# olofson/audiality2

Hardware: AMD Instinct MI355X
Metric: voice-samples/sec + max realtime voices @48kHz (higher is better)
Workload: dtype int32; 1 GPU; 65536 voices 2xwtosc->panmix, 256 per group voice inline->fbdelay->fbdelay (benchmark/fmtest4.a2s delay settings; 256 groups, 512 fbdelays), 48 kHz, fragment=64, stereo (BASELINE configs[3]); voices_per_gpu=65536, chain=osc2-pan, groups=256

## Files before the change

audiality2_amd/build.py:

```python
import hashlib
import os
import shutil
import subprocess

HERE = os.path.dirname(os.path.abspath(__file__))
ROOT = os.path.dirname(HERE)
HIPCC = shutil.which("hipcc") or "/opt/rocm/bin/hipcc"


MARK = b"A2AMD_SRCHASH:"


def source_hash(sources, cmd=()):
    h = hashlib.sha256()
    for s in sources:
        h.update(os.path.basename(s).encode() + b"\0")
        with open(s, "rb") as f:
            h.update(f.read())
        h.update(b"\0")
    h.update(" ".join(cmd).encode())
    return h.hexdigest()[:32]


def stamped_hash(lib, mark=MARK):
    if not os.path.exists(lib):
        return None
    with open(lib, "rb") as f:
        blob = f.read()
    i = blob.find(mark)
    if i < 0:
        return None
    return blob[i + len(mark):i + len(mark) + 32].decode("ascii", "replace")


ENGMARK = b"A2AMD_ENGHASH:"


def engine_hash(engine):
    files = []
    for d in ("include", "src", os.path.join("src", "units"), os.path.join("src", "drivers")):
        p = os.path.join(engine, d)
        if os.path.isdir(p):
            files += [os.path.join(p, f) for f in sorted(os.listdir(p)) if f.endswith((".h", ".h.cmake", ".h.in"))]
    return source_hash(files, (stamped_hash(os.path.join(HERE, "liba2amd_units.so")) or "",))


def _stale(target, want):
    return stamped_hash(target) != want


def _define(h):
    return '-DA2AMD_SRCHASH="%s"' % h


def build_lib(force=False):
    csrc = os.path.join(HERE, "csrc")
    srcs = [os.path.join(csrc, f) for f in ("a2amd_host.cpp", "a2amd_sched.cpp", "a2amd_render.cpp", "a2amd_dist.cpp",
                                            "a2amd_vm.cpp", "a2amd_kernels.hip", "a2amd_fast.hip", "a2amd_vm.hip", "a2amd_wavecap.hip", "a2amd_wavepost.hip", "a2amd_win.hip", "a2amd_vmwin.hip", "a2amd_noise.hip", "a2amd_noisepan.hip", "a2amd_noisefiltpan.hip", "a2amd_cutsweep.hip", "a2amd_oscbare.hip")]
    deps = srcs + [os.path.join(csrc, "a2amd_host.h"), os.path.join(csrc, "a2amd_switches.h"), os.path.join(csrc, "a2amd_device.h"), os.path.join(csrc, "a2amd_dsp.h"),
                   os.path.join(csrc, "a2amd_fm.h"), os.path.join(csrc, "a2amd_vmcore.h"), os.path.join(csrc, "a2amd_taps.h"), os.path.join(csrc, "a2amd_winctl.h"), os.path.join(csrc, "a2amd_vmdev.h"), os.path.join(csrc, "a2amd_noisemap.h"), os.path.join(csrc, "a2amd_noisevoice.h"), os.path.join(csrc, "a2amd_settled.h"), os.path.join(csrc, "a2amd_cutsweep.h"), os.path.join(csrc, "a2amd_filt.h"), os.path.join(ROOT, "include", "a2amd.h"),
                   os.path.join(ROOT, "include", "a2amd_noise.h"), os.path.join(ROOT, "include", "a2amd_noisepan.h"), os.path.join(ROOT, "include", "a2amd_noisefilt.h"), os.path.join(ROOT, "include", "a2amd_sweep.h"), os.path.join(ROOT, "include", "a2amd_wavepost.h"),
                   os.path.join(ROOT, "include", "a2amd_bus.h"), os.path.join(ROOT, "include", "a2amd_oscbare.h"), os.path.join(ROOT, "include", "a2amd_fbdpan.h"), os.path.join(ROOT, "include", "a2amd_buswin.h"), os.path.join(ROOT, "include", "a2amd_vmbatch.h"), os.path.join(ROOT, "include", "a2amd_osc2.h"), os.path.join(ROOT, "include", "a2amd_vm.h")]
    out = os.path.join(HERE, "liba2amd.so")
    flags = ["--offload-arch=gfx950", "-O3", "-std=c++17", "-fPIC", "-shared", "-Wno-unused-value"]
    want = source_hash(deps, flags)
    if force or _stale(out, want):
        subprocess.run([HIPCC] + flags + [_define(want), "-o", out] + srcs, check=True)
    return out


def build_units(force=False):
    src = os.path.join(HERE, "csrc", "a2amd_units.c")
    deps = [src, os.path.join(ROOT, "include", "a2amd.h"), os.path.join(ROOT, "include", "a2amd_noise.h"), os.path.join(ROOT, "include", "a2amd_noisepan.h"),
            os.path.join(ROOT, "include", "a2amd_noisefilt.h"), os.path.join(ROOT, "include", "a2amd_sweep.h"), os.path.join(ROOT, "include", "a2amd_bus.h"),
            os.path.join(ROOT, "include", "a2amd_wavepost.h"), os.path.join(ROOT, "include", "a2amd_oscbare.h"), os.path.join(ROOT, "include", "a2amd_fbdpan.h"), os.path.join(ROOT, "include", "a2amd_buswin.h"), os.path.join(ROOT, "include", "a2amd_vmbatch.h"), os.path.join(ROOT, "include", "a2amd_osc2.h"), os.path.join(ROOT, "include", "a2amd_plugin.h"),
            os.path.join(ROOT, "include", "a2amd_walk.h"), os.path.join(ROOT, "include", "a2amd_vm.h")]
    out = os.path.join(HERE, "liba2amd_units.so")
    flags = ["-O2", "-Wall", "-fPIC", "-shared"]
    want = source_hash(deps, flags)
    if force or _stale(out, want):
        subprocess.run(["gcc"] + flags + [_define(want), "-o", out, src,
                        "-L" + HERE, "-la2amd", "-ldl", "-lpthread", "-lm", "-Wl,-rpath,$ORIGIN"], check=True)
    return out


def build_walk(force=False, engine=None):
    engine = engine or os.environ.get("A2_ENGINE_SRC", "/root/reference")
    out = os.path.join(HERE, "liba2amd_walk.so")
    src = os.path.join(HERE, "csrc", "a2amd_walk.c")
    own = [src, os.path.join(ROOT, "include", "a2amd_walk.h"), os.path.join(ROOT, "include", "a2amd_vm.h"),
           os.path.join(ROOT, "include", "a2amd_plugin.h")]
    flags = ["-O2", "-Wall", "-fPIC", "-shared"]
    want = source_hash(own, flags)
    kept = os.path.join(ROOT, "oracle", "_ref", "liba2amd_walk.so")
    if not (os.path.exists(os.path.join(engine, "src", "internals.h")) and shutil.which("cmake")):
        if (not os.path.exists(out) or _stale(out, want)) and not _stale(kept, want):
            shutil.copyfile(kept, out)
        if os.path.exists(out) and _stale(out, want):
            raise RuntimeError(f"{out} was not built from this tree's a2amd_walk.c (stamp {stamped_hash(out)}, "
                               f"sources {want}) and the engine's source tree ({engine}) is not here to rebuild it")
        return out if os.path.exists(out) else None
    inc = os.path.join(HERE, "_engine_include")
    weng = engine_hash(engine)
    if force or _stale(out, want) or stamped_hash(out, ENGMARK) != weng:
        subprocess.run(["cmake", f"-DENGINE={engine}", f"-DOUT={inc}", "-P", os.path.join(HERE, "csrc", "engine_header.cmake")],
                       check=True, stdout=subprocess.DEVNULL)
        subprocess.run(["gcc"] + flags + [_define(want), '-DA2AMD_ENGHASH="%s"' % weng, "-I" + inc] +
                       ["-I" + os.path.join(engine, d) for d in ("include", "src", "src/units", "src/drivers")] +
                       ["-o", out, src, "-L" + HERE, "-la2amd_units", "-la2amd", "-ldl", "-lpthread", "-Wl,-rpath,$ORIGIN"],
                       check=True)
    if stamped_hash(kept) != want or stamped_hash(kept, ENGMARK) != weng:
        os.makedirs(os.path.dirname(kept), exist_ok=True)
        shutil.copyfile(out, kept)
    return out


def build_oracle(force=False):
    odir = os.path.join(ROOT, "oracle")
    targets = ["restate"]
    if os.path.exists("/root/reference/src/core.c") and shutil.which("cmake"):
        targets += ["ref", "tools", "optionb"]
    subprocess.run(["make", "-s", "-C", odir] + (["-B"] if force else []) + targets, check=True)
    return os.path.join(odir, "liba2oracle.so")


def build_all(force=False):
    lib = build_lib(force)
    build_units(force)
    build_walk(force)
    return lib, build_oracle(force)
```

audiality2_amd/csrc/a2amd_device.h:

```cpp
#pragma once
#include <stdint.h>

#define A2D_MAXCHAIN   16
#define A2D_CHAIN_INLINE 8
#define A2D_MAXBATCH 256
#define FBW_MAXWIN (2 * A2D_MAXBATCH)
#define A2D_USTATE    24
#define A2D_MAXCH      8
#define A2D_FRAG      64
#define A2D_MIPS      10
#define A2D_FBD_BUFSIZE 131072
#define A2D_MAXPHINC  512
#define A2D_COEF_WORDS 3
#define A2D_WTOSC_MAXLENGTH (0x01000000 - 1 - 131)

enum { A2D_WTOSC = 0, A2D_PANMIX, A2D_FILTER12, A2D_FBDELAY, A2D_INLINE, A2D_XINSERT,
	A2D_FM1, A2D_FM2, A2D_FM3, A2D_FM4, A2D_FM3P, A2D_FM4P, A2D_FM2R, A2D_FM4R,
	A2D_DC, A2D_WAVESHAPER, A2D_DCBLOCK, A2D_LIMITER, A2D_XSINK, A2D_XSOURCE };
#define A2D_IS_FM(k) ((k) >= A2D_FM1 && (k) <= A2D_FM4R)

enum { A2D_OSC_OFF = 0, A2D_OSC_NOISE, A2D_OSC_WAVE, A2D_OSC_MIPWAVE };

#define A2D_DESC(kind, add, nin, nout, wired) \
	(((uint32_t)(kind) << 24) | ((uint32_t)(add) << 4) | ((uint32_t)(nin) << 8) | \
	 ((uint32_t)(nout) << 12) | ((uint32_t)(wired) << 16))
#define A2D_KIND(d)  ((d) >> 24)
#define A2D_ADD(d)   (((d) >> 4) & 1u)
#define A2D_NIN(d)   (((d) >> 8) & 15u)
#define A2D_NOUT(d)  (((d) >> 12) & 15u)
#define A2D_WIRED(d) (((d) >> 16) & 1u)

enum {
	OW_MODE = 0, OW_WAVE, OW_DPHASE, OW_PHASE_LO, OW_PHASE_HI, OW_NOISE,
	OW_PRAMPING, OW_P = 7, OW_A = 11, OW_SEED = 15 };
enum {
	PW_VOL = 0, PW_PAN = 4 };
enum {
	FW_Q = 0, FW_LP = 4, FW_BP, FW_HP, FW_F1, FW_D1A, FW_D1B, FW_D2A, FW_D2B,
	FW_F1NEXT, FW_RAMP };
enum {
	DW_FBDELAY = 0, DW_LDELAY, DW_RDELAY, DW_DRYGAIN, DW_FBGAIN, DW_LGAIN,
	DW_RGAIN, DW_BUFPOS, DW_BUFIDX };

enum {
	CW_VALUE = 0, CW_MODE = 4 };
enum {
	SW_AMOUNT = 0 };
enum {
	BW_F1 = 0, BW_D1A, BW_D1B, BW_D2A, BW_D2B };
enum {
	LW_RELEASE = 0, LW_THRESHOLD, LW_PEAK };
enum {
	MW_SLOT = 0 };
enum {
	FO_A = 0, FO_FB = 4, FO_P = 8, FO_LASTPITCH = 12, FO_PHASE, FO_DPHASE, FO_LAST, FO_WORDS };
#define A2D_FMSTATE 64

#define A2D_WF_RAWTAPS 0x40000000u

struct A2DWave {
	int32_t  type;
	uint32_t flags;
	uint32_t period;
	uint32_t size[A2D_MIPS];
	uint32_t off[A2D_MIPS];
	uint32_t pad;
};

struct A2DVoice {
	int32_t nunits;
	int32_t unit[A2D_CHAIN_INLINE];
	int32_t out_off, out_nch;
	int32_t own_off, own_nch;
	int32_t pad[3];
};

static_assert(sizeof(A2DVoice) == 64, "the voice record is one 64-byte line");
struct A2DVoiceExt { int32_t unit[A2D_MAXCHAIN - A2D_CHAIN_INLINE]; };

struct A2DRec {
	uint32_t head;
	int32_t  value;
	uint32_t dur;
	uint32_t start;
};
enum { R_SEG = 1, R_WRITE, R_INIT, R_KILL, R_F1SET, R_F1RAMP, R_NOISESEED, R_NOP };
#define A2D_HEAD(frag, op, unit, reg) \
	((uint32_t)(frag) | ((uint32_t)(op) << 16) | ((uint32_t)(unit) << 24) | ((uint32_t)(reg) << 28))
#define A2D_RFRAG(h) ((h) & 0xffffu)
#define A2D_ROP(h)   (((h) >> 16) & 0xffu)
#define A2D_RUNIT(h) (((h) >> 24) & 15u)
#define A2D_RREG(h)  (((h) >> 28) & 15u)

struct A2DRun { int32_t first, count; };

#define A2D_VM_NOWRITE 0xffu
#define A2D_VM_TRAPWRITE 0xfeu
#define A2D_VM_MAXCUT  2
#define A2D_VM_MAXENV  2
#define A2D_VM_MAXPOS  8
#define A2D_VM_ENVPOS  14
#define A2D_ENV_LUTSHIFT 6
#define A2D_ENV_LUTSIZE  (1 << A2D_ENV_LUTSHIFT)
#define A2D_ENV_LUTS     8
struct A2DVmEnv {
	int32_t ramper[4];
	int32_t lut;
	int32_t scale, offset, out;
	int32_t active;
	uint8_t regbase;
	uint8_t k;
	uint8_t target;
	uint8_t pad;
};
struct A2DVmVoice {
	uint32_t waketime;
	uint32_t code, ncode;
	uint16_t pc;
	uint8_t  state, ncut;
	int32_t  voice;
	int32_t  fault;
	uint8_t  cmap[64];
	uint8_t  kind[A2D_MAXCHAIN];
	uint8_t  cutpos[A2D_VM_MAXCUT];
	uint8_t  pad[2];
	int32_t  cut[A2D_VM_MAXCUT][4];
	A2DVmEnv env[A2D_VM_MAXENV];
	int32_t  nenv;
	uint32_t exit_when;
	int32_t  has_exit;
	int32_t  r[64];
};

struct A2DVmParams {
	A2DVmVoice     *vmv;
	const int      *list;
	int32_t         n;
	const uint32_t *code;
	const uint32_t *ptab;
	const int32_t  *f1tab;
	const uint16_t *envlut;
	A2DRun         *runs;
	A2DRun         *vmrun;
	A2DRec         *recs;
	uint32_t        rec_base, rec_cap;
	uint32_t       *total;
	uint32_t        now;
	uint32_t        msdur;
	int32_t         samplerate, basepitch;
	int32_t         nfrags;
	uint8_t         fragframes[A2D_MAXBATCH];
	uint8_t         fragbase[A2D_MAXBATCH];
};

enum { XW_SLOT = 0, XW_MODE = 1 };
#define A2D_XIO_HALF ((size_t)A2D_MAXBATCH * 8 * A2D_FRAG)
#define A2D_XIO_SLOT (2 * A2D_XIO_HALF)

#define A2D_FAST_FCH 8
#define A2D_OSC2_FCH 4
#define A2D_OSC2_SCH 16
#define A2D_MAXVPW   32

struct A2DParams {
	const A2DVoice *voices;
	const A2DVoiceExt *vext;
	const uint32_t *udesc;
	int32_t        *ustate;
	int32_t        *vactive;
	const A2DRun   *runs;
	const A2DRec   *recs;
	const A2DWave  *waves;
	const int16_t  *wavepool;
	const int32_t  *wavecoef;
	int32_t        *busmem;
	int32_t        *fbdmem;
	const uint32_t *ptab;
	int32_t        *fmstate;
	const uint32_t *fmsine;
	int32_t *xio;
	const uint32_t *nseed;
	const int32_t  *nslot;
	int32_t         nnoise;
	const int32_t  *cutf;
	const int32_t  *cslot;
	int32_t         ncut;
	int32_t         nfrags;
	int32_t         samplerate;
	int32_t         debug;
	uint8_t         fragframes[A2D_MAXBATCH];
	uint16_t        fragstart[A2D_MAXBATCH];
};

#ifdef __HIPCC__
#define A2D_HD static inline __host__ __device__
#else
#define A2D_HD static inline
#endif
A2D_HD bool a2d_osc2_slice(int nfrags, int ysplit, int slice, int *c_lo, int *c_hi, int *nslices)
{
	const int nchunks = (nfrags + A2D_OSC2_FCH - 1) / A2D_OSC2_FCH;
	const int per = (nchunks + ysplit - 1) / ysplit;
	*c_lo = slice * per;
	*c_hi = *c_lo + per < nchunks ? *c_lo + per : nchunks;
	*nslices = (nchunks + per - 1) / per;
	return *c_lo < nchunks;
}
A2D_HD bool a2d_osc2_whole(unsigned start_first, unsigned start_last, unsigned frames_last, int n)
{
	return start_last + frames_last - start_first == (unsigned)n * A2D_FRAG;
}

#ifdef __HIPCC__
static inline __host__ __device__ bool a2d_noise_seed(const A2DParams &p, int f, int ui, unsigned *seed)
{
	if(!p.nseed)
		return false;
	const int k = p.nslot[ui];
	if(k <= 0 || k > p.nnoise)
		return false;
	*seed = p.nseed[(size_t)f * (size_t)p.nnoise + (size_t)(k - 1)];
	return true;
}
#endif

#ifdef __HIPCC__
static inline __host__ __device__ bool a2d_cut_coeff(const A2DParams &p, int f, int ui, int *f1)
{
	if(p.ncut <= 0)
		return false;
#if defined(__HIP_DEVICE_COMPILE__)
	typedef const __attribute__((address_space(4))) A2DParams *CP;
	typedef const __attribute__((address_space(4))) int32_t *CI;
	uintptr_t qa = (uintptr_t)&p;
	asm volatile("" : "+s"(qa));
	const CP q = (CP)qa;
	const int ncut = q->ncut;
	const int k = *((CI)(uintptr_t)q->cslot + ui);
	if(k <= 0 || k > ncut)
		return false;
	const int v = *((CI)(uintptr_t)q->cutf + ((size_t)f * (size_t)ncut + (size_t)(k - 1)));
#else
	const int k = p.cslot[ui];
	if(k <= 0 || k > p.ncut)
		return false;
	const int v = p.cutf[(size_t)f * (size_t)p.ncut + (size_t)(k - 1)];
#endif
	if(v < 0)
		return false;
	*f1 = v;
	return true;
}
#endif

struct A2DCutSweep { int32_t ramper[4]; int32_t unit, slot, pad[2]; };
int a2d_launch_cut_sweep(const A2DCutSweep *list, int n, int f0, int count, unsigned frames, int32_t *cutf, int stride,
		size_t words, int32_t *cslot, int nunits, void *stream);
int a2d_launch_cut_resolve(int32_t *cutf, size_t words, const int32_t *f1tab, void *stream);

struct A2DNoiseOsc { uint32_t ph_lo, ph_hi, dphase; int32_t unit, slot, pad[3]; };
int a2d_launch_noise_seeds(const A2DNoiseOsc *osc, int n, uint32_t start, int f0, int count, unsigned frames,
		uint32_t *seed, int stride, size_t seed_words, int32_t *nslot, int nunits, void *stream);

int a2d_launch_leaf_noisepan(const A2DParams *dparams, const A2DParams &hp, const int *dlist, int nlist, int vpw, void *stream);
int a2d_launch_leaf_noisefiltpan(const A2DParams *dparams, const A2DParams &hp, const int *dlist, int nlist, int vpg, void *stream);
int a2d_launch_leaf_oscbare(const A2DParams *dparams, const A2DParams &hp, const int *dlist, int nlist, int vpw, void *stream);

int a2d_launch_vm(const A2DVmParams &vp, int emit, void *stream);
int a2d_launch_vm_pool(const A2DVmParams &vp, unsigned *out, void *stream);
#define A2D_WIN_STAGED 2
struct A2DVmwOut {
	A2DVmVoice *vmv;
	int        *ustate;
	int        *vactive;
	A2DRun     *runs;
	uint32_t   *total;
	uint32_t   *idle;
};
int a2d_launch_vm_commit(const A2DVmParams &vp, const A2DParams &hp, int nosc, int filt, const A2DVmwOut &from, void *stream);
int a2d_launch_vm_win(const A2DVmParams &vp, const A2DParams &hp, int nosc, int filt, int fa, int fb, uint32_t now_fa,
		uint32_t batch_end, int *wslot, int *wext, int *wscr, unsigned *widx, unsigned *wtop, unsigned wcap, void *stream,
		const A2DVmwOut *out = nullptr);
#define A2D_VMW_ROW (64 - 1 - 1)

int a2d_launch_voices(const A2DParams *dparams, const int *dlist, int nlist, int vpw, void *stream);
enum { A2D_STAGED_NONE = 0, A2D_STAGED_PHASES, A2D_STAGED_FULL };
struct A2DCommit { const int *list; int nlist, nosc; const int *ustage; const unsigned char *staged; };
struct A2DCommitSet { A2DCommit c[2]; int n; };
int a2d_launch_leaf_oscpan(const A2DParams *dparams, const A2DParams &hp, const int *dlist, int nlist,
		int vpw, int ysplit, int *ustage, unsigned char *staged, void *stream, void *event_after_main, A2DCommit *defer);
int a2d_launch_bus_driver(const A2DParams *dparams, const int *dlist, int nlist, int nfrags, int consume,
		const A2DCommitSet *commits, void *stream, int *master_host = nullptr, int ramping = 0);
int a2d_launch_commit(const A2DParams &hp, const A2DCommit &cm, void *stream);
int a2d_launch_bus_fbdchain(const A2DParams *dparams, const int *dlist, int nlist, int consume, void *stream);
int a2d_launch_bus_fbdpan(const A2DParams *dparams, const int *dlist, int nlist, int consume, void *stream, int windows = 0);
int a2d_launch_park(int32_t *stage, int32_t *bus, unsigned words, void *stream);
int a2d_launch_add_bus(int32_t *dst, int32_t *src, unsigned words, void *stream);
int a2d_launch_add_inject(const int32_t *inj, int32_t *bus, int nch, int n, int nfrags, void *stream);
int a2d_launch_build_coef(const int16_t *pool, int *coef, unsigned lo, unsigned hi, void *stream);
int a2d_launch_capture(const int32_t *bus, int32_t *dst, const uint32_t *fragpos, int nfrags, int nch, void *stream);
int a2d_launch_wave_from_pcm(const int32_t *pcm, int16_t *pool, const uint32_t *off, const uint32_t *size, int levels, int looped,
		int pre, int post, void *stream);
int a2d_launch_wave_level0(const int32_t *pcm, int16_t *d, unsigned size, void *stream);
int a2d_launch_wave_finish(int16_t *pool, const uint32_t *off, const uint32_t *size, int levels, int looped, int pre, int post,
		void *stream);
unsigned a2d_wavepost_scratch_words(unsigned size, unsigned flags, unsigned chunk);
int a2d_launch_wave_level0_post(const int32_t *pcm, int16_t *d, unsigned size, unsigned flags, unsigned chunk, uint32_t *scratch,
		void *stream);
int a2d_osc2filtpan_max_vpg(void);
int a2d_launch_leaf_osc2filtpan(const A2DParams *dparams, const A2DParams &hp, const int *dlist, int nlist,
		int vpg, void *stream);
int a2d_launch_leaf_oscfiltpan(const A2DParams *dparams, const A2DParams &hp, const int *dlist, int nlist,
		int vpw, void *stream);
int a2d_launch_scatter_runs(const int *didx, const A2DRun *dval, int n, A2DRun *druns, void *stream);
int a2d_launch_leaf_osc2pan(const A2DParams *dparams, const A2DParams &hp, const int *dlist, int nlist,
		int vpw, int ysplit, int *ustage, unsigned char *staged, void *stream, A2DCommit *defer, int voice_major, int *ysplit_used);
struct A2Switches;
int a2d_launch_leaf_recs(const A2Switches &sw, const A2DParams *dparams, const A2DParams &hp, int nosc, int filt, const int *dlist,
		int nlist, int vpw, void *stream, int skip_empty = 0);
#define A2D_WIN_WORDS 24
#define A2D_WIN_SLOTWORDS(nosc, filt) ((filt) ? ((nosc) == 1 ? 20 : 24) : ((nosc) == 1 ? 12 : 20))
int a2d_launch_win_ctl(const A2DParams *dparams, const A2DParams &hp, int nosc, int filt, const int *dlist, int nlist,
		int skip_empty, int fa, int fb, int *wslot, int *wext, unsigned *widx, unsigned *wtop, unsigned wcap, int *wrc,
		void *stream);
int a2d_launch_win_render(const A2Switches &sw, const A2DParams &hp, int nosc, int filt, const int *dlist, int nlist, int fa, int fb,
		const int *wslot, const int *wext, const unsigned *widx, void *stream);
int a2d_launch_leaf_recs_all(const A2Switches &sw, const A2DParams *dparams, const A2DParams &hp, const int *const *lists, const int *counts,
		int vpw, void *stream, int skip_mask = 0);
int a2d_launch_leaf_fmpan(const A2DParams *dparams, const A2DParams &hp, int kind, const int *dlist, int nlist,
		int vpw, void *stream);
int a2d_launch_leaf_fmpan_all(const A2DParams *dparams, const A2DParams &hp, const int *dlist,
		const int *count8, int vpw, void *stream);
```

audiality2_amd/csrc/a2amd_fast.hip:

```cpp
#include <hip/hip_runtime.h>
#include <type_traits>
#include <algorithm>
#include <stdlib.h>
#include "a2amd_device.h"
#include "a2amd_switches.h"
#include "a2amd_dsp.h"
#include "a2amd_fm.h"
#include "a2amd_filt.h"

#include "a2amd_taps.h"

__global__ void k_build_coef(const int16_t *__restrict__ pool, int *__restrict__ coef, unsigned lo, unsigned hi)
{
	const unsigned j = lo + blockIdx.x * blockDim.x + threadIdx.x;
	if(j >= hi)
		return;
	const int dm = pool[j - 1], d0 = pool[j], d1 = pool[j + 1], d2 = pool[j + 2];
	const int c = (d1 - dm) >> 1;
	const int a = (3 * (d0 - d1) + d2 - dm) >> 1;
	const int b = dm - d0 + c - a;
	int *e = coef + A2D_COEF_WORDS * (size_t)j;
	e[0] = a;
	e[1] = b;
	e[2] = (int)(((unsigned)c << 16) | ((unsigned)d0 & 0xffffu));
// ... 75 lines not shown
};

struct OscPend { Quad16 qa, qb; unsigned ph, ph2; int ak, x; bool taps; };

DEV int osc_fragment_end(const OscPend &pd)
{
	if(pd.taps)
		return mul64s(inter_quads(pd.qa, pd.qb, pd.ph, pd.ph2), pd.ak, 17);
	return pd.x;
}

DEV OscPend osc_fragment_begin(const FastPtrs &g, OscS &o, int nframes, int lane)
{
	OscPend pd;
	pd.qa.lo = pd.qa.hi = pd.qb.lo = pd.qb.hi = 0;
	pd.ph = pd.ph2 = 0;
	pd.ak = 0;
	pd.taps = false;
	int x = 0;
	const bool in = (unsigned)lane < (unsigned)nframes;
	if(o.mode == A2D_OSC_MIPWAVE) {
		const A2DWave *w = g.waves + o.wave;
		const unsigned size0 = w->size[0], period = w->period, flags = w->flags;
		if(!size0) {
			o.wave = -1;
			o.mode = A2D_OSC_OFF;
		} else {
			ramp_prepare_s(o.p, nframes);
			if(!(o.dphase && (!o.p.timer && !o.p_ramping))) {
				unsigned lastv = (unsigned)o.p.value;
				ramp_run(o.p, nframes);
				o.p_ramping = o.p.delta;
				o.dphase = (unsigned)rfl((int)p2i(g.ptab, (int)((lastv + (unsigned)o.p.value) >> 9)));
			}
			ramp_prepare_s(o.a, nframes);
			unsigned dph;
			const unsigned mm = a2s_mip(o.dphase, period, &dph);
			uint64_t ph = o.phase >> mm;
			const unsigned sizem = w->size[mm];
			bool play = true;
			if(flags & 0x100u) {
				ph = wrap_phase(ph, sizem);
			} else if((ph >> 24) > (uint64_t)(sizem + 1))
				play = false;
			if(play) {
				if(dph <= (A2D_MAXPHINC << 16)) {
					const int16_t *d = g.wavepool + w->off[mm];
					if(in) {
						uint64_t phk = ph + (uint64_t)(unsigned)lane * dph;
						pd.ak = wadd(o.a.value, wmul(o.a.delta, lane));
						pd.ph = (unsigned)(phk >> 16);
						pd.ph2 = pd.ph + ((dph >> 16) >> 1);
						pd.qa = *(const Quad16 *)(d + (int)(pd.ph >> 8) - 1);
						pd.qb = *(const Quad16 *)(d + (int)(pd.ph2 >> 8) - 1);
						pd.taps = true;
					}
				}
				ph += (uint64_t)dph * (unsigned)nframes;
				o.phase = ph << mm;
				ramp_run(o.a, nframes);
			}
		}
	} else if(o.mode == A2D_OSC_NOISE) {
		ramp_prepare_s(o.p, nframes);
		if(!(o.dphase && (!o.p.timer && !o.p_ramping))) {
			unsigned lastv = (unsigned)o.p.value;
			ramp_run(o.p, nframes);
			o.p_ramping = o.p.delta;
			o.dphase = (unsigned)rfl((int)p2i(g.ptab, (int)((lastv + (unsigned)o.p.value) >> 9)));
		}
		ramp_prepare_s(o.a, nframes);
		const uint64_t phk = o.phase + (uint64_t)(unsigned)(in ? lane : 0) * o.dphase;
		const uint64_t nph = phk + o.dphase;
		const bool draw = in && ((o.dphase >= (1u << 23)) || ((nph ^ phk) >> 23));
		const unsigned long long m = __ballot(draw);
		const int me = (int)(threadIdx.x & 63);
		const unsigned long long below = (me >= 63) ? ~0ull : ((2ull << me) - 1ull);
		const int mine = __popcll(m & below), total = __popcll(m);
		int held = o.noise, myval = o.noise;
		unsigned st = o.seed;
		for(int j = 1; j <= total; ++j) {
			held = noise_next(st) - 32767;
			if(j == mine)
				myval = held;
		}
		o.seed = st;
		o.noise = held;
		if(in) {
			int ak = wadd(o.a.value, wmul(o.a.delta, lane));
			x = wmul(myval, ak >> 10) >> 6;
		}
		o.phase += (uint64_t)(unsigned)nframes * o.dphase;
		ramp_run(o.a, nframes);
	} else {
		ramp_prepare_s(o.p, nframes);
		ramp_prepare_s(o.a, nframes);
		ramp_run(o.p, nframes);
		ramp_run(o.a, nframes);
	}
	pd.x = x;
	return pd;
}

DEV int osc_fragment_s(const FastPtrs &g, OscS &o, int nframes, int lane)
{
	const OscPend pd = osc_fragment_begin(g, o, nframes, lane);
	return osc_fragment_end(pd);
}

DEV void pan_fragment_s(Ramp &vol, Ramp &pan, int x, int nframes, int lane, int &acc0, int &acc1)
{
	const bool clamp = a2s_pan_over(pan.target) || a2s_pan_over(pan.value);
	ramp_prepare_s(vol, nframes);
	ramp_prepare_s(pan, nframes);
	if((unsigned)lane < (unsigned)nframes) {
		int vk = wadd(vol.value, wmul(vol.delta, lane));
		int pk = wadd(pan.value, wmul(pan.delta, lane));
		int vp = mul64s(pk, vk, 24);
		int v0 = wsub(vk, vp), v1 = wadd(vk, vp);
		if(clamp) {
			int lim = wshl(vk, 1);
			if(v0 > lim) v0 = lim;
			if(v1 > lim) v1 = lim;
		}
		acc0 = wadd(acc0, mul64s(x, v0, 24));
		acc1 = wadd(acc1, mul64s(x, v1, 24));
	}
	ramp_run(vol, nframes);
	ramp_run(pan, nframes);
}

DEV void oscpan_fragment(const FastPtrs &g, OscS &o, Ramp &vol, Ramp &pan,
		int nframes, int lane, int &acc0, int &acc1)
{
	int x = osc_fragment_s(g, o, nframes, lane);
	pan_fragment_s(vol, pan, x, nframes, lane, acc0, acc1);
}

DEV int frames_of(const int (&ffr)[A2D_MAXBATCH / 64], int f)
{
	int r = 0;
#pragma unroll
	for(int k = 0; k < A2D_MAXBATCH / 64; ++k)
		if((f >> 6) == k)
			r = rdl(ffr[k], f & 63);
	return r;
}

enum { SV_MODE = 0, SV_WAVE, SV_DPHASE, SV_PHLO, SV_PHHI, SV_PRAMP, SV_P = 6, SV_A = 10,
	SV_VOL = 14, SV_PAN = 18, SV_NWORDS = 22 };

enum { DV_SETTLED = 0, DV_MM, DV_DPH, DV_SIZEM, DV_DOFF, DV_V0, DV_V1, DV_NWORDS };

DEV bool settled_wave(const A2DWave *w, unsigned dphase, int *d, bool settled = true)
{
	unsigned dph;
	const unsigned mm = a2s_mip(dphase, w->period, &dph);
	d[0] = (int)mm;
	d[1] = (int)dph;
	d[2] = (int)w->size[mm];
	d[3] = (int)w->off[mm];
	return settled && a2s_wave_ok(w->size[0], w->flags, dph);
}

DEV void osc_from_mem(OscS &o, const volatile int *w)
{
	o.mode = rfl(w[OW_MODE]);
	o.wave = rfl(w[OW_WAVE]);
	o.dphase = (unsigned)rfl(w[OW_DPHASE]);
	o.phase = (uint64_t)(unsigned)rfl(w[OW_PHASE_LO]) | ((uint64_t)(unsigned)rfl(w[OW_PHASE_HI]) << 32);
	o.p_ramping = rfl(w[OW_PRAMPING]);
	o.p.value = rfl(w[OW_P]); o.p.target = rfl(w[OW_P + 1]);
	o.p.delta = rfl(w[OW_P + 2]); o.p.timer = rfl(w[OW_P + 3]);
	o.a.value = rfl(w[OW_A]); o.a.target = rfl(w[OW_A + 1]);
	o.a.delta = rfl(w[OW_A + 2]); o.a.timer = rfl(w[OW_A + 3]);
	o.noise = 0;
	o.seed = 0;
}

DEV void osc_to_mem(int *w, const OscS &o)
{
	w[OW_MODE] = o.mode;
	w[OW_WAVE] = o.wave;
	w[OW_DPHASE] = (int)o.dphase;
	w[OW_PHASE_LO] = (int)(unsigned)o.phase;
	w[OW_PHASE_HI] = (int)(unsigned)(o.phase >> 32);
	w[OW_PRAMPING] = o.p_ramping;
	w[OW_P] = o.p.value; w[OW_P + 1] = o.p.target; w[OW_P + 2] = o.p.delta; w[OW_P + 3] = o.p.timer;
	w[OW_A] = o.a.value; w[OW_A + 1] = o.a.target; w[OW_A + 2] = o.a.delta; w[OW_A + 3] = o.a.timer;
}

DEV void stage_mark(unsigned char *m, bool mine, bool settled, bool last_slice, bool walker)
{
	if(mine && !settled) {
		if(walker)
			*m = A2D_STAGED_FULL;
	} else if(last_slice)
		*m = mine ? A2D_STAGED_PHASES : A2D_STAGED_NONE;
}

#define OSC1_WPE 4
__global__ __launch_bounds__(64 * FAST_WPB) __attribute__((amdgpu_waves_per_eu(OSC1_WPE, OSC1_WPE)))
void k_leaf_oscpan(const A2DParams *__restrict__ pp, const int *__restrict__ list, int nlist, int vpw,
		int ysplit, const A2DVoice *__restrict__ voices, const int *ustate,
		int *ustage, const int16_t *__restrict__ wavepool,
		const A2DWave *__restrict__ waves, const uint32_t *__restrict__ ptab, int *__restrict__ busmem,
		const int *__restrict__ wavecoef, unsigned char *__restrict__ staged)
{
	const A2DParams &p = *pp;
	const int wv = rfl((int)(threadIdx.x >> 6));
	const int lane = threadIdx.x & 63;
	const int first = (blockIdx.x * FAST_WPB + wv) * vpw;
	if(first >= nlist)
		return;
	const int nv = min(vpw, nlist - first);
	const int nfrags = p.nfrags;
	const int dbg = p.debug;
	FastPtrs g = { wavepool, waves, ptab, dbg };
	const CoefRsrc crs = coef_rsrc(wavecoef);

	const int nchunks = (nfrags + FAST_FCH - 1) / FAST_FCH;
	const int per = (nchunks + ysplit - 1) / ysplit;
	const int slice = blockIdx.y;
	const int c_lo = slice * per, c_hi = min(nchunks, c_lo + per);
	const bool last_slice = c_hi >= nchunks;
	if(c_lo >= nchunks)
		return;
	const int nslices = (nchunks + per - 1) / per;

	int ffr[A2D_MAXBATCH / 64], fst[A2D_MAXBATCH / 64];
#pragma unroll
	for(int k = 0; k < A2D_MAXBATCH / 64; ++k) {
		ffr[k] = (k * 64 + lane < nfrags) ? p.fragframes[k * 64 + lane] : 0;
		fst[k] = (k * 64 + lane < nfrags) ? p.fragstart[k * 64 + lane] : 0;
	}

	int dv[DV_NWORDS], amp_l = 0, phlo_l = 0, phhi_l = 0;
	int u0 = 0, u1 = 0, my_off = -1, my_nch = 2;
	bool mine = false;
#pragma unroll
	for(int k = 0; k < DV_NWORDS; ++k)
		dv[k] = 0;
	if(lane < nv)
		mine = p.runs[list[first + lane]].count == 0;
	if(mine) {
		const A2DVoice &vc = voices[list[first + lane]];
		u0 = vc.unit[0];
		u1 = vc.unit[1];
		my_off = vc.out_off;
		my_nch = vc.out_nch;
		const int *w0 = ustate + (size_t)u0 * A2D_USTATE;
		const int *w1 = ustate + (size_t)u1 * A2D_USTATE;
		int sv[SV_NWORDS];
		sv[SV_MODE] = w0[OW_MODE]; sv[SV_WAVE] = w0[OW_WAVE]; sv[SV_DPHASE] = w0[OW_DPHASE];
		sv[SV_PHLO] = w0[OW_PHASE_LO]; sv[SV_PHHI] = w0[OW_PHASE_HI]; sv[SV_PRAMP] = w0[OW_PRAMPING];
#pragma unroll
		for(int k = 0; k < 4; ++k) {
			sv[SV_P + k] = w0[OW_P + k];
			sv[SV_A + k] = w0[OW_A + k];
			sv[SV_VOL + k] = w1[PW_VOL + k];
			sv[SV_PAN + k] = w1[PW_PAN + k];
		}
		bool settled = a2s_osc_settled(sv[SV_MODE], (unsigned)sv[SV_DPHASE], sv[SV_PRAMP], sv + SV_P, sv + SV_A) &&
				a2s_arrived(sv + SV_VOL, sv + SV_PAN);
		if(settled) {
			settled = settled_wave(waves + sv[SV_WAVE], (unsigned)sv[SV_DPHASE], dv + DV_MM);
			a2s_pan_gains(sv[SV_VOL], sv[SV_PAN], a2s_pan_over(sv[SV_PAN]), &dv[DV_V0], &dv[DV_V1]);
		}
		dv[DV_SETTLED] = settled ? ((sv[SV_MODE] == A2D_OSC_MIPWAVE && (waves[sv[SV_WAVE]].flags & A2D_WF_RAWTAPS)) ? 3 : 1) : 0;
		amp_l = sv[SV_A];
		phlo_l = sv[SV_PHLO];
		phhi_l = sv[SV_PHHI];
	}
	const unsigned long long unsettled_mask = __ballot(mine && !dv[DV_SETTLED]);
	const unsigned long long settled_mask = __ballot(mine && dv[DV_SETTLED]);
	const unsigned long long raw_mask = __ballot(mine && dv[DV_SETTLED] == 3);

	for(int c = c_lo; c < c_hi; ++c) {
		const int f0 = c * FAST_FCH;
		const int nf = min((int)FAST_FCH, nfrags - f0);
		int acc0[FAST_FCH], acc1[FAST_FCH];
#pragma unroll
		for(int j = 0; j < FAST_FCH; ++j)
			acc0[j] = acc1[j] = 0;
		int nfr[FAST_FCH];
#pragma unroll
		for(int j = 0; j < FAST_FCH; ++j)
			nfr[j] = (j < nf) ? frames_of(ffr, f0 + j) : 0;
		const unsigned before = (unsigned)frames_of(fst, f0);
		unsigned pre[FAST_FCH];
		pre[0] = 0;
#pragma unroll
		for(int j = 1; j < FAST_FCH; ++j)
			pre[j] = pre[j - 1] + (unsigned)nfr[j - 1];
		const uint64_t lbase = ((((uint64_t)(unsigned)phlo_l) | ((uint64_t)(unsigned)phhi_l << 32)) >>
				(unsigned)dv[DV_MM]) + (uint64_t)before * (unsigned)dv[DV_DPH];
		const int base_lo = (int)(unsigned)lbase, base_hi = (int)(unsigned)(lbase >> 32);
		int cur_off = rdl(my_off, 0), cur_nch = rdl(my_nch, 0);
		for(int v = 0; v < nv; ++v) {
			if(!((settled_mask >> v) & 1ull))
				continue;
			const int voff = rdl(my_off, v);
			if(voff != cur_off) {
				flush_acc(busmem, cur_off, cur_nch, f0, nf, lane, dbg, acc0, acc1);
				cur_off = voff;
				cur_nch = rdl(my_nch, v);
			}
			const unsigned dph = (unsigned)rdl(dv[DV_DPH], v);
			const unsigned sizem = (unsigned)rdl(dv[DV_SIZEM], v), doff = (unsigned)rdl(dv[DV_DOFF], v);
			const int v0 = rdl(dv[DV_V0], v), v1 = rdl(dv[DV_V1], v), amp = rdl(amp_l, v);
			const unsigned dph16 = dph >> 16;
			uint64_t ph = (uint64_t)(unsigned)rdl(base_lo, v) | ((uint64_t)(unsigned)rdl(base_hi, v) << 32);
			uint64_t phs[FAST_FCH];
			if(!(sizem & (sizem - 1)) && !(ph >> 48)) {
// ... 48 lines not shown
					kb[j] = coef_at(crs, cb, pb[j]);
				}
#pragma unroll
				for(int j = 0; j < 4; ++j) {
					int sm = inter_coefs(ka[j], pa[j], kb[j], pb[j]);
					int x = mul64s(sm, amp, 17);
					x = (lane < nfr[h + j]) ? x : 0;
					acc0[h + j] = wadd(acc0[h + j], mul64s(x, v0, 24));
					acc1[h + j] = wadd(acc1[h + j], mul64s(x, v1, 24));
				}
			}
			if(last_slice && c == c_hi - 1) {
				const bool me = lane == v;
				const uint64_t endph = ph << (unsigned)rdl(dv[DV_MM], v);
				WRL(phlo_l, (int)(unsigned)endph);
				WRL(phhi_l, (int)(unsigned)(endph >> 32));
			}
		}
		flush_acc(busmem, cur_off, cur_nch, f0, nf, lane, dbg, acc0, acc1);
	}

	const unsigned long long todo_mask = unsettled_mask & __ballot(lane % nslices == slice);
	if(todo_mask) {
		for(int f0 = 0; f0 < nfrags; f0 += FAST_FCH) {
			const int nf = min((int)FAST_FCH, nfrags - f0);
			int acc0[FAST_FCH], acc1[FAST_FCH];
#pragma unroll
			for(int j = 0; j < FAST_FCH; ++j)
				acc0[j] = acc1[j] = 0;
			int cur_off = rdl(my_off, 0), cur_nch = rdl(my_nch, 0);
			for(int v = 0; v < nv; ++v) {
				if(!((todo_mask >> v) & 1ull))
					continue;
				const int voff = rdl(my_off, v);
				if(voff != cur_off) {
					flush_acc(busmem, cur_off, cur_nch, f0, nf, lane, dbg, acc0, acc1);
					cur_off = voff;
					cur_nch = rdl(my_nch, v);
				}
				OscS o;
				Ramp vol, pan;
				const int *src = f0 ? ustage : ustate;
				osc_from_mem(o, src + (size_t)rdl(u0, v) * A2D_USTATE);
				{
					const volatile int *wpv = src + (size_t)rdl(u1, v) * A2D_USTATE;
					vol.value = rfl(wpv[0]); vol.target = rfl(wpv[1]); vol.delta = rfl(wpv[2]); vol.timer = rfl(wpv[3]);
					pan.value = rfl(wpv[4]); pan.target = rfl(wpv[5]); pan.delta = rfl(wpv[6]); pan.timer = rfl(wpv[7]);
				}
				for(int j = 0; j < nf; ++j) {
					int o0 = 0, o1 = 0;
					oscpan_fragment(g, o, vol, pan, frames_of(ffr, f0 + j), lane, o0, o1);
#pragma unroll
					for(int jj = 0; jj < FAST_FCH; ++jj)
						if(jj == j) {
							acc0[jj] = wadd(acc0[jj], o0);
							acc1[jj] = wadd(acc1[jj], o1);
						}
				}
				if(lane == 0) {
					osc_to_mem(ustage + (size_t)rdl(u0, v) * A2D_USTATE, o);
					int *wpv = ustage + (size_t)rdl(u1, v) * A2D_USTATE;
					wpv[0] = vol.value; wpv[1] = vol.target; wpv[2] = vol.delta; wpv[3] = vol.timer;
					wpv[4] = pan.value; wpv[5] = pan.target; wpv[6] = pan.delta; wpv[7] = pan.timer;
				}
			}
			flush_acc(busmem, cur_off, cur_nch, f0, nf, lane, dbg, acc0, acc1);
			__builtin_amdgcn_fence(__ATOMIC_RELEASE, "wavefront");
			__builtin_amdgcn_s_waitcnt(0);
		}
	}

	if(mine && dv[DV_SETTLED] && last_slice) {
		int *w0 = ustage + (size_t)u0 * A2D_USTATE;
		w0[OW_PHASE_LO] = phlo_l;
		w0[OW_PHASE_HI] = phhi_l;
	}
	if(ustage != ustate && lane < nv)
		stage_mark(staged + first + lane, mine, dv[DV_SETTLED] != 0, last_slice, lane % nslices == slice);
}

DEV void commit_block(const A2DCommit &cm, int block, const A2DVoice *__restrict__ voices, int *__restrict__ ustate)
{
	const int i = block * 256 + threadIdx.x;
	if(i >= cm.nlist * cm.nosc)
		return;
	const int e = i / cm.nosc, o = i - e * cm.nosc;
	const int what = cm.staged[e];
	if(what == A2D_STAGED_NONE)
		return;
	const A2DVoice &vc = voices[cm.list[e]];
	const size_t a = (size_t)vc.unit[o] * A2D_USTATE;
	ustate[a + OW_PHASE_LO] = cm.ustage[a + OW_PHASE_LO];
	ustate[a + OW_PHASE_HI] = cm.ustage[a + OW_PHASE_HI];
	if(what != A2D_STAGED_FULL)
		return;
	for(int k = 0; k < 15; ++k)
		if(k != OW_NOISE && k != OW_PHASE_LO && k != OW_PHASE_HI)
			ustate[a + k] = cm.ustage[a + k];
	if(o == 0) {
		const size_t ap = (size_t)vc.unit[cm.nosc] * A2D_USTATE;
		for(int k = 0; k < 8; ++k)
			ustate[ap + k] = cm.ustage[ap + k];
	}
}

DEV int commit_blocks(const A2DCommit &cm) { return (cm.nlist * cm.nosc + 255) / 256; }

__global__ __launch_bounds__(256)
void k_commit_oscpan(A2DCommit cm, const A2DVoice *__restrict__ voices, int *__restrict__ ustate)
{
	commit_block(cm, blockIdx.x, voices, ustate);
}

#define OSC2_FCH A2D_OSC2_FCH
#define OSC2_SCH A2D_OSC2_SCH
static_assert(OSC2_SCH % OSC2_FCH == 0, "a super-chunk is whole chunks");
enum { OV_MODE = 0, OV_WAVE, OV_DPHASE, OV_PHLO, OV_PHHI, OV_PRAMP, OV_P = 6, OV_A = 10, OV_NWORDS = 14 };
enum { OD_MM = 0, OD_DPH, OD_SIZEM, OD_DOFF, OD_NWORDS };

DEV void osc_from_lanes(OscS &o, const int (&so)[OV_NWORDS], int v)
{
	o.mode = rdl(so[OV_MODE], v);
	o.wave = rdl(so[OV_WAVE], v);
	o.dphase = (unsigned)rdl(so[OV_DPHASE], v);
	o.phase = (uint64_t)(unsigned)rdl(so[OV_PHLO], v) | ((uint64_t)(unsigned)rdl(so[OV_PHHI], v) << 32);
	o.p_ramping = rdl(so[OV_PRAMP], v);
	o.p.value = rdl(so[OV_P], v); o.p.target = rdl(so[OV_P + 1], v);
	o.p.delta = rdl(so[OV_P + 2], v); o.p.timer = rdl(so[OV_P + 3], v);
	o.a.value = rdl(so[OV_A], v); o.a.target = rdl(so[OV_A + 1], v);
	o.a.delta = rdl(so[OV_A + 2], v); o.a.timer = rdl(so[OV_A + 3], v);
	o.noise = 0;
	o.seed = 0;
}

DEV void osc_to_lanes(int (&so)[OV_NWORDS], const OscS &o, bool me)
{
	WRL(so[OV_MODE], o.mode);
	WRL(so[OV_WAVE], o.wave);
	WRL(so[OV_DPHASE], (int)o.dphase);
	WRL(so[OV_PHLO], (int)(unsigned)o.phase);
	WRL(so[OV_PHHI], (int)(unsigned)(o.phase >> 32));
	WRL(so[OV_PRAMP], o.p_ramping);
	WRL(so[OV_P], o.p.value); WRL(so[OV_P + 1], o.p.target);
	WRL(so[OV_P + 2], o.p.delta); WRL(so[OV_P + 3], o.p.timer);
	WRL(so[OV_A], o.a.value); WRL(so[OV_A + 1], o.a.target);
	WRL(so[OV_A + 2], o.a.delta); WRL(so[OV_A + 3], o.a.timer);
}

struct Osc2Voice {
	unsigned dph[2], sizem[2];
	int cb[2], amp[2];
	uint64_t ph[2], end[2];
};

template<bool WHOLE>
DEV void osc2_chunk(const CoefRsrc &crs, Osc2Voice &s, const unsigned (&ldph)[2], const int (&nfr)[OSC2_FCH],
		const unsigned (&pre)[OSC2_FCH], int nf, bool park, int (&xs)[OSC2_FCH])
{
	Coef4 ka[2][OSC2_FCH], kb[2][OSC2_FCH];
	unsigned pa[2][OSC2_FCH], pb[2][OSC2_FCH];
#pragma unroll
	for(int o = 0; o < 2; ++o) {
		const unsigned dph = s.dph[o], sizem = s.sizem[o];
		uint64_t ph = s.ph[o];
		uint64_t phs[OSC2_FCH];
		if(!(sizem & (sizem - 1)) && !(ph >> 48)) {
			const uint64_t mask = ((uint64_t)sizem << 24) - 1;
#pragma unroll
			for(int j = 0; j < OSC2_FCH; ++j)
				phs[j] = (ph + (uint64_t)dph * (WHOLE ? (unsigned)(j * A2D_FRAG) : pre[j])) & mask;
			ph = phs[OSC2_FCH - 1] + (uint64_t)dph * (WHOLE ? (unsigned)A2D_FRAG : (unsigned)nfr[OSC2_FCH - 1]);
		} else {
#pragma unroll
			for(int j = 0; j < OSC2_FCH; ++j) {
				ph = wrap_phase(ph, sizem);
				phs[j] = ph;
				ph += (uint64_t)dph * (WHOLE ? (unsigned)A2D_FRAG : (unsigned)nfr[j]);
			}
		}
#pragma unroll
		for(int j = 0; j < OSC2_FCH; ++j) {
			pa[o][j] = tap_phase(phs[j], ldph[o]);
			asm("" : "+v"(pa[o][j]));
			pb[o][j] = pa[o][j] + (dph >> 17);
			ka[o][j] = coef_at(crs, s.cb[o], pa[o][j]);
			kb[o][j] = coef_at(crs, s.cb[o], pb[o][j]);
		}
		if(park) {
			uint64_t e = ph;
#pragma unroll
			for(int j = OSC2_FCH - 2; j >= 0; --j)
				if(nf == j + 1)
					e = phs[j] + (uint64_t)dph * (WHOLE ? (unsigned)A2D_FRAG : (unsigned)nfr[j]);
			s.end[o] = e;
		}
		s.ph[o] = ph;
	}
#pragma unroll
	for(int o = 0; o < 2; ++o)
#pragma unroll
		for(int j = 0; j < OSC2_FCH; ++j) {
			const int y = mul64s(inter_coefs(ka[o][j], pa[o][j], kb[o][j], pb[o][j]), s.amp[o], 17);
			xs[j] = o ? wadd(xs[j], y) : y;
		}
}

DEV void osc2_voice_from_lanes(Osc2Voice &s, unsigned (&ldph)[2], unsigned (&mm)[2], const int (&od)[2][OD_NWORDS],
		const int (&amp_l)[2], const int (&phlo_l)[2], const int (&phhi_l)[2], int v, unsigned before, int lane)
{
#pragma unroll
	for(int o = 0; o < 2; ++o) {
		mm[o] = (unsigned)rdl(od[o][OD_MM], v);
		s.dph[o] = (unsigned)rdl(od[o][OD_DPH], v);
		s.sizem[o] = (unsigned)rdl(od[o][OD_SIZEM], v);
		s.cb[o] = coef_base((unsigned)rdl(od[o][OD_DOFF], v));
		s.amp[o] = rdl(amp_l[o], v);
		const uint64_t phase = (uint64_t)(unsigned)rdl(phlo_l[o], v) | ((uint64_t)(unsigned)rdl(phhi_l[o], v) << 32);
		s.ph[o] = (phase >> mm[o]) + (uint64_t)before * s.dph[o];
		ldph[o] = lane_dph(lane, s.dph[o]);
	}
}

#define OSC2_WPE 4
__global__ __launch_bounds__(64 * FAST_WPB) __attribute__((amdgpu_waves_per_eu(OSC2_WPE, OSC2_WPE)))
void k_leaf_osc2pan(const A2DParams *__restrict__ pp, const int *__restrict__ list, int nlist, int vpw,
		int ysplit, const A2DVoice *__restrict__ voices, const int *ustate, int *ustage,
		const int16_t *__restrict__ wavepool, const A2DWave *__restrict__ waves,
		const uint32_t *__restrict__ ptab, int *__restrict__ busmem, const int *__restrict__ wavecoef,
		unsigned char *__restrict__ staged, int vmajor)
{
	const A2DParams &p = *pp;
	const int wv = rfl((int)(threadIdx.x >> 6));
	const int lane = threadIdx.x & 63;
	const int first = (blockIdx.x * FAST_WPB + wv) * vpw;
	if(first >= nlist)
		return;
	const int nv = min(vpw, nlist - first);
	const int nfrags = p.nfrags;
	const int dbg = p.debug;
	FastPtrs g = { wavepool, waves, ptab, dbg };
	const CoefRsrc crs = coef_rsrc(wavecoef);

	const int slice = blockIdx.y;
	int c_lo, c_hi, nslices;
	if(!a2d_osc2_slice(nfrags, ysplit, slice, &c_lo, &c_hi, &nslices))
		return;
	const bool last_slice = c_hi * OSC2_FCH >= nfrags;

	int ffr[A2D_MAXBATCH / 64], fst[A2D_MAXBATCH / 64];
#pragma unroll
	for(int k = 0; k < A2D_MAXBATCH / 64; ++k) {
		ffr[k] = (k * 64 + lane < nfrags) ? p.fragframes[k * 64 + lane] : 0;
		fst[k] = (k * 64 + lane < nfrags) ? p.fragstart[k * 64 + lane] : 0;
	}

	int od[2][OD_NWORDS], amp_l[2] = { 0, 0 }, phlo_l[2] = { 0, 0 }, phhi_l[2] = { 0, 0 };
	int v0l = 0, v1l = 0, settled_l = 0;
	int uu[3] = { 0, 0, 0 }, my_off = -1, my_nch = 2;
	bool mine = false;
#pragma unroll
	for(int o = 0; o < 2; ++o)
#pragma unroll
		for(int k = 0; k < OD_NWORDS; ++k)
			od[o][k] = 0;
	if(lane < nv)
		mine = p.runs[list[first + lane]].count == 0;
	if(mine) {
		const A2DVoice &vc = voices[list[first + lane]];
		my_off = vc.out_off;
		my_nch = vc.out_nch;
		bool settled = true;
		int wave_l[2], dphase_l[2];
#pragma unroll
		for(int o = 0; o < 2; ++o) {
			uu[o] = vc.unit[o];
			const int *w = ustate + (size_t)uu[o] * A2D_USTATE;
			wave_l[o] = w[OW_WAVE];
			dphase_l[o] = w[OW_DPHASE];
			amp_l[o] = w[OW_A];
			phlo_l[o] = w[OW_PHASE_LO];
			phhi_l[o] = w[OW_PHASE_HI];
			settled = settled && a2s_osc_settled(w[OW_MODE], (unsigned)dphase_l[o], w[OW_PRAMPING], w + OW_P, w + OW_A);
		}
		uu[2] = vc.unit[2];
		const int *wp = ustate + (size_t)uu[2] * A2D_USTATE;
		int sp[8];
#pragma unroll
		for(int k = 0; k < 8; ++k)
			sp[k] = wp[k];
		settled = settled && a2s_arrived(sp + PW_VOL, sp + PW_PAN);
		if(settled) {
#pragma unroll
			for(int o = 0; o < 2; ++o)
				settled = settled_wave(waves + wave_l[o], (unsigned)dphase_l[o], od[o], settled);
			a2s_pan_gains(sp[PW_VOL], sp[PW_PAN], a2s_pan_over(sp[PW_PAN]), &v0l, &v1l);
		}
		settled_l = settled ? 1 : 0;
	}
	const unsigned long long unsettled_mask = __ballot(mine && !settled_l);

	__shared__ int tiles[FAST_WPB][OSC2_SCH][2][A2D_FRAG];
	int (*const tile)[2][A2D_FRAG] = tiles[wv];
	if(vmajor)
#pragma unroll
		for(int r = 0; r < OSC2_SCH; ++r)
			tile[r][0][lane] = tile[r][1][lane] = 0;
	for(int s_lo = c_lo; s_lo < c_hi; s_lo += OSC2_SCH / OSC2_FCH) {
		const int s_hi = min(c_hi, s_lo + OSC2_SCH / OSC2_FCH);
		const int fa = s_lo * OSC2_FCH, nfs = min(nfrags, s_hi * OSC2_FCH) - fa;
		const bool last = last_slice && s_hi == c_hi;
		const unsigned before = (unsigned)frames_of(fst, fa);
		if(vmajor && a2d_osc2_whole(before, (unsigned)frames_of(fst, fa + nfs - 1), (unsigned)frames_of(ffr, fa + nfs - 1), nfs)) {
			const int nsc = s_hi - s_lo;
			const int nopre_i[OSC2_FCH] = { 0, 0, 0, 0 };
			const unsigned nopre_u[OSC2_FCH] = { 0, 0, 0, 0 };
			int cur_off = rdl(my_off, 0), cur_nch = rdl(my_nch, 0);
			for(int v = 0; v < nv; ++v) {
				if(!rdl(settled_l, v))
					continue;
				const int voff = rdl(my_off, v);
				if(voff != cur_off) {
					flush_tile(busmem, cur_off, cur_nch, fa, nfs, nsc * OSC2_FCH, lane, dbg, tile);
					cur_off = voff;
					cur_nch = rdl(my_nch, v);
				}
				const int v0 = rdl(v0l, v), v1 = rdl(v1l, v);
				Osc2Voice s;
				unsigned ldph[2], mm[2];
				osc2_voice_from_lanes(s, ldph, mm, od, amp_l, phlo_l, phhi_l, v, before, lane);
				for(int k = 0; k < nsc; ++k) {
					const bool park = last && k == nsc - 1;
					int xs[OSC2_FCH];
					osc2_chunk<true>(crs, s, ldph, nopre_i, nopre_u, nfs - k * OSC2_FCH, park, xs);
#pragma unroll
					for(int j = 0; j < OSC2_FCH; ++j) {
						tile_add(&tile[k * OSC2_FCH + j][0][lane], mul64s(xs[j], v0, 24));
						tile_add(&tile[k * OSC2_FCH + j][1][lane], mul64s(xs[j], v1, 24));
					}
					if(park) {
						const bool me = lane == v;
#pragma unroll
						for(int o = 0; o < 2; ++o) {
							const uint64_t endph = s.end[o] << mm[o];
							WRL(phlo_l[o], (int)(unsigned)endph);
							WRL(phhi_l[o], (int)(unsigned)(endph >> 32));
						}
					}
				}
			}
			flush_tile(busmem, cur_off, cur_nch, fa, nfs, nsc * OSC2_FCH, lane, dbg, tile);
			continue;
		}
		for(int c = s_lo; c < s_hi; ++c) {
			const int f0 = c * OSC2_FCH;
			const int nf = min((int)OSC2_FCH, nfrags - f0);
			int acc0[OSC2_FCH], acc1[OSC2_FCH], nfr[OSC2_FCH];
#pragma unroll
			for(int j = 0; j < OSC2_FCH; ++j) {
				acc0[j] = acc1[j] = 0;
				nfr[j] = (j < nf) ? frames_of(ffr, f0 + j) : 0;
			}
			const unsigned before = (unsigned)frames_of(fst, f0);
			unsigned pre[OSC2_FCH];
			pre[0] = 0;
#pragma unroll
			for(int j = 1; j < OSC2_FCH; ++j)
				pre[j] = pre[j - 1] + (unsigned)nfr[j - 1];
			const bool park = last && c == s_hi - 1;
			int cur_off = rdl(my_off, 0), cur_nch = rdl(my_nch, 0);
			for(int v = 0; v < nv; ++v) {
				if(!rdl(settled_l, v))
					continue;
				const int voff = rdl(my_off, v);
				if(voff != cur_off) {
					flush_acc(busmem, cur_off, cur_nch, f0, nf, lane, dbg, acc0, acc1);
					cur_off = voff;
					cur_nch = rdl(my_nch, v);
				}
				const int v0 = rdl(v0l, v), v1 = rdl(v1l, v);
				Osc2Voice s;
				unsigned ldph[2], mm[2];
				int xs[OSC2_FCH];
				osc2_voice_from_lanes(s, ldph, mm, od, amp_l, phlo_l, phhi_l, v, before, lane);
				osc2_chunk<false>(crs, s, ldph, nfr, pre, nf, park, xs);
#pragma unroll
				for(int j = 0; j < OSC2_FCH; ++j) {
					const int x = (lane < nfr[j]) ? xs[j] : 0;
					acc0[j] = wadd(acc0[j], mul64s(x, v0, 24));
					acc1[j] = wadd(acc1[j], mul64s(x, v1, 24));
				}
				if(park) {
					const bool me = lane == v;
#pragma unroll
					for(int o = 0; o < 2; ++o) {
						const uint64_t endph = s.end[o] << mm[o];
						WRL(phlo_l[o], (int)(unsigned)endph);
						WRL(phhi_l[o], (int)(unsigned)(endph >> 32));
					}
				}
			}
			flush_acc(busmem, cur_off, cur_nch, f0, nf, lane, dbg, acc0, acc1);
		}
	}

	const unsigned long long todo_mask = unsettled_mask & __ballot(lane % nslices == slice);
	if(todo_mask) {
		for(int f0 = 0; f0 < nfrags; f0 += OSC2_FCH) {
			const int nf = min((int)OSC2_FCH, nfrags - f0);
			int acc0[OSC2_FCH], acc1[OSC2_FCH];
#pragma unroll
			for(int j = 0; j < OSC2_FCH; ++j)
				acc0[j] = acc1[j] = 0;
			int cur_off = rdl(my_off, 0), cur_nch = rdl(my_nch, 0);
			for(int v = 0; v < nv; ++v) {
				if(!((todo_mask >> v) & 1ull))
					continue;
				const int voff = rdl(my_off, v);
				if(voff != cur_off) {
					flush_acc(busmem, cur_off, cur_nch, f0, nf, lane, dbg, acc0, acc1);
					cur_off = voff;
					cur_nch = rdl(my_nch, v);
				}
				OscS oa, ob;
				Ramp vol, pan;
				const int *src = f0 ? ustage : ustate;
				osc_from_mem(oa, src + (size_t)rdl(uu[0], v) * A2D_USTATE);
				osc_from_mem(ob, src + (size_t)rdl(uu[1], v) * A2D_USTATE);
				{
					const volatile int *wpv = src + (size_t)rdl(uu[2], v) * A2D_USTATE;
					vol.value = rfl(wpv[0]); vol.target = rfl(wpv[1]); vol.delta = rfl(wpv[2]); vol.timer = rfl(wpv[3]);
					pan.value = rfl(wpv[4]); pan.target = rfl(wpv[5]); pan.delta = rfl(wpv[6]); pan.timer = rfl(wpv[7]);
				}
				for(int j = 0; j < nf; ++j) {
					const int n = frames_of(ffr, f0 + j);
					int o0 = 0, o1 = 0;
					const OscPend pa_ = osc_fragment_begin(g, oa, n, lane), pb_ = osc_fragment_begin(g, ob, n, lane);
					const int x = wadd(osc_fragment_end(pa_), osc_fragment_end(pb_));
					pan_fragment_s(vol, pan, x, n, lane, o0, o1);
#pragma unroll
					for(int jj = 0; jj < OSC2_FCH; ++jj)
						if(jj == j) {
							acc0[jj] = wadd(acc0[jj], o0);
							acc1[jj] = wadd(acc1[jj], o1);
						}
				}
				if(lane == 0) {
					osc_to_mem(ustage + (size_t)rdl(uu[0], v) * A2D_USTATE, oa);
					osc_to_mem(ustage + (size_t)rdl(uu[1], v) * A2D_USTATE, ob);
					int *wpv = ustage + (size_t)rdl(uu[2], v) * A2D_USTATE;
					wpv[0] = vol.value; wpv[1] = vol.target; wpv[2] = vol.delta; wpv[3] = vol.timer;
					wpv[4] = pan.value; wpv[5] = pan.target; wpv[6] = pan.delta; wpv[7] = pan.timer;
				}
			}
			flush_acc(busmem, cur_off, cur_nch, f0, nf, lane, dbg, acc0, acc1);
			__builtin_amdgcn_fence(__ATOMIC_RELEASE, "wavefront");
			__builtin_amdgcn_s_waitcnt(0);
		}
	}

	if(mine && settled_l && last_slice) {
#pragma unroll
		for(int o = 0; o < 2; ++o) {
			int *w = ustage + (size_t)uu[o] * A2D_USTATE;
			w[OW_PHASE_LO] = phlo_l[o];
			w[OW_PHASE_HI] = phhi_l[o];
		}
	}
	if(ustage != ustate && lane < nv)
		stage_mark(staged + first + lane, mine, settled_l != 0, last_slice, lane % nslices == slice);
}

#define RECS_FCH 4
#define RECS_WPB 8

DEV void osc_init_s(const FastPtrs &g, OscS &o, int pitch)
{
	o.wave = -1;
	o.mode = A2D_OSC_OFF;
	o.phase = 0;
	o.p_ramping = 0;
	o.noise = 0;
	o.seed = 0;
	ramp_init(o.a, 0);
	ramp_init(o.p, pitch);
	o.dphase = (unsigned)rfl((int)p2i(g.ptab, o.p.value >> 8));
}

DEV void osc_write_s(const FastPtrs &g, OscS &o, int reg, int v, int start, int dur)
{
	switch(reg) {
	  case 0: {
		int wt = 0;
		o.wave = v;
		if(v >= 0) {
			const A2DWave *w = g.waves + v;
			wt = w->type;
			if(wt == 3 && w->size[0] > (unsigned)A2D_WTOSC_MAXLENGTH)
				wt = 0;
		}
		if(wt == 3)
			o.mode = A2D_OSC_MIPWAVE;
		else if(wt == 1)
			o.mode = A2D_OSC_NOISE;
// ... 1692 lines not shown
#pragma unroll
	for(int k = 0; k < FBC_MAXD; ++k)
		if(k < nd) {
			const int *w = p.ustate + (size_t)vc.unit[k + 1] * A2D_USTATE;
			d[k].fb = rfl(w[DW_FBDELAY]); d[k].l = rfl(w[DW_LDELAY]); d[k].r = rfl(w[DW_RDELAY]);
			d[k].dry = rfl(w[DW_DRYGAIN]); d[k].fbg = rfl(w[DW_FBGAIN]); d[k].lg = rfl(w[DW_LGAIN]); d[k].rg = rfl(w[DW_RGAIN]);
			d[k].pos = rfl(w[DW_BUFPOS]);
			d[k].b0 = p.fbdmem + (size_t)rfl(w[DW_BUFIDX]) * 2 * A2D_FBD_BUFSIZE;
			d[k].b1 = d[k].b0 + A2D_FBD_BUFSIZE;
			d[k].add = rfl((int)A2D_ADD(p.udesc[vc.unit[k + 1]]));
			dmin = min(dmin, min(d[k].fb, min(d[k].l, d[k].r)));
			dmax = max(dmax, max(d[k].fb, max(d[k].l, d[k].r)));
		}
	__syncthreads();
	const bool rest = at_rest != 0;
	int rv0 = 0, rv1 = 0;
	if(rest) {
		const int vk = fr[0][0], vp = mul64s(fr[0][2], vk, 24);
		rv0 = wsub(vk, vp); rv1 = wadd(vk, vp);
		if(fr[0][4]) {
			const int lim = wshl(vk, 1);
			if(rv0 > lim) rv0 = lim;
			if(rv1 > lim) rv1 = lim;
		}
	}
	const int rf = max(1, min(dmin, A2D_FBD_BUFSIZE - dmax) / A2D_FRAG);
	int *own = p.busmem + vc.own_off;
	int *out = p.busmem + vc.out_off;
	const int out_nch = vc.out_nch;
	for(int f0 = 0; f0 < nfrags; f0 += rf) {
		const int fend = min(nfrags, f0 + rf);
		for(int idx = f0 * A2D_FRAG + (int)threadIdx.x; idx < fend * A2D_FRAG; idx += FBC_THREADS) {
			const int f = idx >> 6, lane = idx & 63;
			if(lane >= p.fragframes[f])
				continue;
			const int t = (int)p.fragstart[f] + lane;
			int *src = own + (size_t)f * 2 * A2D_FRAG;
			int x0 = src[lane], x1 = src[A2D_FRAG + lane];
			if(consume) {
				src[lane] = 0;
				src[A2D_FRAG + lane] = 0;
			}
#pragma unroll
			for(int k = 0; k < FBC_MAXD; ++k)
				if(k < nd) {
					const FbdU &u = d[k];
					const int pos = wadd(u.pos, t);
					int o0 = mul64s(u.b1[(pos - u.fb) & M], u.fbg, 16);
					int o1 = mul64s(u.b0[(pos - u.fb) & M], u.fbg, 16);
					const int t0 = u.b0[(pos - u.l) & M], t1 = u.b1[(pos - u.r) & M];
					u.b0[pos & M] = wadd(x0, o0);
					u.b1[pos & M] = wadd(x1, o1);
					o0 = wadd(o0, mul64s(t0, u.lg, 16));
					o1 = wadd(o1, mul64s(t1, u.rg, 16));
					o0 = wadd(o0, mul64s(x0, u.dry, 16));
					o1 = wadd(o1, mul64s(x1, u.dry, 16));
					if(u.add) {
						x0 = wadd(x0, o0);
						x1 = wadd(x1, o1);
					} else {
						x0 = o0;
						x1 = o1;
					}
				}
			int v0 = rv0, v1 = rv1;
			if(!rest) {
				int r = f, wk = lane;
				if constexpr(WIN) {
					r = min((int)wfirst[f], FBW_MAXWIN - 1);
					const int rl = min((int)wfirst[f + 1], FBW_MAXWIN) - 1;
					while(r < rl && lane >= (fr[r][4] >> 16))
						++r;
					wk = lane - ((fr[r][4] >> 8) & 0xff);
				}
				const int vk = wadd(fr[r][0], wmul(fr[r][1], wk));
				const int pk = wadd(fr[r][2], wmul(fr[r][3], wk));
				const int vp = mul64s(pk, vk, 24);
				v0 = wsub(vk, vp); v1 = wadd(vk, vp);
				if(WIN ? fr[r][4] & 1 : fr[r][4]) {
					const int lim = wshl(vk, 1);
					if(v0 > lim) v0 = lim;
					if(v1 > lim) v1 = lim;
				}
			}
			const int o0 = mul64s(x0, v0, 24), o1 = mul64s(x1, v1, 24);
			int *dst = out + (size_t)f * out_nch * A2D_FRAG;
			if(o0)
				atomicAdd(&dst[lane], o0);
			if(o1)
				atomicAdd(&dst[A2D_FRAG + lane], o1);
		}
		if(fend < nfrags)
			__syncthreads();
	}
	if(threadIdx.x == 0) {
		int total = 0;
		for(int f = 0; f < nfrags; ++f)
			total += p.fragframes[f];
#pragma unroll
		for(int k = 0; k < FBC_MAXD; ++k)
			if(k < nd)
				p.ustate[(size_t)vc.unit[k + 1] * A2D_USTATE + DW_BUFPOS] = wadd(d[k].pos, total);
	}
}

__global__ __launch_bounds__(FBC_THREADS)
void k_bus_fbdpan(const A2DParams *__restrict__ pp, const int *__restrict__ list, int nlist, int consume)
{
	bus_fbdpan<false>(pp, list, consume);
}

__global__ __launch_bounds__(FBC_THREADS)
void k_bus_fbdpan_win(const A2DParams *__restrict__ pp, const int *__restrict__ list, int nlist, int consume)
{
	bus_fbdpan<true>(pp, list, consume);
}

int a2d_launch_bus_fbdpan(const A2DParams *dparams, const int *dlist, int nlist, int consume, void *stream, int windows)
{
	if(nlist <= 0)
		return 0;
	hipLaunchKernelGGL(windows ? k_bus_fbdpan_win : k_bus_fbdpan, dim3(nlist), dim3(FBC_THREADS), 0, (hipStream_t)stream,
			dparams, dlist, nlist, consume);
	return (int)hipGetLastError();
}

int a2d_launch_leaf_oscpan(const A2DParams *dparams, const A2DParams &hp, const int *dlist, int nlist,
		int vpw, int ysplit, int *ustage, unsigned char *staged, void *stream, void *event_after_main, A2DCommit *defer)
{
	if(nlist <= 0)
		return 0;
	vpw = vpw < 1 ? 1 : (vpw > 64 ? 64 : vpw);
	if(ysplit < 1 || !ustage || !staged)
		ysplit = 1;
	int nwaves = (nlist + vpw - 1) / vpw;
	int nblocks = (nwaves + FAST_WPB - 1) / FAST_WPB;
	hipLaunchKernelGGL(k_leaf_oscpan, dim3(nblocks, ysplit), dim3(64 * FAST_WPB), 0, (hipStream_t)stream,
			dparams, dlist, nlist, vpw, ysplit, hp.voices, (const int *)hp.ustate,
			ysplit > 1 ? ustage : hp.ustate, hp.wavepool, hp.waves, hp.ptab, hp.busmem, hp.wavecoef, staged);
	if(event_after_main)
		hipEventRecord((hipEvent_t)event_after_main, (hipStream_t)stream);
	if(ysplit > 1) {
		A2DCommit cm = { dlist, nlist, 1, ustage, staged };
		if(defer)
			*defer = cm;
		else
			a2d_launch_commit(hp, cm, stream);
	} else if(defer)
		defer->nlist = 0;
	return (int)hipGetLastError();
}

int a2d_launch_leaf_osc2pan(const A2DParams *dparams, const A2DParams &hp, const int *dlist, int nlist,
		int vpw, int ysplit, int *ustage, unsigned char *staged, void *stream, A2DCommit *defer, int voice_major, int *ysplit_used)
{
	if(nlist <= 0)
		return 0;
	vpw = vpw < 1 ? 1 : (vpw > 64 ? 64 : vpw);
	if(ysplit < 1 || !ustage || !staged)
		ysplit = 1;
	if(ysplit_used)
		*ysplit_used = ysplit;
	int nwaves = (nlist + vpw - 1) / vpw;
	int nblocks = (nwaves + FAST_WPB - 1) / FAST_WPB;
	hipLaunchKernelGGL(k_leaf_osc2pan, dim3(nblocks, ysplit), dim3(64 * FAST_WPB), 0, (hipStream_t)stream,
			dparams, dlist, nlist, vpw, ysplit, hp.voices, (const int *)hp.ustate,
			ysplit > 1 ? ustage : hp.ustate, hp.wavepool, hp.waves, hp.ptab, hp.busmem, hp.wavecoef, staged, voice_major);
	if(ysplit > 1) {
		A2DCommit cm = { dlist, nlist, 2, ustage, staged };
		if(defer)
			*defer = cm;
		else
			a2d_launch_commit(hp, cm, stream);
	} else if(defer)
		defer->nlist = 0;
	return (int)hipGetLastError();
}

__global__ void k_scatter_runs(const int *__restrict__ idx, const A2DRun *__restrict__ val, int n,
		A2DRun *__restrict__ runs)
{
	int i = blockIdx.x * blockDim.x + threadIdx.x;
	if(i < n)
		runs[idx[i]] = val[i];
}

int a2d_launch_scatter_runs(const int *didx, const A2DRun *dval, int n, A2DRun *druns, void *stream)
{
	if(n <= 0)
		return 0;
	hipLaunchKernelGGL(k_scatter_runs, dim3((n + 255) / 256), dim3(256), 0, (hipStream_t)stream,
			didx, dval, n, druns);
	return (int)hipGetLastError();
}

int a2d_launch_leaf_oscfiltpan(const A2DParams *dparams, const A2DParams &hp, const int *dlist, int nlist,
		int vpg, void *stream)
{
	if(nlist <= 0)
		return 0;
	vpg = vpg < 1 ? 1 : (vpg > FILT_MAXV ? FILT_MAXV : vpg);
	int nblocks = (nlist + vpg - 1) / vpg;
	size_t lds = (size_t)3 * vpg * FILT_PITCH * sizeof(int);
	hipLaunchKernelGGL(k_leaf_oscfiltpan, dim3(nblocks), dim3(64 * FILT_WAVES), lds, (hipStream_t)stream,
			dparams, dlist, nlist, vpg, hp.voices, hp.ustate, hp.wavepool, hp.waves, hp.ptab, hp.busmem, hp.wavecoef);
	return (int)hipGetLastError();
}

int a2d_osc2filtpan_max_vpg(void)
{
	const int nfull = FILT_WAVES - 1 - (FILT_WAVES / 4 - 1);
	const int v = nfull * (FILT2_LAUNCHV < FILT2_FASTV ? FILT2_LAUNCHV : FILT2_FASTV);
	return v > FILT_MAXV ? FILT_MAXV : v;
}

int a2d_launch_leaf_osc2filtpan(const A2DParams *dparams, const A2DParams &hp, const int *dlist, int nlist,
		int vpg, void *stream)
{
	if(nlist <= 0)
		return 0;
	vpg = vpg < 1 ? 1 : (vpg > FILT_MAXV ? FILT_MAXV : vpg);
	int nblocks = (nlist + vpg - 1) / vpg;
	size_t lds = (size_t)3 * vpg * FILT_PITCH * sizeof(int);
	hipLaunchKernelGGL(k_leaf_osc2filtpan, dim3(nblocks), dim3(64 * FILT_WAVES), lds, (hipStream_t)stream,
			dparams, dlist, nlist, vpg, hp.voices, hp.ustate, hp.wavepool, hp.waves, hp.ptab, hp.busmem, hp.wavecoef);
	return (int)hipGetLastError();
}

enum { PV_VOL = 0, PV_PAN = 4, PV_NWORDS = 8 };

DEV void pan_window_s(Ramp &vol, Ramp &pan, int x, int off, int len, int lane, int &acc0, int &acc1)
{
	const bool clamp = a2s_pan_over(pan.target) || a2s_pan_over(pan.value);
	ramp_prepare_s(vol, len);
	ramp_prepare_s(pan, len);
	const int k = lane - off;
	if(k >= 0 && k < len) {
		int vk = wadd(vol.value, wmul(vol.delta, k));
		int pk = wadd(pan.value, wmul(pan.delta, k));
		int vp = mul64s(pk, vk, 24);
		int v0 = wsub(vk, vp), v1 = wadd(vk, vp);
		if(clamp) {
			int lim = wshl(vk, 1);
			if(v0 > lim) v0 = lim;
			if(v1 > lim) v1 = lim;
		}
		acc0 = wadd(acc0, mul64s(x, v0, 24));
		acc1 = wadd(acc1, mul64s(x, v1, 24));
	}
	ramp_run(vol, len);
	ramp_run(pan, len);
}

template<int NOPS, int OSBITS, int PAR>
DEV void fmpan_body(const A2DParams &p, const int *__restrict__ list, int first, int nv, int lane,
		int *tile, const uint32_t *sine, const A2DVoice *__restrict__ voices, int *ustate,
		int *fmstate, const uint32_t *__restrict__ ptab, int *__restrict__ busmem)
{
	const int nfrags = p.nfrags;
	const int dbg = p.debug;
	const A2DRec *__restrict__ recs = p.recs;
	int ffr[A2D_MAXBATCH / 64];
#pragma unroll
	for(int k = 0; k < A2D_MAXBATCH / 64; ++k)
		ffr[k] = (k * 64 + lane < nfrags) ? p.fragframes[k * 64 + lane] : 0;

	int pv[PV_NWORDS];
#pragma unroll
	for(int k = 0; k < PV_NWORDS; ++k)
		pv[k] = 0;
	FmOp op[NOPS];
#pragma unroll
	for(int i = 0; i < NOPS; ++i) {
		op[i].a = op[i].fb = op[i].p = Ramp{ 0, 0, 0, 0 };
		op[i].last_pitch = op[i].last = 0;
		op[i].phase = op[i].dphase = 0;
	}
	unsigned step[NOPS], fix[NOPS];
#pragma unroll
	for(int i = 0; i < NOPS; ++i)
		step[i] = fix[i] = 0;
	int slot = -1, u0 = 0, u1 = 0, my_off = -1, my_nch = 2, v0 = 0, v1 = 0, settled = 0;
	int run_first = 0, run_count = 0, fmslot = -1;
	int actB = 0;
	const bool writer = lane < nv;
	if(lane < nv)
		slot = list[first + lane];
	else if(lane < 16 && !(p.debug & 4))
		slot = list[first + lane % nv];
	const bool mine = slot >= 0;
	const unsigned long long mine_mask = __ballot(mine);
	if(mine) {
		const A2DVoice &vc = voices[slot];
		u0 = vc.unit[0];
		u1 = vc.unit[1];
		my_off = vc.out_off;
		my_nch = vc.out_nch;
		const A2DRun run = p.runs[slot];
		run_first = run.first;
		run_count = run.count;
		actB = p.vactive[slot];
	}
	bool touched = mine && actB;
	if(touched) {
		fmslot = ustate[(size_t)u0 * A2D_USTATE + MW_SLOT];
		const int *fw = fmstate + (size_t)fmslot * A2D_FMSTATE;
#pragma unroll
		for(int i = 0; i < NOPS; ++i)
			fmop_load(op[i], fw + i * FO_WORDS);
		const int *w1 = ustate + (size_t)u1 * A2D_USTATE;
#pragma unroll
		for(int k = 0; k < 4; ++k) {
			pv[PV_VOL + k] = w1[PW_VOL + k];
			pv[PV_PAN + k] = w1[PW_PAN + k];
		}
		settled = !run_count && a2s_arrived(pv + PV_VOL, pv + PV_PAN);
		if(settled)
			a2s_pan_gains(pv[PV_VOL], pv[PV_PAN], a2s_pan_over(pv[PV_PAN]), &v0, &v1);
	}
	int curB = 0, curC = 0, actC = actB;
// ... 389 lines not shown
```

audiality2_amd/csrc/a2amd_host.cpp:

```cpp
#include "a2amd_host.h"
#include "a2amd_noisemap.h"
#include "a2amd_cutsweep.h"
#include "a2amd_settled.h"

namespace a2h { thread_local char g_err[256] = ""; }

extern "C" {

const char *a2amd_version(void) { return "a2amd 0.1 (gfx950)"; }
#ifndef A2AMD_SRCHASH
#define A2AMD_SRCHASH "unstamped"
#endif
const char *a2amd_source_stamp(void) { return "A2AMD_SRCHASH:" A2AMD_SRCHASH; }

const char *a2amd_last_error(const a2amd_ctx *c) { return c ? c->err : g_err; }

int a2amd_device_count(void)
{
	int n = 0;
	return hipGetDeviceCount(&n) == hipSuccess ? n : 0;
}


int a2amd_open(const a2amd_config *cfg, a2amd_ctx **out)
{
	if(!cfg || !out || cfg->channels < 1 || cfg->channels > A2D_MAXCH || cfg->samplerate <= 0) {
		snprintf(g_err, sizeof(g_err), "a2amd_open: bad configuration");
		return A2AMD_EINVAL;
	}
	int ndev = 0;
	hipError_t e = hipGetDeviceCount(&ndev);
	if(e != hipSuccess || ndev <= 0 || cfg->device >= ndev) {
		snprintf(g_err, sizeof(g_err), "a2amd_open: no usable HIP device (%s, %d devices, want #%d); "
				"this library has no CPU fallback", hipGetErrorString(e), ndev, cfg->device);
		return A2AMD_ENODEVICE;
	}
	a2amd_ctx *c = new a2amd_ctx();
	c->cfg = *cfg;
	c->err[0] = 0;
	if(!c->cfg.max_batch)
		c->cfg.max_batch = 1;
	if(c->cfg.max_batch > A2D_MAXBATCH)
		c->cfg.max_batch = A2D_MAXBATCH;
	memset(&c->stats, 0, sizeof(c->stats));
	build_pitch_table(c->ptab);
	a2amd_read_switches(&c->sw);
	c->bus_stride_frames = (size_t)c->cfg.max_batch * A2D_FRAG;
	c->bus_used = c->bus_stride_frames * (size_t)c->cfg.channels;
#define OPENCHK(call) do { hipError_t e_ = (call); if(e_ != hipSuccess) { \
	snprintf(g_err, sizeof(g_err), "a2amd_open: %s: %s", #call, hipGetErrorString(e_)); \
	delete c; return A2AMD_EHIP; } } while(0)
	OPENCHK(hipSetDevice(cfg->device));
	if(cfg->stream)
		c->stream = (hipStream_t)cfg->stream;
	else {
		OPENCHK(hipStreamCreateWithFlags(&c->stream, hipStreamNonBlocking));
		c->own_stream = true;
	}
	OPENCHK(hipEventCreate(&c->ev0));
	OPENCHK(hipEventCreate(&c->ev1));
	OPENCHK(hipEventCreate(&c->ev2));
	c->ev_pool.push_back(c->ev0);
	c->ev_pool.push_back(c->ev1);
	c->ev_pool.push_back(c->ev2);
	OPENCHK(hipMalloc((void **)&c->d_ptab, sizeof(c->ptab)));
	OPENCHK(hipMalloc((void **)&c->d_wavepool.d, (size_t)(8u << 20) * sizeof(int16_t)));
	c->d_wavepool.cap = 8u << 20;
	OPENCHK(hipMalloc((void **)&c->d_wavecoef.d, (size_t)(8u << 20) * A2D_COEF_WORDS * sizeof(int32_t)));
	c->d_wavecoef.cap = 8u << 20;
#undef OPENCHK
	*out = c;
	return A2AMD_OK;
}

void a2amd_close(a2amd_ctx *c)
{
	if(!c)
		return;
	use_device(c);
	hipStreamSynchronize(c->stream);
	if(c->vm.pred_stream)
		hipStreamSynchronize(c->vm.pred_stream);
	drop_graphs(c);
	if(c->comm && g_rccl.CommDestroy)
		g_rccl.CommDestroy(c->comm);
	if(c->grp_ev)
		hipEventDestroy(c->grp_ev);
	hipFree(c->d_voices.d); hipFree(c->d_vext.d); hipFree(c->d_udesc.d); hipFree(c->d_ustate.d); hipFree(c->d_ustage.d);
	hipFree(c->d_vactive.d); hipFree(c->d_runs.d); hipFree(c->d_recs.d);
	hipFree(c->d_nseed.d); hipFree(c->d_nslot.d);
	hipFree(c->d_cutf.d); hipFree(c->d_cslot.d);
	hipFree(c->d_win.d); hipFree(c->d_wext.d); hipFree(c->d_wscr.d); hipFree(c->d_wrc.d); hipFree(c->d_widx.d); hipFree(c->d_wtop);
	if(c->h_wtop)
		hipHostFree(c->h_wtop);
	if(c->wtop_ev)
		hipEventDestroy(c->wtop_ev);
	if(c->win_stream)
		hipStreamDestroy(c->win_stream);
	for(int k = 0; k < 7; ++k)
		if(c->win_fork[k])
			hipStreamDestroy(c->win_fork[k]);
	for(int k = 0; k < 8; ++k)
		if(c->win_fev[k])
			hipEventDestroy(c->win_fev[k]);
	for(int k = 0; k < 5; ++k)
		if(c->win_ev[k])
			hipEventDestroy(c->win_ev[k]);
	hipFree(c->d_waves.d); hipFree(c->d_wavepool.d); hipFree(c->d_wavecoef.d); hipFree(c->d_busmem.d);
	vm_close(c);
	hipFree(c->capture.d); hipFree(c->capture.d_fragpos); hipFree(c->d_wavepost.d);
	hipFree(c->d_fbdmem.d); hipFree(c->d_fmstate.d); hipFree(c->d_xio.d); hipFree(c->d_fmsine); hipFree(c->d_list.d); hipFree(c->d_staged.d); hipFree(c->d_scatter.d); hipFree(c->d_ptab); hipFree(c->d_blob.d);
	for(int k = 0; k < 2; ++k) { if(c->h_blob[k]) hipHostFree(c->h_blob[k]); if(c->blob_ev[k]) hipEventDestroy(c->blob_ev[k]); }
	if(c->h_master)
		hipHostFree(c->h_master);
	for(int k = 0; k < 2; ++k) { if(c->rb[k].h) hipHostFree(c->rb[k].h); if(c->rb[k].ev) hipEventDestroy(c->rb[k].ev); }
	for(hipEvent_t e : c->ev_pool)
		hipEventDestroy(e);
	if(c->own_stream)
		hipStreamDestroy(c->stream);
	delete c;
}

int a2amd_set_pitch_table(a2amd_ctx *c, const uint32_t *t)
{
	memcpy(c->ptab, t, sizeof(c->ptab));
	c->ptab_dirty = true;
	return A2AMD_OK;
}

int a2amd_get_pitch_table(const a2amd_ctx *c, uint32_t *t)
{
	memcpy(t, c->ptab, sizeof(c->ptab));
	return A2AMD_OK;
}

}
namespace a2h {
void wave_tap_policy(a2amd_ctx *c)
{
	const int force = c->sw.raw;
	const size_t budget = (size_t)c->sw.coef_cache_mb << 20;
	const bool big = c->wavepool_used * (4 * A2D_COEF_WORDS) > budget;
	for(size_t i = 0; i < c->waves.size(); ++i) {
		HWave &w = c->waves[i];
		if(!w.live || w.dw.type != A2AMD_WMIPWAVE)
			continue;
		const bool raw = force >= 0 ? force != 0 : (big && w.dw.size[0] >= 4096);
		const uint32_t f = (w.dw.flags & ~A2D_WF_RAWTAPS) | (raw ? A2D_WF_RAWTAPS : 0u);
		if(f != w.dw.flags) {
			w.dw.flags = f;
			c->mwaves[i].flags = f;
			c->waves_dirty = true;
		}
	}
}
}
// ... 65 lines not shown
		cap->d = c->capture.d;
		cap->n = c->capture.n;
		cap->device = c->cfg.device;
		c->capture.d = nullptr;
		c->capture.cap = 0;
		*out = cap;
	}
	c->capture.on = false;
	c->capture.n = 0;
	return A2AMD_OK;
}

unsigned a2amd_capture_frames(const a2amd_capture *cap) { return cap ? (unsigned)cap->n : 0; }

void a2amd_capture_free(a2amd_capture *cap)
{
	if(!cap)
		return;
	int dev = 0;
	hipGetDevice(&dev);
	hipSetDevice(cap->device);
	hipFree(cap->d);
	hipSetDevice(dev);
	delete cap;
}

int a2amd_wave_stats(a2amd_ctx *c, uint64_t *h2d, uint32_t *uploaded, uint32_t *resident)
{
	if(h2d) *h2d = c->wave_h2d_bytes;
	if(uploaded) *uploaded = c->waves_uploaded;
	if(resident) *resident = c->waves_resident;
	return A2AMD_OK;
}

static int wave_place(a2amd_ctx *c, uint64_t key, const a2amd_wavedesc *w, const a2amd_capture *cap, unsigned chunk = 0);

int a2amd_wave_upload(a2amd_ctx *c, uint64_t key, const a2amd_wavedesc *w)
{
	if(!w)
		return c->fail(A2AMD_EINVAL, "wave_upload: null descriptor");
	return wave_place(c, key, w, nullptr);
}

static int captured_refusals(a2amd_ctx *c, const a2amd_wavedesc *w, const a2amd_capture *cap)
{
	if(!w || !cap)
		return c->fail(A2AMD_EINVAL, "wave_upload_captured: null");
	if(cap->device != c->cfg.device)
		return c->fail(A2AMD_EUNSUPPORTED, "wave_upload_captured: the capture lives on GPU %d, the context on %d", cap->device, c->cfg.device);
	if(w->type != A2AMD_WWAVE && w->type != A2AMD_WMIPWAVE)
		return c->fail(A2AMD_EUNSUPPORTED, "wave_upload_captured: wave type %d", w->type);
	if((size_t)w->size[0] != cap->n)
		return c->fail(A2AMD_EUNSUPPORTED, "wave_upload_captured: the wave has %u samples, the capture %zu", w->size[0], cap->n);
	for(int l = 1; l < (w->type == A2AMD_WMIPWAVE ? A2D_MIPS : 1); ++l)
		if(w->size[l] != ((w->size[0] + (1u << l) - 1) >> l))
			return c->fail(A2AMD_EINVAL, "wave_upload_captured: level %d has %u samples", l, w->size[l]);
	return A2AMD_OK;
}

int a2amd_wave_upload_captured(a2amd_ctx *c, uint64_t key, const a2amd_wavedesc *w, const a2amd_capture *cap)
{
	if(w && cap && (w->flags & 0x000d0000u))
		return c->fail(A2AMD_EUNSUPPORTED, "wave_upload_captured: flags %#x ask for post-processing", w->flags);
	if(int r = captured_refusals(c, w, cap))
		return r;
	return wave_place(c, key, w, cap);
}

int a2amd_wave_upload_captured_post(a2amd_ctx *c, uint64_t key, const a2amd_wavedesc *w, const a2amd_capture *cap, unsigned chunk)
{
	if(int r = captured_refusals(c, w, cap))
		return r;
	if(w->flags & 0x00080000u)
		return c->fail(A2AMD_EUNSUPPORTED, "wave_upload_captured_post: A2_REVMIX (the reference's result is not defined)");
	if((w->flags & 0x00040000u) && w->size[0] < 2)
		return c->fail(A2AMD_EUNSUPPORTED, "wave_upload_captured_post: A2_XFADE on %u samples", w->size[0]);
	if((w->flags & 0x00010000u) && !chunk)
		return c->fail(A2AMD_EUNSUPPORTED, "wave_upload_captured_post: A2_NORMALIZE needs the size of the writes");
	use_device(c);
	if(int r = grow(c, c->d_wavepost, a2d_wavepost_scratch_words(w->size[0], w->flags, chunk), 1, false))
		return r;
	return wave_place(c, key, w, cap, chunk);
}

static int wave_place(a2amd_ctx *c, uint64_t key, const a2amd_wavedesc *w, const a2amd_capture *cap, unsigned chunk)
{
	use_device(c);
	int id = -1;
	for(size_t i = 0; i < c->waves.size(); ++i)
		if(c->waves[i].live && c->waves[i].key == key)
			id = (int)i;
	if(id < 0) {
		if(!c->free_wave_slots.empty()) {
			id = c->free_wave_slots.back();
			c->free_wave_slots.pop_back();
		} else {
			id = (int)c->waves.size();
			c->waves.push_back(HWave());
			c->mwaves.push_back(A2DWave());
		}
	} else {
		if(c->waves[id].pool_len)
			c->deferred_wavepool_free.push_back(std::make_pair(c->waves[id].pool_off, c->waves[id].pool_len));
		--c->stats.live_waves;
	}
	HWave &hw = c->waves[id];
	hw.live = true;
	hw.key = key;
	memset(&hw.dw, 0, sizeof(hw.dw));
	hw.dw.type = w->type;
	hw.dw.flags = w->flags;
	hw.dw.period = w->period;
	int levels = w->type == A2AMD_WMIPWAVE ? A2D_MIPS : w->type == A2AMD_WWAVE ? 1 : 0;
	size_t total = 0;
	for(int l = 0; l < levels; ++l)
		total += A2AMD_WAVEPRE + (size_t)w->size[l] + A2AMD_WAVEPOST;
	total = (total + 7) & ~(size_t)7;
	size_t pos = (size_t)-1;
	for(size_t k = 0; k < c->wavepool_free.size() && total; ++k)
		if(c->wavepool_free[k].second >= total) {
			pos = c->wavepool_free[k].first;
			c->wavepool_free[k].first += total;
			c->wavepool_free[k].second -= total;
			if(!c->wavepool_free[k].second)
				c->wavepool_free.erase(c->wavepool_free.begin() + (long)k);
			HIPCHK(c, hipStreamSynchronize(c->stream));
			break;
		}
	if(pos == (size_t)-1) {
		if(c->wavepool_used + total > c->d_wavepool.cap) {
			if((c->wavepool_used + total) * (4 * A2D_COEF_WORDS) > (((size_t)1 << 32) - 4096))
				return c->fail(A2AMD_ENOMEM, "wave pool beyond %zu samples", (((size_t)1 << 32) - 4096) / (4 * A2D_COEF_WORDS));
			if(int r = grow(c, c->d_wavepool, c->wavepool_used + total, 1, true)) return r;
			if(int r = grow(c, c->d_wavecoef, c->d_wavepool.cap, A2D_COEF_WORDS, false)) return r;
			if(c->wavepool_used > 3 && a2d_launch_build_coef(c->d_wavepool.d, c->d_wavecoef.d, 1,
					(unsigned)c->wavepool_used - 2, c->stream))
				return c->fail(A2AMD_EHIP, "coefficient build failed");
			c->waves_dirty = true;
			drop_graphs(c);
			c->blob_quiet = false;
		}
		pos = c->wavepool_used;
		c->wavepool_used += total;
	}
	hw.pool_off = pos;
	hw.pool_len = total;
	uint32_t loff[A2D_MIPS] = { 0 }, lsize[A2D_MIPS] = { 0 };
	const size_t pos0 = pos;
	for(int l = 0; l < levels; ++l) {
		size_t n = A2AMD_WAVEPRE + (size_t)w->size[l] + A2AMD_WAVEPOST;
		if(!cap) {
			HIPCHK(c, hipMemcpy(c->d_wavepool.d + pos, w->data[l], n * sizeof(int16_t), hipMemcpyHostToDevice));
			c->wave_h2d_bytes += n * sizeof(int16_t);
		}
		loff[l] = (uint32_t)(pos - pos0);
		lsize[l] = w->size[l];
		hw.dw.size[l] = w->size[l];
		hw.dw.off[l] = (uint32_t)(pos + A2AMD_WAVEPRE);
		pos += n;
	}
	if(cap) {
		int16_t *pool0 = c->d_wavepool.d + pos0;
		const int looped = (w->flags & 0x100u) != 0;
		if(levels && ((w->flags & 0x00050000u)
				? a2d_launch_wave_level0_post(cap->d, pool0 + A2AMD_WAVEPRE, lsize[0], w->flags, chunk, c->d_wavepost.d, c->stream) ||
					a2d_launch_wave_finish(pool0, loff, lsize, levels, looped, A2AMD_WAVEPRE, A2AMD_WAVEPOST, c->stream)
				: a2d_launch_wave_from_pcm(cap->d, pool0, loff, lsize, levels, looped, A2AMD_WAVEPRE, A2AMD_WAVEPOST, c->stream)))
			return c->fail(A2AMD_EHIP, "wave build from capture failed");
		++c->waves_resident;
	} else
		++c->waves_uploaded;
	if(total > 3 && a2d_launch_build_coef(c->d_wavepool.d, c->d_wavecoef.d, (unsigned)hw.pool_off + 1,
			(unsigned)(hw.pool_off + total) - 2, c->stream))
		return c->fail(A2AMD_EHIP, "coefficient build failed");
	c->mwaves[id] = hw.dw;
	c->waves_dirty = true;
	++c->stats.live_waves;
	wave_tap_policy(c);
	return id;
}

int a2amd_wave_drop(a2amd_ctx *c, uint64_t key)
{
	for(size_t i = 0; i < c->waves.size(); ++i)
		if(c->waves[i].live && c->waves[i].key == key) {
			c->waves[i].live = false;
			c->waves[i].dw.size[0] = 0;
			if(c->waves[i].pool_len)
				c->deferred_wavepool_free.push_back(std::make_pair(c->waves[i].pool_off, c->waves[i].pool_len));
			c->waves[i].pool_len = 0;
			c->waves[i].key = 0;
			c->deferred_wave_slots.push_back((int)i);
			if(!c->nfrags && !c->frag_open) {
				for(auto &r : c->deferred_wavepool_free)
					wavepool_release(c, r.first, r.second);
				c->deferred_wavepool_free.clear();
			}
			c->mwaves[i] = c->waves[i].dw;
			c->waves_dirty = true;
			--c->stats.live_waves;
			return A2AMD_OK;
		}
	return c->fail(A2AMD_EINVAL, "wave_drop: unknown key");
}

int a2amd_fragment(a2amd_ctx *c, unsigned frames)
{
	if(!frames || frames > A2D_FRAG)
		return c->fail(A2AMD_EINVAL, "fragment of %u frames", frames);
	if(!c->stack.empty())
		return c->fail(A2AMD_ESTATE, "fragment inside an inline window");
	if(c->uploaded)
		return c->fail(A2AMD_ESTATE, "batch already uploaded; finish the render first");
	close_fragment(c);
	if(c->nfrags >= (int)c->cfg.max_batch)
		return c->fail(A2AMD_ESTATE, "more than max_batch=%u fragments without a render", c->cfg.max_batch);
	if(!c->nfrags)
		c->vm.batch_time = c->walk_time;
	c->cur_frag = c->nfrags++;
	c->walk_serial = c->serial_base + c->cur_frag;
	c->fragframes[c->cur_frag] = frames;
	c->fragbase[c->cur_frag] = 0;
	c->frag_open = true;
	c->walked_started = 0;
	c->building = -1;
	if(c->defmap_dirty || c->defmap.size() < c->voices.size() + 4096) {
		if(c->defmap.size() < c->voices.size() + 4096)
			c->defmap.assign(c->voices.size() * 2 + 65536, 0);
		else
			std::fill(c->defmap.begin(), c->defmap.begin() + std::min(c->defmap.size(), c->voices.size()), 0);
		c->defmap_dirty = false;
	}
	c->defmap_used = false;
	return A2AMD_OK;
}

int a2amd_fragment_offset(a2amd_ctx *c, unsigned offset)
{
	if(!c->frag_open || c->uploaded)
		return c->fail(A2AMD_ESTATE, "fragment_offset outside a fragment");
	if(offset + c->fragframes[c->cur_frag] > A2D_FRAG)
		return c->fail(A2AMD_EINVAL, "fragment_offset %u with %u frames", offset, c->fragframes[c->cur_frag]);
	c->fragbase[c->cur_frag] = (uint8_t)offset;
	return A2AMD_OK;
}

namespace {
int sweep_stretch_check(a2amd_ctx *c, const char *who, unsigned frames, unsigned count)
{
	if(!frames || frames > A2D_FRAG)
		return c->fail(A2AMD_EINVAL, "fragment of %u frames", frames);
	if(!c->stack.empty())
		return c->fail(A2AMD_ESTATE, "fragment inside an inline window");
	if(c->uploaded)
		return c->fail(A2AMD_ESTATE, "batch already uploaded; finish the render first");
	if((uint64_t)c->nfrags + count > c->cfg.max_batch)
		return c->fail(A2AMD_ESTATE, "more than max_batch=%u fragments without a render", c->cfg.max_batch);
	for(int ui : c->sweeping) {
		const HUnit &u = c->units[ui];
		const HVoice &v = c->voices[u.voice];
		if(v.vm >= 0)
			continue;
		if(!c->frag_open && !v.recs.empty() && (int)A2D_RFRAG(v.recs.back().head) >= c->nfrags)
			return c->fail(A2AMD_ESTATE, "%s: a write to the voice of filter %d, whose cutoff is sweeping, since the last "
					"fragment was closed: walk a fragment by calls first", who, ui);
	}
	return 0;
}

void sweep_stretch(a2amd_ctx *c, unsigned frames, unsigned count)
{
	a2amd_ctx::CutStretch st = { c->nfrags, (int)count, frames, c->cut_list.size(), 0 };
	for(size_t i = c->sweeping.size(); i-- > 0;) {
		const int ui = c->sweeping[i];
		HUnit &u = c->units[ui];
		HVoice &v = c->voices[u.voice];
		if(v.vm >= 0)
			continue;
		if(u.cslot_batch != c->serial_base) {
			u.cslot_batch = c->serial_base;
			u.cslot = c->cut_slots++;
		}
		int32_t r[4] = { u.cutoff.value, u.cutoff.target, u.cutoff.delta, u.cutoff.timer };
		const A2DCutSweep e = { { r[0], r[1], r[2], r[3] }, ui, u.cslot, { 0, 0 } };
		c->cut_list.push_back(e);
		const bool was = u.cutoff.timer != 0;
		for(unsigned j = 0; j < count && a2cs_moving(r); ++j) {
			int32_t pitch;
			c->n_cut_windows += a2cs_step(r, (int)frames, &pitch);
		}
		u.cutoff.value = r[0];
		u.cutoff.target = r[1];
		u.cutoff.delta = r[2];
		u.cutoff.timer = r[3];
		c->n_cutoff_ramps += (int)(u.cutoff.timer != 0) - (int)was;
		if(!cutoff_moving(u))
			v.plain = 0;
		sweep_track(c, ui);
	}
	st.n = c->cut_list.size() - st.first;
	if(st.n)
		c->cut_st.push_back(st);
}
}

int a2amd_cutoff_sweep(int32_t ramper[4], unsigned frames, unsigned count, const uint32_t *ptab128, int samplerate,
// ... 1119 lines not shown
```

audiality2_amd/csrc/a2amd_render.cpp:

```cpp
#include "a2amd_host.h"

extern "C" {
static double now_us()
{
	timespec ts;
	clock_gettime(CLOCK_MONOTONIC, &ts);
	return ts.tv_sec * 1e6 + ts.tv_nsec * 1e-3;
}
static double g_t[4], g_n;
static double g_why[13];
static double g_cnt[6];
struct TimingDump { ~TimingDump() {
	A2Switches sw; a2amd_read_switches(&sw); if(sw.hosttiming && g_n) fprintf(stderr,
	"a2amd host timing per render: upload %.1f us, issue %.1f us, readback %.1f us (%g renders; %g quiet uploads, "
	"%g graph launches, %g records, %g voices with records, %g walk scans, %g R_NOPs)\n",
	g_t[0] / g_n, g_t[1] / g_n, g_t[2] / g_n, g_n, g_cnt[0], g_cnt[5], g_cnt[1], g_cnt[4], g_cnt[2], g_cnt[3]);
	if(sw.hosttiming && g_n) { fprintf(stderr, "a2amd uploads by first reason against the quiet path "
	"(blob, recs, prev recs, voices, udesc, waves, lists, ptab, dirty voices, fbd, nfrags, bus, none):");
	for(int k = 0; k < 13; ++k) fprintf(stderr, " %g", g_why[k]); fprintf(stderr, "\n"); } } } g_timing_dump;

}
namespace a2h { double *dbg_counters() { return g_cnt; } double *dbg_why() { return g_why; } }
extern "C" {

}
int a2h::fetch_taps(a2amd_ctx *c, bool final)
{
	bool any = false;
	for(size_t k = 0; k < c->xio.size(); ++k) {
		XioSlot &x = c->xio[k];
		if(x.unit >= 0 && x.tapped) {
			if(final)
				x.tapped = (c->units[x.unit].xio_mode & A2AMD_XIO_TAP) != 0;
			HIPCHK(c, hipMemcpyAsync(x.tap.data(), c->d_xio.d + k * A2D_XIO_SLOT,
					(size_t)c->nfrags * A2AMD_MAXCHANNELS * A2D_FRAG * sizeof(int32_t),
					hipMemcpyDeviceToHost, c->stream));
			any = true;
		}
	}
	if(any)
		HIPCHK(c, hipStreamSynchronize(c->stream));
	return 0;
}

extern "C" {
int a2amd_render(a2amd_ctx *c, unsigned phases, int32_t *const *out, unsigned cap)
{
	use_device(c);
	const bool timing = c->sw.hosttiming;
	double t0 = timing ? now_us() : 0;
	if(!c->stack.empty())
		return c->fail(A2AMD_ESTATE, "render inside an inline window");
	if((phases & A2AMD_RENDER_KEEP) && !c->noise_st.empty())
		return c->fail(A2AMD_EUNSUPPORTED, "A2AMD_RENDER_KEEP on a batch with device-seeded noise windows "
				"(a2amd_fragment_repeat_noise): a re-run would need a new generator word");
	if((phases & A2AMD_RENDER_KEEP) && !c->cut_st.empty())
		return c->fail(A2AMD_EUNSUPPORTED, "A2AMD_RENDER_KEEP on a batch with a cutoff sweep table "
				"(a2amd_fragment_repeat with a sweeping filter): a re-run would need the ramp to go on");
	close_fragment(c);
	unsigned total = 0;
	for(int f = 0; f < c->nfrags; ++f)
		total += c->fragframes[f];
	if(!c->nfrags) {
		if(!(phases & A2AMD_RENDER_KEEP))
			;
		return 0;
	}
	c->snap_valid = false;
	if(c->vm.unwalked >= 0)
		return c->fail(A2AMD_ESTATE, "voice %d is run by the device VM, but the host's walk left it out of a fragment "
				"(no default window reported, no call)", c->vm.unwalked);
	if(phases & A2AMD_RENDER_UPLOAD)
		if(int r = upload(c))
			return r;
	double t1 = timing ? now_us() : 0;
	if(timing)
		g_t[0] += t1 - t0;
	if((phases & (A2AMD_RENDER_SUBTREES | A2AMD_RENDER_ROOT)) && !c->uploaded)
		return c->fail(A2AMD_ESTATE, "render phases out of order: upload first");

	if((phases & A2AMD_RENDER_SUBTREES) && c->profiling) {
		if(c->ev_used + 3 > c->ev_pool.size())
			for(int i = 0; i < 3; ++i) {
				hipEvent_t e;
				HIPCHK(c, hipEventCreate(&e));
				c->ev_pool.push_back(e);
			}
		c->ev0 = c->ev_pool[c->ev_used];
		c->ev1 = c->ev_pool[c->ev_used + 1];
		c->ev2 = c->ev_pool[c->ev_used + 2];
		c->ev_used += 3;
	}
	c->master_dst = nullptr;
	c->master_direct = false;
	int gv = 0;
	{
		const unsigned both = A2AMD_RENDER_SUBTREES | A2AMD_RENDER_ROOT;
		bool taps = false;
		for(const XioSlot &x : c->xio)
			if(x.unit >= 0 && x.tapped)
				taps = true;
		if(!c->sw.no_direct && (phases & A2AMD_RENDER_READBACK) && (phases & both) == both && !(phases & A2AMD_RENDER_KEEP) &&
				!(phases & A2AMD_RENDER_TAPS) && !c->comm && !c->dist_local && c->uploaded &&
				(c->with_recs.empty() || c->last_buswin.fbd_dropped + c->last_buswin.fbdpan_voices) &&
				c->consume_ok && c->sub_resume < 0 && !c->paused_at && !taps) {
			const size_t n = (size_t)c->nfrags * c->cfg.channels * A2D_FRAG;
			if(phases & A2AMD_RENDER_ASYNC) {
				if(c->rb_count < 2) {
					const int ri = (c->rb_head + c->rb_count) & 1;
					a2amd_ctx::Readback &rb = c->rb[ri];
					if(n > rb.cap) {
						if(rb.h)
							HIPCHK(c, hipHostFree(rb.h));
						rb.h = nullptr;
						rb.cap = 0;
						HIPCHK(c, hipHostMalloc((void **)&rb.h, n * sizeof(int32_t), hipHostMallocDefault));
						rb.cap = n;
					}
					c->master_dst = rb.h;
					gv = 1 + ri;
				}
			} else if(out) {
				if(n > c->h_master_cap) {
					if(c->h_master)
						HIPCHK(c, hipHostFree(c->h_master));
					c->h_master = nullptr;
					c->h_master_cap = 0;
					HIPCHK(c, hipHostMalloc((void **)&c->h_master, n * sizeof(int32_t), hipHostMallocDefault));
					c->h_master_cap = n;
				}
				c->master_dst = c->h_master;
				gv = 1;
			}
		}
	}
	auto run_phases = [&](unsigned kphases) -> int {
		if(!kphases)
			return 0;
		if(c->uploaded && !c->profiling && c->stream && c->with_recs.empty() && !c->sw.no_graph &&
				c->vm.list.empty() &&
				!(phases & A2AMD_RENDER_TAPS) && c->sub_resume < 0 && !c->paused_at &&
				((phases & A2AMD_RENDER_KEEP) ? (phases & ~A2AMD_RENDER_KEEP) ==
				 (phases & (A2AMD_RENDER_SUBTREES | A2AMD_RENDER_ROOT)) :
				 c->quiet_streak >= 1 && c->nfrags >= 8)) {
			const int slot = kphases == A2AMD_RENDER_SUBTREES ? 2 : kphases == A2AMD_RENDER_ROOT ? 3 : 1;
			const int gi = slot + 4 * (slot == 2 ? 0 : gv);
			if((c->gexec[gi] && c->gdst[gi] == c->master_dst) || !build_graph(c, gi, 1, kphases)) {
				if(slot != 3)
					if(int r = ensure_clean(c))
						return r;
				HIPCHK(c, hipGraphLaunch(c->gexec[gi], c->stream));
				c->master_direct = c->gdirect[gi];
				c->last_bus.consume = c->gconsume[gi];
// ... 191 lines not shown
			drop_graphs(c);
			graphs = false;
		}
	}
	while(steps) {
		if(graphs && steps >= (unsigned)GRAPH_STEPS) {
			if(int r = ensure_clean(c))
				return r;
			HIPCHK(c, hipGraphLaunch(c->gexec[0], c->stream));
			c->others_clean = c->root_clean = c->consume_ok;
			steps -= GRAPH_STEPS;
			c->stats.fragments += (uint64_t)c->nfrags * GRAPH_STEPS;
			c->stats.voice_fragments += (uint64_t)c->nfrags * c->list_all.size() * GRAPH_STEPS;
		} else if(graphs) {
			if(int r = ensure_clean(c))
				return r;
			HIPCHK(c, hipGraphLaunch(c->gexec[1], c->stream));
			c->others_clean = c->root_clean = c->consume_ok;
			--steps;
			c->stats.fragments += c->nfrags;
			c->stats.voice_fragments += (uint64_t)c->nfrags * c->list_all.size();
		} else {
			if(c->profiling) {
				if(c->ev_used + 3 > c->ev_pool.size())
					for(int i = 0; i < 3; ++i) {
						hipEvent_t e;
						HIPCHK(c, hipEventCreate(&e));
						c->ev_pool.push_back(e);
					}
				c->ev0 = c->ev_pool[c->ev_used];
				c->ev1 = c->ev_pool[c->ev_used + 1];
				c->ev2 = c->ev_pool[c->ev_used + 2];
				c->ev_used += 3;
			}
			if(int r = c->profiling ?
					issue_kernels(c, A2AMD_RENDER_SUBTREES | A2AMD_RENDER_ROOT, c->ev0, c->ev1, c->ev2) :
					issue_kernels(c, A2AMD_RENDER_SUBTREES | A2AMD_RENDER_ROOT, nullptr, nullptr, nullptr))
				return r;
			--steps;
		}
	}
	return A2AMD_OK;
}

static int drain_events(a2amd_ctx *c)
{
	if(!c->ev_used)
		return 0;
	HIPCHK(c, hipStreamSynchronize(c->stream));
	for(size_t i = 0; i + 2 < c->ev_used + 0 && i + 2 < c->ev_pool.size(); i += 3) {
		float a = 0, b = 0;
		if(hipEventElapsedTime(&a, c->ev_pool[i], c->ev_pool[i + 1]) == hipSuccess &&
				hipEventElapsedTime(&b, c->ev_pool[i], c->ev_pool[i + 2]) == hipSuccess) {
			c->stats.timed_leaf_ms += a;
			c->stats.timed_all_ms += b;
			++c->stats.timed_batches;
		}
	}
	c->ev_used = 0;
	return 0;
}

int a2amd_get_stats(a2amd_ctx *c, a2amd_stats *st)
{
	if(c->profiling)
		if(int r = drain_events(c))
			return r;
	*st = c->stats;
	return A2AMD_OK;
}

int a2amd_last_batch(const a2amd_ctx *c, a2amd_batch_info *bi)
{
	if(!c || !bi)
		return A2AMD_EINVAL;
	*bi = c->last_batch;
	return A2AMD_OK;
}

int a2amd_last_batch_noise(const a2amd_ctx *c, a2amd_noise_batch_info *out)
{
	if(!c || !out)
		return A2AMD_EINVAL;
	*out = c->last_noise;
	return A2AMD_OK;
}

int a2amd_last_batch_noise_filter(const a2amd_ctx *c, a2amd_noise_filter_batch_info *out)
{
	if(!c || !out)
		return A2AMD_EINVAL;
	*out = c->last_noise_filter;
	out->min_voices = (uint32_t)c->sw.nzf_min;
	return A2AMD_OK;
}

int a2amd_last_batch_sweeps(const a2amd_ctx *c, a2amd_sweep_batch_info *out)
{
	if(!c || !out)
		return A2AMD_EINVAL;
	*out = c->last_sweeps;
	return A2AMD_OK;
}

int a2amd_last_batch_buses(const a2amd_ctx *c, a2amd_bus_info *out)
{
	if(!c || !out)
		return A2AMD_EINVAL;
	*out = c->last_bus;
	out->master_direct = c->master_direct;
	return A2AMD_OK;
}

int a2amd_last_batch_bare(const a2amd_ctx *c, a2amd_bare_batch_info *out)
{
	if(!c || !out)
		return A2AMD_EINVAL;
	*out = c->last_bare;
	return A2AMD_OK;
}

int a2amd_last_batch_osc2(const a2amd_ctx *c, a2amd_osc2_batch_info *out)
{
	if(!c || !out)
		return A2AMD_EINVAL;
	*out = c->last_osc2;
	if(!out->launched || c->blob_nfrags < 1 || c->blob_nfrags > A2D_MAXBATCH)
		return A2AMD_OK;
	unsigned start[A2D_MAXBATCH];
	for(int f = 0, acc = 0; f < c->blob_nfrags; ++f) {
		start[f] = (unsigned)acc;
		acc += (int)c->blob_frames[f];
	}
	unsigned n = 0;
	for(int slice = 0; slice < (int)out->ysplit; ++slice) {
		int c_lo, c_hi, nslices;
		if(!a2d_osc2_slice(c->blob_nfrags, (int)out->ysplit, slice, &c_lo, &c_hi, &nslices))
			break;
		for(int s_lo = c_lo; s_lo < c_hi; s_lo += A2D_OSC2_SCH / A2D_OSC2_FCH, ++n) {
			const int s_hi = std::min(c_hi, s_lo + A2D_OSC2_SCH / A2D_OSC2_FCH);
			const int fa = s_lo * A2D_OSC2_FCH, fb = std::min(c->blob_nfrags, s_hi * A2D_OSC2_FCH);
			if(out->voice_major && a2d_osc2_whole(start[fa], start[fb - 1], c->blob_frames[fb - 1], fb - fa))
				++out->superchunks_voice_major;
			else {
				++out->superchunks_chunk_major;
				if(n < 64)
					out->chunk_major_mask |= 1ull << n;
			}
		}
	}
	return A2AMD_OK;
}

int a2amd_last_batch_fbdpan(const a2amd_ctx *c, a2amd_fbdpan_batch_info *out)
{
	if(!c || !out)
		return A2AMD_EINVAL;
	*out = c->last_fbdpan;
	return A2AMD_OK;
}

int a2amd_last_batch_bus_windows(const a2amd_ctx *c, a2amd_bus_windows_info *out)
{
	if(!c || !out)
		return A2AMD_EINVAL;
	*out = c->last_buswin;
	out->window_cap = FBW_MAXWIN;
	return A2AMD_OK;
}

int a2amd_set_profiling(a2amd_ctx *c, int on)
{
	if(int r = drain_events(c))
		return r;
	if(on) {
		c->stats.timed_leaf_ms = c->stats.timed_all_ms = 0;
		c->stats.timed_batches = 0;
	}
	c->profiling = on != 0;
	return A2AMD_OK;
}

}
```

audiality2_amd/csrc/a2amd_sched.cpp:

```cpp
#include "a2amd_host.h"
#include "a2amd_cutsweep.h"
#include <functional>

namespace a2h {




void touch(a2amd_ctx *c, int vi)
{
	HVoice &v = c->voices[vi];
	const long long serial = c->serial_base + rec_tag(c);
	if(v.touched != serial) {
		v.touched = serial;
		v.frag_mark = v.recs.size();
	}
}



void spell_out_pending(a2amd_ctx *c, int vi)
{
	HVoice &dv = c->voices[vi];
	const bool marked = c->frag_open && c->defmap_used && (size_t)vi < c->defmap.size() && c->defmap[vi];
// ... 1370 lines not shown
				HIPCHK(c, hipStreamWaitEvent(c->stream, c->vm.spec_go, 0));
				c->vm.spec_go_pending = false;
			}
		}
		at = atw = 0;
		for(int j = 0; j < nj; ++j) {
			const Job &b = jobs[j];
			if(b.spec) {
				if(fa == 0 && a2d_launch_win_render(c->sw, c->hparams, b.nosc, b.filt, b.list, b.n, 0, nfrags, c->vm.d_swin[sset].d + b.satw,
						c->vm.d_swext[sset].d, c->vm.d_swidx[sset].d + b.sat, c->stream))
					return c->fail(A2AMD_EHIP, "window render launch failed: %s", hipGetErrorString(hipGetLastError()));
				if(fa == 0)
					++c->stats.launches;
				continue;
			}
			if(a2d_launch_win_render(c->sw, c->hparams, b.nosc, b.filt, b.list, b.n, fa, fb, wslot + atw,
					wext, widx + at, c->stream))
				return c->fail(A2AMD_EHIP, "window render launch failed: %s", hipGetErrorString(hipGetLastError()));
			at += (size_t)b.n * (size_t)(fb - fa);
			atw += (size_t)b.n * (size_t)(fb - fa) * A2D_WIN_SLOTWORDS(b.nosc, b.filt);
			++c->stats.launches;
		}
		if(two)
			HIPCHK(c, hipEventRecord(c->win_ev[2 + set], c->stream));
		if(wtiming && !two && !c->capturing) {
			float t_ctl = 0, t_ren = 0;
			HIPCHK(c, hipEventRecord(tev[2], c->stream));
			HIPCHK(c, hipEventSynchronize(tev[2]));
			hipEventElapsedTime(&t_ctl, tev[0], tev[1]);
			hipEventElapsedTime(&t_ren, tev[1], tev[2]);
			fprintf(stderr, "a2amd windows: fragments [%d, %d), %zu voices in %d list(s), %zu records: control pass %.1f us, render pass %.1f us\n",
					fa, fb, nvoices, nj, nrec, t_ctl * 1e3, t_ren * 1e3);
		}
	}
	if(!c->capturing && plain_jobs) {
		if(!c->h_wtop) {
			HIPCHK(c, hipHostMalloc((void **)&c->h_wtop, 4 * sizeof(unsigned), hipHostMallocDefault));
			memset(c->h_wtop, 0, 4 * sizeof(unsigned));
			HIPCHK(c, hipEventCreateWithFlags(&c->wtop_ev, hipEventDisableTiming));
		}
		HIPCHK(c, hipMemcpyAsync(c->h_wtop, c->d_wtop, 4 * sizeof(unsigned), hipMemcpyDeviceToHost, c->stream));
		HIPCHK(c, hipEventRecord(c->wtop_ev, c->stream));
		c->wtop_pending = true;
	}
	if(c->vm.fused && !c->vm.spec_use)
		if(int r = vm_fused_done(c))
			return r;
	if(c->sw.win_check && !c->capturing && plain_jobs) {
		unsigned top[4] = { 0, 0, 0, 0 };
		HIPCHK(c, hipMemcpyAsync(top, c->d_wtop, sizeof(top), hipMemcpyDeviceToHost, c->stream));
		HIPCHK(c, hipStreamSynchronize(c->stream));
		if(top[1] || (two && top[3])) {
			if(c->vm.fused)
				c->vm.fused_off = true;
			return c->fail(A2AMD_ESTATE, "window pool overflow (%u / %u of %zu entries)", top[0], top[2], c->d_wext.cap);
		}
	}
	return 0;
}

static void flush_commits(a2amd_ctx *c, A2DCommitSet *pend)
{
	for(int k = 0; k < pend->n; ++k)
		a2d_launch_commit(c->hparams, pend->c[k], c->stream);
	pend->n = 0;
}

static int launch_recs(a2amd_ctx *c, int nosc, int filt, const int *list, int n, int skip_empty)
{
	if(!n)
		return 0;
	const int vpw = c->sw.rvpw_set ? c->sw.rvpw : (n + 8191) / 8192;
	if(a2d_launch_leaf_recs(c->sw, c->d_params, c->hparams, nosc, filt, list, n, vpw, c->stream, skip_empty))
		return c->fail(A2AMD_EHIP, "leaf records launch failed: %s", hipGetErrorString(hipGetLastError()));
	++c->stats.launches;
	return 0;
}

static bool oscpan_alone(const a2amd_ctx *c)
{
	for(int k = 0; k < LEAF_N; ++k)
		if((c->leaf[k].count != 0) != (k == LEAF_OSCPAN))
			return false;
	return c->dyn[DYN_REST].first + c->dyn[DYN_REST].count == 0;
}

struct LeafPass {
	A2DCommitSet *pend;
	hipEvent_t e1;
	bool use_win;
	bool solo;
	bool done;
};

static int launch_leaves(a2amd_ctx *c, LeafPass &lp)
{
	if(lp.done)
		return 0;
	lp.done = true;
	A2DCommitSet &pend = *lp.pend;
	const int *const list = c->d_list.d;
	auto none_quiet = [&](int k, int nleaf) {
		return (c->sw.vmskip & (k == 2 ? 2 : 1)) && c->vm.spec_use && !c->vm.list.empty() && c->vm.n_cls[k] == nleaf && c->vm.spec_idle[k] == 0;
	};
	const ListRange oscpan = c->leaf[LEAF_OSCPAN];
	if(oscpan.count && none_quiet(0, oscpan.count)) {
		if(lp.solo && lp.e1)
			HIPCHK(c, hipEventRecord(lp.e1, c->stream));
		++c->vm.quiet_skipped;
	} else if(oscpan.count) {
		int vpw, ysplit;
		pick_fast_shape(c->sw, oscpan.count, c->nfrags, &vpw, &ysplit);
		if(a2d_launch_leaf_oscpan(c->d_params, c->hparams, list + oscpan.first, oscpan.count,
				vpw, ysplit, c->d_ustage.d, c->d_staged.d + oscpan.first, c->stream, lp.solo ? (void *)lp.e1 : nullptr,
				&pend.c[pend.n]))
			return c->fail(A2AMD_EHIP, "fast leaf launch failed: %s", hipGetErrorString(hipGetLastError()));
		if(pend.c[pend.n].nlist)
			++pend.n;
		++c->stats.launches;
		c->vm.last.quiet_launched[0] = 1;
	}
	const ListRange noisepan = c->leaf[LEAF_NOISEPAN];
	if(noisepan.count && !c->noise_st.empty() && c->n_noise_quiet) {
		const int vpw = c->sw.nzvpw_set ? c->sw.nzvpw : (noisepan.count + 1023) / 1024;
		if(a2d_launch_leaf_noisepan(c->d_params, c->hparams, list + noisepan.first, noisepan.count, vpw, c->stream))
			return c->fail(A2AMD_EHIP, "noise leaf launch failed: %s", hipGetErrorString(hipGetLastError()));
		++c->stats.launches;
		c->last_noise.quiet_launched = 1;
	}
	const ListRange noisefilt = c->leaf[LEAF_NOISEFILTPAN];
	if(noisefilt.count && !c->noise_st.empty() && c->n_noise_filt_quiet) {
		const int vpg = c->sw.nzfvpg_set ? c->sw.nzfvpg : (noisefilt.count + 255) / 256;
		if(a2d_launch_leaf_noisefiltpan(c->d_params, c->hparams, list + noisefilt.first, noisefilt.count, vpg, c->stream))
			return c->fail(A2AMD_EHIP, "noise filter leaf launch failed: %s", hipGetErrorString(hipGetLastError()));
		++c->stats.launches;
		c->last_noise_filter.quiet_launched = 1;
	}
	const ListRange bare = c->leaf[LEAF_OSCBARE];
	if(bare.count && c->n_bare_quiet) {
		const int vpw = std::min(std::max(c->sw.vpw_set ? c->sw.vpw : (bare.count + 1023) / 1024, 1), 64);
		if(a2d_launch_leaf_oscbare(c->d_params, c->hparams, list + bare.first, bare.count, vpw, c->stream))
			return c->fail(A2AMD_EHIP, "bare oscillator leaf launch failed: %s", hipGetErrorString(hipGetLastError()));
		++c->stats.launches;
		c->last_bare.launched = 1;
		c->last_bare.vpw = (uint32_t)vpw;
	}
	const ListRange osc2pan = c->leaf[LEAF_OSC2PAN];
	if(osc2pan.count && none_quiet(1, osc2pan.count))
		++c->vm.quiet_skipped;
	else if(osc2pan.count) {
		int vpw, ysplit;
		pick_fast_shape(c->sw, osc2pan.count, c->nfrags * A2D_FAST_FCH / A2D_OSC2_FCH, &vpw, &ysplit, 16);
		const int voice_major = !(c->sw.debug & 16);
		if(a2d_launch_leaf_osc2pan(c->d_params, c->hparams, list + osc2pan.first, osc2pan.count,
				vpw, ysplit, c->d_ustage.d, c->d_staged.d + osc2pan.first, c->stream, &pend.c[pend.n], voice_major, &ysplit))
			return c->fail(A2AMD_EHIP, "2-osc leaf launch failed: %s", hipGetErrorString(hipGetLastError()));
		c->last_osc2.launched = 1;
		c->last_osc2.voices = (uint32_t)osc2pan.count;
		c->last_osc2.vpw = (uint32_t)std::min(std::max(vpw, 1), 64);
		c->last_osc2.ysplit = (uint32_t)ysplit;
		c->last_osc2.voice_major = (uint32_t)voice_major;
		if(pend.c[pend.n].nlist)
			++pend.n;
		++c->stats.launches;
		c->vm.last.quiet_launched[1] = 1;
	}
	const ListRange oscfilt = c->leaf[LEAF_OSCFILTPAN];
	if(oscfilt.count && none_quiet(2, oscfilt.count))
		++c->vm.quiet_skipped;
	else if(oscfilt.count) {
		const int nf = oscfilt.count;
		int vpw = c->sw.fvpw_set ? c->sw.fvpw : std::min(std::max((nf + 255) / 256, 1), 64);
		if(a2d_launch_leaf_oscfiltpan(c->d_params, c->hparams, list + oscfilt.first, nf, vpw, c->stream))
			return c->fail(A2AMD_EHIP, "filter leaf launch failed: %s", hipGetErrorString(hipGetLastError()));
		++c->stats.launches;
		c->vm.last.quiet_launched[2] = 1;
	}
	const ListRange o2f = c->leaf[LEAF_OSC2FILTPAN];
	if(o2f.count && c->o2f_quiet) {
		const int nf = o2f.count;
		const int maxv = a2d_osc2filtpan_max_vpg();
		const int rounds = std::max(1, (nf + 256 * maxv - 1) / (256 * maxv));
		const int vpg = c->sw.f2vpw ? c->sw.f2vpw : std::min(std::max((nf + 256 * rounds - 1) / (256 * rounds), 1), maxv);
		if(a2d_launch_leaf_osc2filtpan(c->d_params, c->hparams, list + o2f.first, nf, vpg, c->stream))
			return c->fail(A2AMD_EHIP, "2-osc filter leaf launch failed: %s", hipGetErrorString(hipGetLastError()));
		++c->stats.launches;
		c->last_batch.o2f_launched = 1;
		c->last_batch.o2f_voices = (uint32_t)nf;
		c->last_batch.o2f_max_vpg = (uint32_t)maxv;
		c->last_batch.o2f_vpg = (uint32_t)std::min(std::max(vpg, 1), 64);
	}
	const ListRange fm = c->leaf[LEAF_FMPAN];
	int fm_kinds = 0;
	for(int k = 0; k < 8; ++k)
		fm_kinds += c->fm_kind_count[k] != 0;
	if(fm_kinds > 1 && fm.count <= 16384 && !c->sw.fmvpw_set) {
		if(a2d_launch_leaf_fmpan_all(c->d_params, c->hparams, list + fm.first, c->fm_kind_count, (fm.count + 1023) / 1024, c->stream))
			return c->fail(A2AMD_EHIP, "fm leaf launch failed: %s", hipGetErrorString(hipGetLastError()));
		++c->stats.launches;
	} else {
		for(int k = 0, at = fm.first; k < 8; at += c->fm_kind_count[k++]) {
			const int n = c->fm_kind_count[k];
			if(!n)
				continue;
			int vpw = c->sw.fmvpw_set ? c->sw.fmvpw : (n + 1023) / 1024;
			vpw = std::min(std::max(vpw, 1), 64);
			if(a2d_launch_leaf_fmpan(c->d_params, c->hparams, A2AMD_FM1 + k, list + at, n, vpw, c->stream))
				return c->fail(A2AMD_EHIP, "fm leaf launch failed: %s", hipGetErrorString(hipGetLastError()));
			++c->stats.launches;
		}
	}
	const ListRange gen = c->leaf[LEAF_GENERIC];
	if(gen.count) {
		if(a2d_launch_voices(c->d_params, list + gen.first, gen.count, pick_vpw(gen.count), c->stream))
			return c->fail(A2AMD_EHIP, "leaf launch failed: %s", hipGetErrorString(hipGetLastError()));
		++c->stats.launches;
	}
	if(!lp.use_win) {
		static const int nosc[4] = { 1, 2, 1, 2 }, filt[4] = { 0, 0, 1, 1 };
		const int *lists[4];
		int counts[4], total = 0, kinds = 0;
		for(int k = 0; k < 4; ++k) {
			lists[k] = c->d_dyn + c->dyn[k].first;
			counts[k] = c->dyn[k].count;
			total += counts[k];
			kinds += counts[k] != 0;
		}
		c->last_batch.recs_voices = (uint32_t)total;
		if(!c->vm.list.empty())
			c->last_batch.recs_voices += (uint32_t)(c->vm.n_cls[0] + c->vm.n_cls[1] + c->vm.n_cls[2]);
		if(kinds > 1 && total <= 4096 && !c->sw.rvpw_set) {
			if(a2d_launch_leaf_recs_all(c->sw, c->d_params, c->hparams, lists, counts, 1, c->stream, c->o2f_quiet ? 8 : 0))
				return c->fail(A2AMD_EHIP, "leaf records launch failed: %s", hipGetErrorString(hipGetLastError()));
			++c->stats.launches;
		} else {
			for(int k = 0; k < 4; ++k)
				if(int r = launch_recs(c, nosc[k], filt[k], lists[k], counts[k], k == DYN_FILT2 && c->o2f_quiet))
					return r;
		}
		if(!c->vm.list.empty()) {
			const int *l = c->vm.d_list.d + c->vm.list.size();
			for(int k = 0; k < 3; l += c->vm.n_cls[k++])
				if(int r = launch_recs(c, nosc[k], filt[k], l, c->vm.n_cls[k], 1))
					return r;
		}
	}
	const ListRange rest = c->dyn[DYN_REST];
	if(rest.count > 0) {
		if(a2d_launch_voices(c->d_params, c->d_dyn + rest.first, rest.count, pick_vpw(rest.count), c->stream))
			return c->fail(A2AMD_EHIP, "leaf launch failed: %s", hipGetErrorString(hipGetLastError()));
		++c->stats.launches;
	}
	return 0;
}

static int issue_leaf_phase(a2amd_ctx *c, bool consume, bool consume_sub, hipEvent_t e0, hipEvent_t e1, A2DCommitSet *pend)
{
	const bool selfclean = consume || consume_sub;
	if(c->capturing ? !selfclean : !(selfclean && c->others_clean && c->root_clean))
		HIPCHK(c, hipMemsetAsync(c->d_busmem.d, 0, c->bus_used * sizeof(int32_t), c->stream));
	c->others_clean = selfclean;
	c->root_clean = consume;
	if(e0)
		HIPCHK(c, hipEventRecord(e0, c->stream));
	bool use_win;
	{
		int nwinv = 0;
		for(int k = DYN_OSC1; k <= DYN_FILT2; ++k)
			nwinv += c->dyn[k].count;
		for(int k = 0; k < 3; ++k)
			nwinv += c->vm.list.empty() ? 0 : c->vm.n_cls[k];
		use_win = c->sw.win >= 0 ? c->sw.win != 0 : nwinv >= c->sw.win_min;
	}
	const bool vmwin_ok = c->sw.vmwin;
	if(int r = vm_issue(c, use_win && vmwin_ok && !c->vm.fused_off))
		return r;
	c->last_batch = a2amd_batch_info{};
	c->last_batch.o2f_class = (uint32_t)c->leaf[LEAF_OSC2FILTPAN].count;
	c->last_batch.o2f_listed = (uint32_t)c->dyn[DYN_FILT2].count;
	c->last_batch.n_moving_listed = (uint32_t)c->n_moving_listed;
	c->last_batch.general_voices = (uint32_t)c->dyn[DYN_REST].count;
	c->last_noise = a2amd_noise_batch_info{};
	c->last_noise.class_voices = (uint32_t)c->leaf[LEAF_NOISEPAN].count;
	c->last_noise.standin_voices = c->n_noise_standin;
	c->last_noise.quiet_voices = c->n_noise_quiet;
	c->last_noise_filter = a2amd_noise_filter_batch_info{};
	c->last_noise_filter.class_voices = (uint32_t)c->leaf[LEAF_NOISEFILTPAN].count;
	c->last_noise_filter.quiet_voices = c->n_noise_filt_quiet;
	c->last_noise_filter.min_voices = (uint32_t)c->sw.nzf_min;
	c->last_bare = a2amd_bare_batch_info{};
	c->last_bare.class_voices = (uint32_t)c->leaf[LEAF_OSCBARE].count;
	c->last_bare.quiet_voices = c->n_bare_quiet;
	c->last_bare.gliding_voices = c->n_bare_gliding;
	c->last_bare.record_voices = c->n_bare_records;
	c->last_bare.mono_drivers = c->n_mono_drivers;
	c->last_osc2 = a2amd_osc2_batch_info{};
	LeafPass lp = { pend, e1, use_win, oscpan_alone(c), false };
	const std::function<int()> mid = [&]() -> int {
		if(!c->sw.vmspec_early || !vmwin_ok || !vm_spec_wanted(c))
			return 0;
		if(int r = launch_leaves(c, lp))
			return r;
		flush_commits(c, pend);
		return vm_speculate(c);
	};
	if(use_win) {
		if(int r = issue_windows(c, c->d_dyn, c->dyn, mid))
			return r;
// ... 124 lines not shown
```

audiality2_amd/csrc/a2amd_taps.h:

```cpp
#pragma once
#include <hip/hip_runtime.h>
#include <stdint.h>
#include "a2amd_device.h"
#include "a2amd_dsp.h"
#include "a2amd_fm.h"

#define FAST_WPB   4
#define FAST_FCH   A2D_FAST_FCH

#define WRL(reg, val) reg = me ? (val) : reg

DEV int hermite_step(int v, unsigned ph)
{
	int p;
	asm("v_mul_i32_i24_sdwa %0, %1, %2 dst_sel:DWORD dst_unused:UNUSED_PAD src0_sel:DWORD src1_sel:BYTE_0"
			: "=v"(p) : "v"(v), "v"(ph));
	return __builtin_amdgcn_sbfe(p, 8, 17);
}

DEV int hermite4(int dm, int d0, int d1, int d2, unsigned ph)
{
	int c = (d1 - dm) >> 1;
	int a = (3 * (d0 - d1) + d2 - dm) >> 1;
	int b = dm - d0 + c - a;
	a = hermite_step(a, ph);
	a = hermite_step(a + b, ph);
	return d0 + hermite_step(a + c, ph);
}

struct __attribute__((packed, aligned(2))) Quad16 { uint32_t lo, hi; };

DEV int inter_quads(const Quad16 qa, const Quad16 qb, unsigned ph, unsigned ph2)
{
	int h0 = hermite4((int16_t)(qa.lo & 0xffff), (int)qa.lo >> 16, (int16_t)(qa.hi & 0xffff), (int)qa.hi >> 16, ph);
	int h1 = hermite4((int16_t)(qb.lo & 0xffff), (int)qb.lo >> 16, (int16_t)(qb.hi & 0xffff), (int)qb.hi >> 16, ph2);
	return h0 + h1;
}

DEV int inter_dwords(const int16_t *d, unsigned ph, unsigned dph16)
{
	const unsigned ph2 = ph + (dph16 >> 1);
	const Quad16 qa = *(const Quad16 *)(d + (int)(ph >> 8) - 1);
	const Quad16 qb = *(const Quad16 *)(d + (int)(ph2 >> 8) - 1);
	return inter_quads(qa, qb, ph, ph2);
}

typedef int Coef4 __attribute__((ext_vector_type(3)));
#define A2D_COEF_LOAD "llvm.amdgcn.struct.buffer.load.v3i32"
typedef int CoefRsrc __attribute__((ext_vector_type(4)));
extern "C" __device__ Coef4 a2d_coef_load(CoefRsrc rsrc, int vindex, int voffset, int soffset, int aux)
		__asm(A2D_COEF_LOAD);

DEV CoefRsrc coef_rsrc(const int *wavecoef)
{
	const uint64_t b = (uint64_t)wavecoef;
	CoefRsrc r;
	r.x = rfl((int)(unsigned)b);
	r.y = rfl((int)(((unsigned)(b >> 32) & 0xffffu) | ((4u * A2D_COEF_WORDS) << 16)));
	r.z = -1;
	r.w = 0x00020000;
	return r;
}

DEV int coef_base(unsigned doff) { return (int)(doff * (4u * A2D_COEF_WORDS)); }

DEV int hermite_ct(const Coef4 k, unsigned ph)
{
	int t = hermite_step(k.x, ph);
	t = hermite_step(wadd(t, k.y), ph);
	return hermite_step(wadd(t, k.z >> 16), ph);
}

DEV int inter_coefs(const Coef4 ka, unsigned pa, const Coef4 kb, unsigned pb)
{
	int d;
	asm("v_add_u32_sdwa %0, sext(%1), sext(%2) dst_sel:DWORD dst_unused:UNUSED_PAD src0_sel:WORD_0 src1_sel:WORD_0"
			: "=v"(d) : "v"(ka.z), "v"(kb.z));
	return wadd(wadd(d, hermite_ct(ka, pa)), hermite_ct(kb, pb));
}

DEV int frac_x(unsigned ph)
{
	int x;
	const int seven = 7;
	asm("v_lshlrev_b32_sdwa %0, %1, %2 dst_sel:DWORD dst_unused:UNUSED_PAD src0_sel:DWORD src1_sel:BYTE_0"
			: "=v"(x) : "v"(seven), "v"(ph));
	return x;
}

DEV int hermite_cx(const Coef4 k, unsigned ph)
{
	const int x = frac_x(ph);
	int t = wmul(k.x, x) >> 15;
	t = wmul(wadd(t, k.y), x) >> 15;
	t = wmul(wadd(t, k.z >> 16), x) >> 15;
	return wadd((int)(int16_t)(k.z & 0xffff), t);
}

DEV int inter_coefs_x(const Coef4 ka, unsigned pa, const Coef4 kb, unsigned pb)
{
	return hermite_cx(ka, pa) + hermite_cx(kb, pb);
}

DEV Coef4 coef_at(const CoefRsrc rs, int cb, unsigned ph)
{
	return a2d_coef_load(rs, (int)(ph >> 8), 0, cb, 0);
}

DEV unsigned tap_phase(uint64_t ph, unsigned ldph)
{
	const unsigned lo = (unsigned)ph & 0xffffu, hi = (unsigned)(ph >> 16);
	return hi + ((lo + ldph) >> 16);
}

DEV unsigned lane_dph(int lane, unsigned dph)
{
	unsigned t = (unsigned)lane * dph;
	asm("" : "+v"(t));
	return t;
}

DEV int64_t div_trunc_exact(int64_t n, int d)
{
	int64_t q = (int64_t)((double)n / (double)d);
	const int64_t r = n - q * d;
	if(n >= 0) {
		if(r < 0) --q; else if(r >= d) ++q;
	} else {
		if(r > 0) ++q; else if(r <= -(int64_t)d) --q;
	}
	return q;
}


template<int N>
DEV void flush_acc(int *busmem, int off, int nch, int f0, int nf, int lane, int dbg,
		int (&acc0)[N], int (&acc1)[N])
{
#pragma unroll
	for(int j = 0; j < N; ++j) {
		if(j < nf && off >= 0 && !(dbg & 1)) {
			int *dst = busmem + off + (size_t)(f0 + j) * nch * A2D_FRAG;
			if(acc0[j])
				atomicAdd(&dst[lane], acc0[j]);
			if(acc1[j])
				atomicAdd(&dst[A2D_FRAG + lane], acc1[j]);
		}
		acc0[j] = 0;
		acc1[j] = 0;
	}
}

DEV void tile_add(int *w, int x)
{
	(void)__hip_atomic_fetch_add(w, x, __ATOMIC_RELAXED, __HIP_MEMORY_SCOPE_WAVEFRONT);
}

DEV void flush_tile(int *busmem, int off, int nch, int f0, int nf, int nrows, int lane, int dbg, int (*tile)[2][A2D_FRAG])
{
	for(int r = 0; r < nrows; ++r) {
		const int a0 = tile[r][0][lane], a1 = tile[r][1][lane];
		tile[r][0][lane] = 0;
		tile[r][1][lane] = 0;
		if(r < nf && off >= 0 && !(dbg & 1)) {
			int *dst = busmem + off + (size_t)(f0 + r) * nch * A2D_FRAG;
			if(a0)
				atomicAdd(&dst[lane], a0);
			if(a1)
				atomicAdd(&dst[A2D_FRAG + lane], a1);
		}
	}
}
```

audiality2_amd/replay.py:

```python
import ctypes as C
import gzip
import lzma

import numpy as np

T_FRAGMENT, T_INIT, T_DEINIT, T_WRITE, T_PROCESS, T_INLINE_END, T_WAVE, T_CONFIG, T_WAVEDROP = range(1, 10)
MIPLEVELS = 10
WAVEPRE = 1
WAVEPOST = 131


class Trace:

    def __init__(self, path):
        opener = gzip.open if str(path).endswith(".gz") else lzma.open if str(path).endswith(".xz") else open
        with opener(path, "rb") as f:
            raw = f.read()
        words = np.frombuffer(raw[: len(raw) // 4 * 4], dtype="<i4")
        self.records = []
        self.waves = {}
        self.config = None
        i = 0
        n = len(words)
        while i + 8 <= n:
# ... 30 lines not shown

class a2amd_config(C.Structure):
    _fields_ = [("struct_size", C.c_uint32), ("samplerate", C.c_int32),
                ("basepitch", C.c_int32), ("channels", C.c_int32),
                ("device", C.c_int32), ("max_batch", C.c_uint32),
                ("stream", C.c_void_p)]


class a2amd_wavedesc(C.Structure):
    _fields_ = [("type", C.c_int32), ("flags", C.c_uint32), ("period", C.c_uint32),
                ("size", C.c_uint32 * MIPLEVELS),
                ("data", C.POINTER(C.c_int16) * MIPLEVELS)]


class a2amd_noise_batch_info(C.Structure):
    _fields_ = [("quiet_launched", C.c_uint32), ("quiet_voices", C.c_uint32),
                ("class_voices", C.c_uint32), ("standin_voices", C.c_uint32)]

    def __repr__(self):
        return "noise_batch_info(" + ", ".join(f"{n}={getattr(self, n)}" for n, _ in self._fields_) + ")"


class a2amd_noise_filter_batch_info(C.Structure):
    _fields_ = [("quiet_launched", C.c_uint32), ("quiet_voices", C.c_uint32),
                ("class_voices", C.c_uint32), ("min_voices", C.c_uint32)]

    def __repr__(self):
        return "noise_filter_batch_info(" + ", ".join(f"{n}={getattr(self, n)}" for n, _ in self._fields_) + ")"


class a2amd_sweep_batch_info(C.Structure):
    _fields_ = [("pass_launched", C.c_uint32), ("filters", C.c_uint32),
                ("ramp_windows", C.c_uint32), ("standin_voices", C.c_uint32)]

    def __repr__(self):
        return "sweep_batch_info(" + ", ".join(f"{n}={getattr(self, n)}" for n, _ in self._fields_) + ")"


class a2amd_bus_info(C.Structure):
    _fields_ = [(n, C.c_uint32) for n in ("driver_voices", "driver_ramping", "driver_windows_dropped", "fbd_voices",
                                          "generic_voices", "consume", "master_direct")]

    def __repr__(self):
        return "bus_info(" + ", ".join(f"{n}={getattr(self, n)}" for n, _ in self._fields_) + ")"


class a2amd_bare_batch_info(C.Structure):
    _fields_ = [(n, C.c_uint32) for n in ("launched", "class_voices", "quiet_voices", "gliding_voices", "record_voices",
                                          "vpw", "mono_drivers", "reserved")]

    def __repr__(self):
        return "bare_batch_info(" + ", ".join(f"{n}={getattr(self, n)}" for n, _ in self._fields_) + ")"


class a2amd_osc2_batch_info(C.Structure):
    _fields_ = [(n, C.c_uint32) for n in ("launched", "voices", "vpw", "ysplit", "voice_major", "superchunks_voice_major",
                                          "superchunks_chunk_major", "reserved")] + [("chunk_major_mask", C.c_uint64)]

    def __repr__(self):
        return "osc2_batch_info(" + ", ".join(f"{n}={getattr(self, n)}" for n, _ in self._fields_) + ")"


class a2amd_fbdpan_batch_info(C.Structure):
    _fields_ = [(n, C.c_uint32) for n in ("launched", "class_voices", "quiet_voices", "gliding_voices", "record_voices",
                                          "max_delays")] + [("reserved", C.c_uint32 * 2)]

    def __repr__(self):
        return "fbdpan_batch_info(" + ", ".join(f"{n}={getattr(self, n)}" for n, _ in self._fields_[:-1]) + ")"


class a2amd_bus_windows_info(C.Structure):
    _fields_ = [(n, C.c_uint32) for n in ("fbd_dropped", "fbdpan_voices", "fbdpan_gliding", "fbdpan_windows", "refused_tiling",
                                          "refused_cap", "window_cap", "launched")]

    def __repr__(self):
        return "bus_windows_info(" + ", ".join(f"{n}={getattr(self, n)}" for n, _ in self._fields_) + ")"


class a2amd_vm_batch_info(C.Structure):
    _fields_ = [("listed", C.c_uint32), ("class_voices", C.c_uint32 * 3), ("other_voices", C.c_uint32),
                ("pending", C.c_uint32), ("fused", C.c_uint32), ("not_fused", C.c_uint32),
                ("spec_valid", C.c_uint32), ("spec_taken", C.c_uint32), ("spec_miss", C.c_uint32),
                ("spec_next", C.c_uint32), ("spec_why_not", C.c_uint32), ("records", C.c_uint32),
                ("idle_known", C.c_uint32), ("idle", C.c_uint32 * 3), ("quiet_launched", C.c_uint32 * 3)]

    def __repr__(self):
        return ("vm_batch_info(" + ", ".join(f"{n}={list(getattr(self, n)) if n in ('class_voices', 'idle', 'quiet_launched') else getattr(self, n)}"
                                             for n, _ in self._fields_) + ")")


class a2amd_vm_state(C.Structure):
    _fields_ = [("waketime", C.c_uint32), ("state", C.c_uint8), ("func", C.c_uint8), ("pc", C.c_uint16),
                ("r", C.c_int32 * 64)]


class Backend:

    def __init__(self, lib, prefix, samplerate, basepitch, channels=2, device=0,
                 max_batch=64, stream=None):
        self.lib, self.prefix, self.channels = lib, prefix, channels

        def fn(name, restype, *argtypes):
            f = getattr(lib, prefix + name)
            f.restype, f.argtypes = restype, list(argtypes)
            return f

        vp, i32, u32, u64 = C.c_void_p, C.c_int, C.c_uint, C.c_uint64
        self._open = fn("open", i32, C.POINTER(a2amd_config), C.POINTER(vp))
        self._close = fn("close", None, vp)
        self._err = fn("last_error", C.c_char_p, vp)
        self._wave_upload = fn("wave_upload", i32, vp, u64, C.POINTER(a2amd_wavedesc))
        self._wave_drop = fn("wave_drop", i32, vp, u64)
        self._fragment = fn("fragment", i32, vp, u32)
        self._unit_init = fn("unit_init", i32, vp, u64, i32, u32, i32, i32, i32, i32, u32)
        self._unit_deinit = fn("unit_deinit", i32, vp, i32)
        self._unit_write = fn("unit_write", i32, vp, i32, i32, i32, u32, u32, i32)
        self._unit_process = fn("unit_process", i32, vp, i32, u32, u32, C.POINTER(C.c_uint32))
        self._inline_end = fn("inline_end", i32, vp, i32)
        self._unit_clients = fn("unit_clients", i32, vp, i32, u32)
        self._unit_inject = fn("unit_inject", i32, vp, i32, u32, u32, C.POINTER(C.POINTER(C.c_int32)))
        self._unit_tapped = fn("unit_tapped", i32, vp, i32, u32, C.POINTER(C.POINTER(C.c_int32)))
        self._render = fn("render", i32, vp, u32, C.POINTER(C.POINTER(C.c_int32)), u32)
        self._set_pt = fn("set_pitch_table", i32, vp, C.POINTER(C.c_uint32))
        self._get_pt = fn("get_pitch_table", i32, vp, C.POINTER(C.c_uint32))
        self.has_walk = hasattr(lib, prefix + "voice_process")
        if self.has_walk:
            self._voice_process = fn("voice_process", i32, vp, i32, u32, u32, C.POINTER(C.c_uint32))
            self._voice_slot = fn("voice_slot", i32, vp, i32)
            self._default_map = fn("default_map", C.POINTER(C.c_uint8), vp, C.POINTER(u32))
        self._fragment_repeat_noise = None
        if hasattr(lib, prefix + "fragment_repeat_noise"):
            self._fragment_repeat_noise = fn("fragment_repeat_noise", i32, vp, u32, u32, C.POINTER(C.c_uint32))
        self._last_batch_noise = None
        if hasattr(lib, prefix + "last_batch_noise"):
            self._last_batch_noise = fn("last_batch_noise", i32, vp, C.POINTER(a2amd_noise_batch_info))
        self._last_batch_noise_filter = None
        if hasattr(lib, prefix + "last_batch_noise_filter"):
            self._last_batch_noise_filter = fn("last_batch_noise_filter", i32, vp, C.POINTER(a2amd_noise_filter_batch_info))
        self._fragment_repeat = None
        if hasattr(lib, prefix + "fragment_repeat"):
            self._fragment_repeat = fn("fragment_repeat", i32, vp, u32, u32)
        self._last_batch_sweeps = None
        if hasattr(lib, prefix + "last_batch_sweeps"):
            self._last_batch_sweeps = fn("last_batch_sweeps", i32, vp, C.POINTER(a2amd_sweep_batch_info))
        self._last_batch_buses = None
        if hasattr(lib, prefix + "last_batch_buses"):
            self._last_batch_buses = fn("last_batch_buses", i32, vp, C.POINTER(a2amd_bus_info))
        self._last_batch_bare = None
        if hasattr(lib, prefix + "last_batch_bare"):
            self._last_batch_bare = fn("last_batch_bare", i32, vp, C.POINTER(a2amd_bare_batch_info))
        self._last_batch_osc2 = None
        if hasattr(lib, prefix + "last_batch_osc2"):
            self._last_batch_osc2 = fn("last_batch_osc2", i32, vp, C.POINTER(a2amd_osc2_batch_info))
        self._last_batch_fbdpan = None
        if hasattr(lib, prefix + "last_batch_fbdpan"):
            self._last_batch_fbdpan = fn("last_batch_fbdpan", i32, vp, C.POINTER(a2amd_fbdpan_batch_info))
        self._last_batch_bus_windows = None
        if hasattr(lib, prefix + "last_batch_bus_windows"):
            self._last_batch_bus_windows = fn("last_batch_bus_windows", i32, vp, C.POINTER(a2amd_bus_windows_info))
        self.has_vm = hasattr(lib, prefix + "vm_adopt")
        if self.has_vm:
            self._fragment_offset = fn("fragment_offset", i32, vp, u32)
            self._vm_program = fn("vm_program", i32, vp, u64, C.POINTER(C.c_uint32), u32)
            self._vm_adopt = fn("vm_adopt", i32, vp, i32, i32, C.POINTER(a2amd_vm_state), C.POINTER(C.c_int32),
                                C.POINTER(C.c_uint8), C.c_uint32, C.c_uint32, vp, i32)
            self._vm_expect_cuts = fn("vm_expect_cuts", i32, vp, C.POINTER(C.c_uint32), i32)
            self._vm_recall = fn("vm_recall", i32, vp, C.POINTER(C.c_int32), u32, C.POINTER(a2amd_vm_state), vp)
        self._last_batch_vm = None
        if hasattr(lib, prefix + "last_batch_vm"):
            self._last_batch_vm = fn("last_batch_vm", i32, vp, C.POINTER(a2amd_vm_batch_info))
        self.has_capture = hasattr(lib, prefix + "wave_upload_captured_post")
        if self.has_capture:
            self._capture_begin = fn("capture_begin", i32, vp)
            self._capture_end = fn("capture_end", i32, vp, C.POINTER(vp))
            self._capture_frames = fn("capture_frames", u32, vp)
            self._capture_free = fn("capture_free", None, vp)
            self._wave_upload_captured = fn("wave_upload_captured", i32, vp, u64, C.POINTER(a2amd_wavedesc), vp)
            self._wave_upload_captured_post = fn("wave_upload_captured_post", i32, vp, u64, C.POINTER(a2amd_wavedesc), vp, u32)
            self._wave_stats = fn("wave_stats", i32, vp, C.POINTER(u64), C.POINTER(u32), C.POINTER(u32))
        cfg = a2amd_config(C.sizeof(a2amd_config), samplerate, basepitch, channels,
                           device, max_batch, stream)
        self.ctx = vp()
        rc = self._open(C.byref(cfg), C.byref(self.ctx))
        if rc != 0:
            raise RuntimeError(f"{prefix}open failed: {rc} "
                               f"{self._err(None).decode(errors='replace')}")
        self.noise = C.c_uint32(0)
        self._keep = []

    def close(self):
        if self.ctx:
            self._close(self.ctx)
            self.ctx = None

    def _chk(self, rc, what):
        if rc < 0:
            msg = self._err(self.ctx)
            raise RuntimeError(f"{self.prefix}{what}: {rc} {msg.decode(errors='replace') if msg else ''}")
        return rc

    def wave_upload(self, key, wtype, flags, period, sizes, data):
        d = a2amd_wavedesc()
        d.type, d.flags, d.period = wtype, flags, period
        for lv, arr in enumerate(data):
            arr = np.ascontiguousarray(arr, dtype=np.int16)
            self._keep.append(arr)
            d.size[lv] = sizes[lv]
            d.data[lv] = arr.ctypes.data_as(C.POINTER(C.c_int16))
        return self._chk(self._wave_upload(self.ctx, key, C.byref(d)), "wave_upload")

    def capture_begin(self):
        return self._chk(self._capture_begin(self.ctx), "capture_begin")

    def capture_end(self):
        cap = C.c_void_p()
        self._chk(self._capture_end(self.ctx, C.byref(cap)), "capture_end")
        return cap if cap.value else None

    def capture_frames(self, cap):
        return self._capture_frames(cap)

    def capture_free(self, cap):
        self._capture_free(cap)

    def wave_upload_captured(self, key, wtype, flags, period, sizes, cap, chunk=None, check=True):
        d = a2amd_wavedesc()
        d.type, d.flags, d.period = wtype, flags, period
        for lv, n in enumerate(sizes):
            d.size[lv] = n
        if chunk is None:
            rc = self._wave_upload_captured(self.ctx, key, C.byref(d), cap)
        else:
            rc = self._wave_upload_captured_post(self.ctx, key, C.byref(d), cap, chunk)
        return self._chk(rc, "wave_upload_captured") if check else rc

    def wave_stats(self):
        h2d, up, res = C.c_uint64(), C.c_uint32(), C.c_uint32()
        self._chk(self._wave_stats(self.ctx, C.byref(h2d), C.byref(up), C.byref(res)), "wave_stats")
        return h2d.value, up.value, res.value

    def wave_drop(self, key):
        return self._chk(self._wave_drop(self.ctx, key), "wave_drop")

    def fragment(self, frames):
        return self._chk(self._fragment(self.ctx, frames), "fragment")

    def fragment_repeat(self, frames, count):
        if self._fragment_repeat is None:
            raise RuntimeError(f"this library has no {self.prefix}fragment_repeat")
        return self._chk(self._fragment_repeat(self.ctx, frames, count), "fragment_repeat")

    def last_batch_sweeps(self):
        if self._last_batch_sweeps is None:
            raise RuntimeError(f"this library has no {self.prefix}last_batch_sweeps")
        bi = a2amd_sweep_batch_info()
        self._chk(self._last_batch_sweeps(self.ctx, C.byref(bi)), "last_batch_sweeps")
        return bi

    def fragment_repeat_noise(self, frames, count):
        if self._fragment_repeat_noise is None:
            raise RuntimeError(f"this library has no {self.prefix}fragment_repeat_noise")
        return self._chk(self._fragment_repeat_noise(self.ctx, frames, count, C.byref(self.noise)),
                         "fragment_repeat_noise")

    def last_batch_noise(self):
        if self._last_batch_noise is None:
            raise RuntimeError(f"this library has no {self.prefix}last_batch_noise")
        bi = a2amd_noise_batch_info()
        self._chk(self._last_batch_noise(self.ctx, C.byref(bi)), "last_batch_noise")
        return bi

    def last_batch_noise_filter(self):
        if self._last_batch_noise_filter is None:
            raise RuntimeError(f"this library has no {self.prefix}last_batch_noise_filter")
        bi = a2amd_noise_filter_batch_info()
        self._chk(self._last_batch_noise_filter(self.ctx, C.byref(bi)), "last_batch_noise_filter")
        return bi

    def last_batch_buses(self):
        if self._last_batch_buses is None:
            raise RuntimeError(f"this library has no {self.prefix}last_batch_buses")
        bi = a2amd_bus_info()
        self._chk(self._last_batch_buses(self.ctx, C.byref(bi)), "last_batch_buses")
        return bi

    def last_batch_bare(self):
        if self._last_batch_bare is None:
            raise RuntimeError(f"this library has no {self.prefix}last_batch_bare")
        bi = a2amd_bare_batch_info()
        self._chk(self._last_batch_bare(self.ctx, C.byref(bi)), "last_batch_bare")
        return bi

    def last_batch_osc2(self):
        if self._last_batch_osc2 is None:
            raise RuntimeError(f"this library has no {self.prefix}last_batch_osc2")
        bi = a2amd_osc2_batch_info()
        self._chk(self._last_batch_osc2(self.ctx, C.byref(bi)), "last_batch_osc2")
        return bi

    def last_batch_fbdpan(self):
        if self._last_batch_fbdpan is None:
            raise RuntimeError(f"this library has no {self.prefix}last_batch_fbdpan")
        bi = a2amd_fbdpan_batch_info()
        self._chk(self._last_batch_fbdpan(self.ctx, C.byref(bi)), "last_batch_fbdpan")
        return bi

    def last_batch_bus_windows(self):
        if self._last_batch_bus_windows is None:
            raise RuntimeError(f"this library has no {self.prefix}last_batch_bus_windows")
        bi = a2amd_bus_windows_info()
        self._chk(self._last_batch_bus_windows(self.ctx, C.byref(bi)), "last_batch_bus_windows")
        return bi

    def last_batch_vm(self):
        if self._last_batch_vm is None:
            raise RuntimeError(f"this library has no {self.prefix}last_batch_vm")
        bi = a2amd_vm_batch_info()
        self._chk(self._last_batch_vm(self.ctx, C.byref(bi)), "last_batch_vm")
        return bi

    def fragment_offset(self, offset):
        return self._chk(self._fragment_offset(self.ctx, offset), "fragment_offset")

    def vm_program(self, key, words):
        code = (C.c_uint32 * len(words))(*[w & 0xffffffff for w in words])
        return self._chk(self._vm_program(self.ctx, key, code, len(words)), "vm_program")

    def vm_adopt(self, head_unit, prog, state, wires, now, msdur, check=True):
        wu = (C.c_int32 * 64)(*([-1] * 64))
        wr = (C.c_uint8 * 64)()
        for r, (u, ureg) in wires.items():
            wu[r], wr[r] = u, ureg
        rc = self._vm_adopt(self.ctx, head_unit, prog, C.byref(state), wu, wr, now & 0xffffffff, msdur, None, 0)
        return self._chk(rc, "vm_adopt") if check else rc

    def vm_expect_cuts(self, when):
        arr = (C.c_uint32 * max(len(when), 1))(*[w & 0xffffffff for w in when])
        return self._chk(self._vm_expect_cuts(self.ctx, arr, len(when)), "vm_expect_cuts")

    def vm_recall(self, head_units):
        n = len(head_units)
        out = (a2amd_vm_state * n)()
        self._chk(self._vm_recall(self.ctx, (C.c_int32 * n)(*head_units), n, out, None), "vm_recall")
        return list(out)

    def last_error(self):
        msg = self._err(self.ctx)
        return msg.decode(errors="replace") if msg else ""

    def unit_init(self, voice_key, kind, flags, nin, nout, wired, transpose=0, wakefrac=0):
        return self._chk(self._unit_init(self.ctx, voice_key, kind, flags, nin, nout, wired,
                                         transpose, wakefrac), "unit_init")

    def unit_deinit(self, unit):
        return self._chk(self._unit_deinit(self.ctx, unit), "unit_deinit")

    def unit_write(self, unit, reg, value, start=0, dur=0, transpose=0):
        return self._chk(self._unit_write(self.ctx, unit, reg, value, start, dur, transpose),
                         "unit_write")

    def unit_process(self, unit, offset, frames, use_noise=True):
        return self._chk(self._unit_process(self.ctx, unit, offset, frames,
                                            C.byref(self.noise) if use_noise else None),
                         "unit_process")

    def voice_process(self, units, offset, frames):
        if self.has_walk:
            return self._chk(self._voice_process(self.ctx, units[0], offset, frames, C.byref(self.noise)),
                             "voice_process")
        for u in units:
            self.unit_process(u, offset, frames)
        return 0

    def mark_default(self, units):
        n = C.c_uint(0)
        m = self._default_map(self.ctx, C.byref(n))
        slot = self._chk(self._voice_slot(self.ctx, units[0]), "voice_slot")
        assert m and slot < n.value
        m[slot] = 1

    def inline_end(self, unit):
        return self._chk(self._inline_end(self.ctx, unit), "inline_end")

    def unit_clients(self, unit, mode):
        return self._chk(self._unit_clients(self.ctx, unit, mode), "unit_clients")

    def unit_inject(self, unit, offset, audio):
        audio = np.ascontiguousarray(audio, dtype=np.int32)
        ptrs = (C.POINTER(C.c_int32) * audio.shape[0])()
        for c in range(audio.shape[0]):
            ptrs[c] = audio[c].ctypes.data_as(C.POINTER(C.c_int32))
        return self._chk(self._unit_inject(self.ctx, unit, offset, audio.shape[1], ptrs), "unit_inject")

    def unit_tapped(self, unit, fragment):
        ptrs = (C.POINTER(C.c_int32) * 8)()
        n = self._chk(self._unit_tapped(self.ctx, unit, fragment, ptrs), "unit_tapped")
        return np.stack([np.ctypeslib.as_array(ptrs[c], shape=(64,)).copy() for c in range(n)])

    def render(self, capacity_frames, phases=15):
        out = np.zeros((self.channels, max(capacity_frames, 1)), dtype=np.int32)
        ptrs = (C.POINTER(C.c_int32) * self.channels)()
        for c in range(self.channels):
            ptrs[c] = out[c].ctypes.data_as(C.POINTER(C.c_int32))
        n = self._chk(self._render(self.ctx, phases, ptrs, capacity_frames), "render")
        return out[:, :n]

    def set_pitch_table(self, tab):
        tab = np.ascontiguousarray(tab, dtype=np.uint32)
        return self._chk(self._set_pt(self.ctx, tab.ctypes.data_as(C.POINTER(C.c_uint32))), "set_pt")

    def get_pitch_table(self):
        tab = np.zeros(128, dtype=np.uint32)
        self._chk(self._get_pt(self.ctx, tab.ctypes.data_as(C.POINTER(C.c_uint32))), "get_pt")
        return tab


def replay(trace, backend, batch=64, check_noise=True, max_fragments=None):
    umap, wmap = {}, {}
    outs = []
    nfrag = 0
    pending = 0
    backend.noise.value = trace.config["noiseseed"]
    for r in trace.records:
        op = r[0]
        if op == T_FRAGMENT:
            if max_fragments is not None and nfrag >= max_fragments:
                break
            if pending and nfrag % batch == 0:
                outs.append(backend.render(pending))
                pending = 0
            backend.fragment(r[1])
            pending += r[1]
            nfrag += 1
        elif op == T_WAVE:
            w = trace.waves[r[1]]
            wmap[r[1]] = backend.wave_upload(0x1000 + r[1], w["type"], w["flags"], w["period"],
                                             w["sizes"], w["data"])
        elif op == T_WAVEDROP:
            if pending:
                outs.append(backend.render(pending))
                pending = 0
            backend.wave_drop(0x1000 + r[1])
            wmap.pop(r[1], None)
        elif op == T_INIT:
            _, uid, voice, kind, flags, io, transpose, wakefrac = r
            umap[uid] = backend.unit_init(voice, kind, flags & 0xFFFFFFFF, io & 0xFF,
                                          (io >> 8) & 0xFF, (io >> 16) & 1, transpose, wakefrac)
        elif op == T_DEINIT:
            backend.unit_deinit(umap.pop(r[1]))
        elif op == T_WRITE:
            _, uid, reg, value, start, dur, transpose, _g = r
# ... 30 lines not shown
```

include/a2amd.h:

```cpp
#ifndef A2AMD_H
#define A2AMD_H

#include <stdint.h>

#ifdef __cplusplus
extern "C" {
#endif

#define A2AMD_MAXFRAG      64
#define A2AMD_MAXCHANNELS   8
#define A2AMD_MIPLEVELS    10
#define A2AMD_WAVEPRE       1
#define A2AMD_WAVEPOST    131
#define A2AMD_MAXCHAIN     16

typedef struct a2amd_ctx a2amd_ctx;

typedef enum a2amd_errors {
	A2AMD_OK = 0,
	A2AMD_ENODEVICE   = -1,
	A2AMD_EINVAL      = -2,
	A2AMD_ENOMEM      = -3,
	A2AMD_EUNSUPPORTED= -4,
	A2AMD_ESTATE      = -5,
// ... 25 lines not shown
} a2amd_unitkind;

#define A2AMD_PROCADD 0x00000001u

#define A2AMD_WOFF     0
#define A2AMD_WNOISE   1
#define A2AMD_WWAVE    2
#define A2AMD_WMIPWAVE 3
#define A2AMD_LOOPED   0x00000100u

typedef struct a2amd_config {
	uint32_t struct_size;
	int32_t  samplerate;
	int32_t  basepitch;
	int32_t  channels;
	int32_t  device;
	uint32_t max_batch;
	void    *stream;
} a2amd_config;

typedef struct a2amd_wavedesc {
	int32_t  type;
	uint32_t flags;
	uint32_t period;
	uint32_t size[A2AMD_MIPLEVELS];
	const int16_t *data[A2AMD_MIPLEVELS];
} a2amd_wavedesc;

int  a2amd_open(const a2amd_config *cfg, a2amd_ctx **out);
void a2amd_close(a2amd_ctx *ctx);
const char *a2amd_last_error(const a2amd_ctx *ctx);
const char *a2amd_version(void);
const char *a2amd_source_stamp(void);
int  a2amd_device_count(void);

int  a2amd_set_pitch_table(a2amd_ctx *ctx, const uint32_t *tab128);
int  a2amd_get_pitch_table(const a2amd_ctx *ctx, uint32_t *tab128);

int  a2amd_wave_upload(a2amd_ctx *ctx, uint64_t key, const a2amd_wavedesc *w);
int  a2amd_wave_drop(a2amd_ctx *ctx, uint64_t key);

typedef struct a2amd_capture a2amd_capture;
int  a2amd_capture_begin(a2amd_ctx *ctx);
int  a2amd_capture_end(a2amd_ctx *ctx, a2amd_capture **cap);
unsigned a2amd_capture_frames(const a2amd_capture *cap);
void a2amd_capture_free(a2amd_capture *cap);
int  a2amd_wave_upload_captured(a2amd_ctx *ctx, uint64_t key, const a2amd_wavedesc *w, const a2amd_capture *cap);
int  a2amd_wave_stats(a2amd_ctx *ctx, uint64_t *h2d_bytes, uint32_t *uploaded, uint32_t *resident);

int  a2amd_fragment(a2amd_ctx *ctx, unsigned frames);
int  a2amd_fragment_offset(a2amd_ctx *ctx, unsigned offset);

int  a2amd_unit_init(a2amd_ctx *ctx, uint64_t voice_key, int kind,
		unsigned flags, int ninputs, int noutputs, int wired_out,
		int transpose, unsigned wakefrac);
int  a2amd_unit_deinit(a2amd_ctx *ctx, int unit);

int  a2amd_unit_write(a2amd_ctx *ctx, int unit, int reg, int value,
		unsigned start, unsigned duration, int transpose);

int  a2amd_unit_process(a2amd_ctx *ctx, int unit, unsigned offset,
		unsigned frames, uint32_t *noisestate);
int  a2amd_voice_process(a2amd_ctx *ctx, int head_unit, unsigned offset, unsigned frames,
		uint32_t *noisestate);
int  a2amd_voice_slot(a2amd_ctx *ctx, int unit);
int  a2amd_voice_markable(a2amd_ctx *ctx, int unit);
int  a2amd_default_hold(a2amd_ctx *ctx, const uint32_t *slots, unsigned n, unsigned lo, int on);
int  a2amd_default_release_all(a2amd_ctx *ctx);
uint8_t *a2amd_default_map(a2amd_ctx *ctx, unsigned *nslots);

#define A2AMD_XIO_TAP     1u
#define A2AMD_XIO_INJECT  2u
#define A2AMD_XIO_MUTE    4u
int  a2amd_unit_clients(a2amd_ctx *ctx, int unit, unsigned mode);
int  a2amd_unit_insertable(a2amd_ctx *ctx, int unit);
int  a2amd_render_paused(a2amd_ctx *ctx);
int  a2amd_unit_insert(a2amd_ctx *ctx, int unit, unsigned fragment, unsigned offset, unsigned frames,
		const int32_t *const *bufs);
int  a2amd_unit_inject(a2amd_ctx *ctx, int unit, unsigned offset, unsigned frames,
		const int32_t *const *bufs);
int  a2amd_unit_tapped(a2amd_ctx *ctx, int unit, unsigned fragment, const int32_t **bufs);

int  a2amd_inline_end(a2amd_ctx *ctx, int unit);

#define A2AMD_RENDER_SUBTREES 1u
#define A2AMD_RENDER_ROOT     2u
#define A2AMD_RENDER_UPLOAD   4u
#define A2AMD_RENDER_READBACK 8u
#define A2AMD_RENDER_TAPS     64u
#define A2AMD_RENDER_KEEP    16u
#define A2AMD_RENDER_ASYNC   32u
#define A2AMD_RENDER_EXCHANGE 128u
#define A2AMD_RENDER_ALL     15u
int  a2amd_render(a2amd_ctx *ctx, unsigned phases, int32_t *const *out,
		unsigned out_capacity_frames);
int  a2amd_collect(a2amd_ctx *ctx, int32_t *const *out, unsigned out_capacity_frames);
int  a2amd_replay(a2amd_ctx *ctx, unsigned steps);
int  a2amd_rootbus(a2amd_ctx *ctx, void **devptr, uint64_t *bytes);
int  a2amd_rootbus_copy(a2amd_ctx *ctx, void *stage, int to_stage);

int  a2amd_dist_unique_id(void *id128);
int  a2amd_dist_init(a2amd_ctx *ctx, const void *id128, int rank, int nranks);
int  a2amd_dist_init_local(a2amd_ctx *const *ctxs, int n);
int  a2amd_render_group(a2amd_ctx *const *ctxs, int n, unsigned phases, int32_t *const *out,
		unsigned out_capacity_frames);

int  a2amd_fragment_repeat(a2amd_ctx *ctx, unsigned frames, unsigned count);


typedef struct a2amd_stats {
	uint64_t fragments;
	uint64_t voice_fragments;
	uint64_t records;
	uint64_t launches;
	double   last_kernel_ms;
	double   last_leaf_ms;
	uint32_t live_units, live_voices, live_waves, reserved;
	double   timed_leaf_ms;
	double   timed_all_ms;
	uint64_t timed_batches;
} a2amd_stats;
int  a2amd_get_stats(a2amd_ctx *ctx, a2amd_stats *st);
int  a2amd_set_profiling(a2amd_ctx *ctx, int on);
typedef struct a2amd_batch_info {
	uint32_t o2f_launched;
	uint32_t o2f_voices;
	uint32_t o2f_vpg;
	uint32_t o2f_max_vpg;
	uint32_t o2f_class;
	uint32_t o2f_listed;
	uint32_t recs_voices;
	uint32_t win_voices;
	uint32_t win_slabs;
	uint32_t n_moving_listed;
	uint32_t general_voices;
} a2amd_batch_info;
int  a2amd_last_batch(const a2amd_ctx *ctx, a2amd_batch_info *bi);

#ifdef __cplusplus
}
#endif

#include "a2amd_noise.h"
#include "a2amd_noisepan.h"
#include "a2amd_noisefilt.h"
#include "a2amd_sweep.h"
#include "a2amd_bus.h"
#include "a2amd_wavepost.h"
#include "a2amd_oscbare.h"
#include "a2amd_fbdpan.h"
#include "a2amd_buswin.h"
#include "a2amd_vmbatch.h"
#include "a2amd_osc2.h"

#endif
```

Before: 525.4 billion voice-samples/s.

## Stage small periodic wavetable mip levels in LDS for 2-osc pan leaf taps

When a voice's selected mip level is periodic, a power of two and small enough, the osc2pan leaf kernel copies that level's interpolation coefficients into per-wave LDS. Tap lookups then read LDS with a masked index instead of issuing global buffer loads. Periodicity is detected on the host at wave upload by checking the pad samples, and is stored in the former pad field of the wave descriptor. This adds per-voice staging copies, wave fences, a larger shared-memory footprint that may lower occupancy, and template variants.

```diff
diff --git a/audiality2_amd/build.py b/audiality2_amd/build.py
--- a/audiality2_amd/build.py
+++ b/audiality2_amd/build.py
@@ -58,9 +58,9 @@
     srcs = [os.path.join(csrc, f) for f in ("a2amd_host.cpp", "a2amd_sched.cpp", "a2amd_render.cpp", "a2amd_dist.cpp",
                                             "a2amd_vm.cpp", "a2amd_kernels.hip", "a2amd_fast.hip", "a2amd_vm.hip", "a2amd_wavecap.hip", "a2amd_wavepost.hip", "a2amd_win.hip", "a2amd_vmwin.hip", "a2amd_noise.hip", "a2amd_noisepan.hip", "a2amd_noisefiltpan.hip", "a2amd_cutsweep.hip", "a2amd_oscbare.hip")]
     deps = srcs + [os.path.join(csrc, "a2amd_host.h"), os.path.join(csrc, "a2amd_switches.h"), os.path.join(csrc, "a2amd_device.h"), os.path.join(csrc, "a2amd_dsp.h"),
-                   os.path.join(csrc, "a2amd_fm.h"), os.path.join(csrc, "a2amd_vmcore.h"), os.path.join(csrc, "a2amd_taps.h"), os.path.join(csrc, "a2amd_winctl.h"), os.path.join(csrc, "a2amd_vmdev.h"), os.path.join(csrc, "a2amd_noisemap.h"), os.path.join(csrc, "a2amd_noisevoice.h"), os.path.join(csrc, "a2amd_settled.h"), os.path.join(csrc, "a2amd_cutsweep.h"), os.path.join(csrc, "a2amd_filt.h"), os.path.join(ROOT, "include", "a2amd.h"),
+                   os.path.join(csrc, "a2amd_fm.h"), os.path.join(csrc, "a2amd_vmcore.h"), os.path.join(csrc, "a2amd_taps.h"), os.path.join(csrc, "a2amd_winctl.h"), os.path.join(csrc, "a2amd_vmdev.h"), os.path.join(csrc, "a2amd_noisemap.h"), os.path.join(csrc, "a2amd_noisevoice.h"), os.path.join(csrc, "a2amd_settled.h"), os.path.join(csrc, "a2amd_cutsweep.h"), os.path.join(csrc, "a2amd_filt.h"), os.path.join(csrc, "a2amd_wavepads.h"), os.path.join(ROOT, "include", "a2amd.h"),
                    os.path.join(ROOT, "include", "a2amd_noise.h"), os.path.join(ROOT, "include", "a2amd_noisepan.h"), os.path.join(ROOT, "include", "a2amd_noisefilt.h"), os.path.join(ROOT, "include", "a2amd_sweep.h"), os.path.join(ROOT, "include", "a2amd_wavepost.h"),
-                   os.path.join(ROOT, "include", "a2amd_bus.h"), os.path.join(ROOT, "include", "a2amd_oscbare.h"), os.path.join(ROOT, "include", "a2amd_fbdpan.h"), os.path.join(ROOT, "include", "a2amd_buswin.h"), os.path.join(ROOT, "include", "a2amd_vmbatch.h"), os.path.join(ROOT, "include", "a2amd_osc2.h"), os.path.join(ROOT, "include", "a2amd_vm.h")]
+                   os.path.join(ROOT, "include", "a2amd_bus.h"), os.path.join(ROOT, "include", "a2amd_oscbare.h"), os.path.join(ROOT, "include", "a2amd_fbdpan.h"), os.path.join(ROOT, "include", "a2amd_buswin.h"), os.path.join(ROOT, "include", "a2amd_vmbatch.h"), os.path.join(ROOT, "include", "a2amd_osc2.h"), os.path.join(ROOT, "include", "a2amd_osc2lds.h"), os.path.join(ROOT, "include", "a2amd_vm.h")]
     out = os.path.join(HERE, "liba2amd.so")
     flags = ["--offload-arch=gfx950", "-O3", "-std=c++17", "-fPIC", "-shared", "-Wno-unused-value"]
     want = source_hash(deps, flags)
@@ -73,7 +73,7 @@
     src = os.path.join(HERE, "csrc", "a2amd_units.c")
     deps = [src, os.path.join(ROOT, "include", "a2amd.h"), os.path.join(ROOT, "include", "a2amd_noise.h"), os.path.join(ROOT, "include", "a2amd_noisepan.h"),
             os.path.join(ROOT, "include", "a2amd_noisefilt.h"), os.path.join(ROOT, "include", "a2amd_sweep.h"), os.path.join(ROOT, "include", "a2amd_bus.h"),
-            os.path.join(ROOT, "include", "a2amd_wavepost.h"), os.path.join(ROOT, "include", "a2amd_oscbare.h"), os.path.join(ROOT, "include", "a2amd_fbdpan.h"), os.path.join(ROOT, "include", "a2amd_buswin.h"), os.path.join(ROOT, "include", "a2amd_vmbatch.h"), os.path.join(ROOT, "include", "a2amd_osc2.h"), os.path.join(ROOT, "include", "a2amd_plugin.h"),
+            os.path.join(ROOT, "include", "a2amd_wavepost.h"), os.path.join(ROOT, "include", "a2amd_oscbare.h"), os.path.join(ROOT, "include", "a2amd_fbdpan.h"), os.path.join(ROOT, "include", "a2amd_buswin.h"), os.path.join(ROOT, "include", "a2amd_vmbatch.h"), os.path.join(ROOT, "include", "a2amd_osc2.h"), os.path.join(ROOT, "include", "a2amd_osc2lds.h"), os.path.join(ROOT, "include", "a2amd_plugin.h"),
             os.path.join(ROOT, "include", "a2amd_walk.h"), os.path.join(ROOT, "include", "a2amd_vm.h")]
     out = os.path.join(HERE, "liba2amd_units.so")
     flags = ["-O2", "-Wall", "-fPIC", "-shared"]
diff --git a/audiality2_amd/csrc/a2amd_device.h b/audiality2_amd/csrc/a2amd_device.h
--- a/audiality2_amd/csrc/a2amd_device.h
+++ b/audiality2_amd/csrc/a2amd_device.h
@@ -64,7 +64,7 @@
 	uint32_t period;
 	uint32_t size[A2D_MIPS];
 	uint32_t off[A2D_MIPS];
-	uint32_t pad;
+	uint32_t periodic;
 };
 
 struct A2DVoice {
@@ -160,6 +160,7 @@
 #define A2D_FAST_FCH 8
 #define A2D_OSC2_FCH 4
 #define A2D_OSC2_SCH 16
+#define A2D_OSC2_LDS_ENT 128
 #define A2D_MAXVPW   32
 
 struct A2DParams {
@@ -209,6 +210,13 @@
 A2D_HD bool a2d_osc2_whole(unsigned start_first, unsigned start_last, unsigned frames_last, int n)
 {
 	return start_last + frames_last - start_first == (unsigned)n * A2D_FRAG;
+}
+
+A2D_HD unsigned a2d_osc2_stage(unsigned size0, unsigned periodic0, unsigned size1, unsigned periodic1)
+{
+	const bool c0 = periodic0 && size0 && !(size0 & (size0 - 1)) && size0 <= A2D_OSC2_LDS_ENT;
+	const bool c1 = periodic1 && size1 && !(size1 & (size1 - 1)) && size1 <= A2D_OSC2_LDS_ENT;
+	return (c0 ? 1u : 0u) | (c1 && (c0 ? size0 : 0u) + size1 <= A2D_OSC2_LDS_ENT ? 2u : 0u);
 }
 
 #ifdef __HIPCC__
@@ -314,7 +322,8 @@
 		int vpw, void *stream);
 int a2d_launch_scatter_runs(const int *didx, const A2DRun *dval, int n, A2DRun *druns, void *stream);
 int a2d_launch_leaf_osc2pan(const A2DParams *dparams, const A2DParams &hp, const int *dlist, int nlist,
-		int vpw, int ysplit, int *ustage, unsigned char *staged, void *stream, A2DCommit *defer, int voice_major, int *ysplit_used);
+		int vpw, int ysplit, int *ustage, unsigned char *staged, void *stream, A2DCommit *defer, int voice_major, int lds_taps,
+		int *ysplit_used);
 struct A2Switches;
 int a2d_launch_leaf_recs(const A2Switches &sw, const A2DParams *dparams, const A2DParams &hp, int nosc, int filt, const int *dlist,
 		int nlist, int vpw, void *stream, int skip_empty = 0);
diff --git a/audiality2_amd/csrc/a2amd_fast.hip b/audiality2_amd/csrc/a2amd_fast.hip
--- a/audiality2_amd/csrc/a2amd_fast.hip
+++ b/audiality2_amd/csrc/a2amd_fast.hip
@@ -251,7 +251,7 @@
 
 enum { DV_SETTLED = 0, DV_MM, DV_DPH, DV_SIZEM, DV_DOFF, DV_V0, DV_V1, DV_NWORDS };
 
-DEV bool settled_wave(const A2DWave *w, unsigned dphase, int *d, bool settled = true)
+DEV bool settled_wave(const A2DWave *w, unsigned dphase, int *d, bool settled = true, unsigned *periodic = nullptr)
 {
 	unsigned dph;
 	const unsigned mm = a2s_mip(dphase, w->period, &dph);
@@ -259,6 +259,8 @@
 	d[1] = (int)dph;
 	d[2] = (int)w->size[mm];
 	d[3] = (int)w->off[mm];
+	if(periodic)
+		*periodic = (w->periodic >> mm) & 1u;
 	return settled && a2s_wave_ok(w->size[0], w->flags, dph);
 }
 
@@ -613,10 +615,14 @@
 	int cb[2], amp[2];
 	uint64_t ph[2], end[2];
 };
-
-template<bool WHOLE>
+struct Osc2Lds {
+	const LdsInt *level[2];
+	unsigned lg[2];
+};
+
+template<bool WHOLE, int ST = 0>
 DEV void osc2_chunk(const CoefRsrc &crs, Osc2Voice &s, const unsigned (&ldph)[2], const int (&nfr)[OSC2_FCH],
-		const unsigned (&pre)[OSC2_FCH], int nf, bool park, int (&xs)[OSC2_FCH])
+		const unsigned (&pre)[OSC2_FCH], int nf, bool park, int (&xs)[OSC2_FCH], const Osc2Lds &lv = Osc2Lds())
 {
 	Coef4 ka[2][OSC2_FCH], kb[2][OSC2_FCH];
 	unsigned pa[2][OSC2_FCH], pb[2][OSC2_FCH];
@@ -644,8 +650,13 @@
 			pa[o][j] = tap_phase(phs[j], ldph[o]);
 			asm("" : "+v"(pa[o][j]));
 			pb[o][j] = pa[o][j] + (dph >> 17);
-			ka[o][j] = coef_at(crs, s.cb[o], pa[o][j]);
-			kb[o][j] = coef_at(crs, s.cb[o], pb[o][j]);
+			if((ST >> o) & 1) {
+				ka[o][j] = coef_lds(lv.level[o], pa[o][j], lv.lg[o]);
+				kb[o][j] = coef_lds(lv.level[o], pb[o][j], lv.lg[o]);
+			} else {
+				ka[o][j] = coef_at(crs, s.cb[o], pa[o][j]);
+				kb[o][j] = coef_at(crs, s.cb[o], pb[o][j]);
+			}
 		}
 		if(park) {
 			uint64_t e = ph;
@@ -682,13 +693,92 @@
 	}
 }
 
+template<int ST>
+DEV void osc2_voice_chunks(const CoefRsrc &crs, Osc2Voice &s, const unsigned (&ldph)[2], const unsigned (&mm)[2],
+		const Osc2Lds &lv, int nsc, int nfs, bool last, int v0, int v1, int v, int lane, int (*tile)[2][A2D_FRAG],
+		int (&phlo_l)[2], int (&phhi_l)[2])
+{
+	const int nopre_i[OSC2_FCH] = { 0, 0, 0, 0 };
+	const unsigned nopre_u[OSC2_FCH] = { 0, 0, 0, 0 };
+	for(int k = 0; k < nsc; ++k) {
+		const bool park = last && k == nsc - 1;
+		int xs[OSC2_FCH];
+		osc2_chunk<true, ST>(crs, s, ldph, nopre_i, nopre_u, nfs - k * OSC2_FCH, park, xs, lv);
+#pragma unroll
+		for(int j = 0; j < OSC2_FCH; ++j) {
+			tile_add(&tile[k * OSC2_FCH + j][0][lane], mul64s(xs[j], v0, 24));
+			tile_add(&tile[k * OSC2_FCH + j][1][lane], mul64s(xs[j], v1, 24));
+		}
+		if(park) {
+			const bool me = lane == v;
+#pragma unroll
+			for(int o = 0; o < 2; ++o) {
+				const uint64_t endph = s.end[o] << mm[o];
+				WRL(phlo_l[o], (int)(unsigned)endph);
+				WRL(phhi_l[o], (int)(unsigned)(endph >> 32));
+			}
+		}
+	}
+}
+
+template<bool STAGE>
+DEV void osc2_superchunk(const CoefRsrc &crs, const int *wavecoef, int *busmem, const int (&od)[2][OD_NWORDS],
+		const int (&amp_l)[2], int (&phlo_l)[2], int (&phhi_l)[2], int settled_l, int my_off, int my_nch, int v0l, int v1l,
+		int nv, int nsc, int fa, int nfs, bool last, unsigned before, int lane, int dbg, int (*tile)[2][A2D_FRAG],
+		LdsInt *level)
+{
+	int cur_off = rdl(my_off, 0), cur_nch = rdl(my_nch, 0);
+	for(int v = 0; v < nv; ++v) {
+		const int sl = rdl(settled_l, v);
+		if(!sl)
+			continue;
+		const int voff = rdl(my_off, v);
+		if(voff != cur_off) {
+			flush_tile(busmem, cur_off, cur_nch, fa, nfs, nsc * OSC2_FCH, lane, dbg, tile);
+			cur_off = voff;
+			cur_nch = rdl(my_nch, v);
+		}
+		const int v0 = rdl(v0l, v), v1 = rdl(v1l, v);
+		Osc2Voice s;
+		unsigned ldph[2], mm[2];
+		osc2_voice_from_lanes(s, ldph, mm, od, amp_l, phlo_l, phhi_l, v, before, lane);
+		Osc2Lds lv = { { level, level }, { 0, 0 } };
+		if(!STAGE) {
+			osc2_voice_chunks<0>(crs, s, ldph, mm, lv, nsc, nfs, last, v0, v1, v, lane, tile, phlo_l, phhi_l);
+			continue;
+		}
+		const int st = sl >> 1;
+		if(st) {
+			lds_wave_fence();
+			if(st & 1) {
+				lv.lg[0] = (unsigned)__builtin_ctz(s.sizem[0]);
+				stage_level(level, wavecoef, s.cb[0], s.sizem[0], lane);
+			}
+			if(st & 2) {
+				LdsInt *const l1 = (st & 1) ? level + s.sizem[0] * A2D_COEF_WORDS : level;
+				lv.level[1] = l1;
+				lv.lg[1] = (unsigned)__builtin_ctz(s.sizem[1]);
+				stage_level(l1, wavecoef, s.cb[1], s.sizem[1], lane);
+			}
+			lds_wave_fence();
+		}
+		switch(st) {
+		case 0: osc2_voice_chunks<0>(crs, s, ldph, mm, lv, nsc, nfs, last, v0, v1, v, lane, tile, phlo_l, phhi_l); break;
+		case 1: osc2_voice_chunks<1>(crs, s, ldph, mm, lv, nsc, nfs, last, v0, v1, v, lane, tile, phlo_l, phhi_l); break;
+		case 2: osc2_voice_chunks<2>(crs, s, ldph, mm, lv, nsc, nfs, last, v0, v1, v, lane, tile, phlo_l, phhi_l); break;
+		default: osc2_voice_chunks<3>(crs, s, ldph, mm, lv, nsc, nfs, last, v0, v1, v, lane, tile, phlo_l, phhi_l); break;
+		}
+	}
+	flush_tile(busmem, cur_off, cur_nch, fa, nfs, nsc * OSC2_FCH, lane, dbg, tile);
+}
+
 #define OSC2_WPE 4
 __global__ __launch_bounds__(64 * FAST_WPB) __attribute__((amdgpu_waves_per_eu(OSC2_WPE, OSC2_WPE)))
 void k_leaf_osc2pan(const A2DParams *__restrict__ pp, const int *__restrict__ list, int nlist, int vpw,
 		int ysplit, const A2DVoice *__restrict__ voices, const int *ustate, int *ustage,
 		const int16_t *__restrict__ wavepool, const A2DWave *__restrict__ waves,
 		const uint32_t *__restrict__ ptab, int *__restrict__ busmem, const int *__restrict__ wavecoef,
-		unsigned char *__restrict__ staged, int vmajor)
+		unsigned char *__restrict__ staged, int vmajor, int lds_taps)
 {
 	const A2DParams &p = *pp;
 	const int wv = rfl((int)(threadIdx.x >> 6));
@@ -732,6 +822,7 @@
 		my_nch = vc.out_nch;
 		bool settled = true;
 		int wave_l[2], dphase_l[2];
+		unsigned periodic[2] = { 0, 0 };
 #pragma unroll
 		for(int o = 0; o < 2; ++o) {
 			uu[o] = vc.unit[o];
@@ -753,15 +844,20 @@
 		if(settled) {
 #pragma unroll
 			for(int o = 0; o < 2; ++o)
-				settled = settled_wave(waves + wave_l[o], (unsigned)dphase_l[o], od[o], settled);
+				settled = settled_wave(waves + wave_l[o], (unsigned)dphase_l[o], od[o], settled, &periodic[o]);
 			a2s_pan_gains(sp[PW_VOL], sp[PW_PAN], a2s_pan_over(sp[PW_PAN]), &v0l, &v1l);
 		}
 		settled_l = settled ? 1 : 0;
+		if(settled && lds_taps)
+			settled_l |= (int)a2d_osc2_stage((unsigned)od[0][OD_SIZEM], periodic[0], (unsigned)od[1][OD_SIZEM], periodic[1]) << 1;
 	}
 	const unsigned long long unsettled_mask = __ballot(mine && !settled_l);
+	const bool any_staged = __ballot(settled_l > 1) != 0;
 
 	__shared__ int tiles[FAST_WPB][OSC2_SCH][2][A2D_FRAG];
+	__shared__ int levels[FAST_WPB][A2D_OSC2_LDS_ENT * A2D_COEF_WORDS];
 	int (*const tile)[2][A2D_FRAG] = tiles[wv];
+	LdsInt *const level = (LdsInt *)levels[wv];
 	if(vmajor)
 #pragma unroll
 		for(int r = 0; r < OSC2_SCH; ++r)
@@ -772,44 +868,12 @@
 		const bool last = last_slice && s_hi == c_hi;
 		const unsigned before = (unsigned)frames_of(fst, fa);
 		if(vmajor && a2d_osc2_whole(before, (unsigned)frames_of(fst, fa + nfs - 1), (unsigned)frames_of(ffr, fa + nfs - 1), nfs)) {
-			const int nsc = s_hi - s_lo;
-			const int nopre_i[OSC2_FCH] = { 0, 0, 0, 0 };
-			const unsigned nopre_u[OSC2_FCH] = { 0, 0, 0, 0 };
-			int cur_off = rdl(my_off, 0), cur_nch = rdl(my_nch, 0);
-			for(int v = 0; v < nv; ++v) {
-				if(!rdl(settled_l, v))
-					continue;
-				const int voff = rdl(my_off, v);
-				if(voff != cur_off) {
-					flush_tile(busmem, cur_off, cur_nch, fa, nfs, nsc * OSC2_FCH, lane, dbg, tile);
-					cur_off = voff;
-					cur_nch = rdl(my_nch, v);
-				}
-				const int v0 = rdl(v0l, v), v1 = rdl(v1l, v);
-				Osc2Voice s;
-				unsigned ldph[2], mm[2];
-				osc2_voice_from_lanes(s, ldph, mm, od, amp_l, phlo_l, phhi_l, v, before, lane);
-				for(int k = 0; k < nsc; ++k) {
-					const bool park = last && k == nsc - 1;
-					int xs[OSC2_FCH];
-					osc2_chunk<true>(crs, s, ldph, nopre_i, nopre_u, nfs - k * OSC2_FCH, park, xs);
-#pragma unroll
-					for(int j = 0; j < OSC2_FCH; ++j) {
-						tile_add(&tile[k * OSC2_FCH + j][0][lane], mul64s(xs[j], v0, 24));
-						tile_add(&tile[k * OSC2_FCH + j][1][lane], mul64s(xs[j], v1, 24));
-					}
-					if(park) {
-						const bool me = lane == v;
-#pragma unroll
-						for(int o = 0; o < 2; ++o) {
-							const uint64_t endph = s.end[o] << mm[o];
-							WRL(phlo_l[o], (int)(unsigned)endph);
-							WRL(phhi_l[o], (int)(unsigned)(endph >> 32));
-						}
-					}
-				}
-			}
-			flush_tile(busmem, cur_off, cur_nch, fa, nfs, nsc * OSC2_FCH, lane, dbg, tile);
+			if(any_staged)
+				osc2_superchunk<true>(crs, wavecoef, busmem, od, amp_l, phlo_l, phhi_l, settled_l, my_off, my_nch, v0l, v1l,
+						nv, s_hi - s_lo, fa, nfs, last, before, lane, dbg, tile, level);
+			else
+				osc2_superchunk<false>(crs, wavecoef, busmem, od, amp_l, phlo_l, phhi_l, settled_l, my_off, my_nch, v0l, v1l,
+						nv, s_hi - s_lo, fa, nfs, last, before, lane, dbg, tile, level);
 			continue;
 		}
 		for(int c = s_lo; c < s_hi; ++c) {
@@ -2808,7 +2872,8 @@
 }
 
 int a2d_launch_leaf_osc2pan(const A2DParams *dparams, const A2DParams &hp, const int *dlist, int nlist,
-		int vpw, int ysplit, int *ustage, unsigned char *staged, void *stream, A2DCommit *defer, int voice_major, int *ysplit_used)
+		int vpw, int ysplit, int *ustage, unsigned char *staged, void *stream, A2DCommit *defer, int voice_major, int lds_taps,
+		int *ysplit_used)
 {
 	if(nlist <= 0)
 		return 0;
@@ -2821,7 +2886,7 @@
 	int nblocks = (nwaves + FAST_WPB - 1) / FAST_WPB;
 	hipLaunchKernelGGL(k_leaf_osc2pan, dim3(nblocks, ysplit), dim3(64 * FAST_WPB), 0, (hipStream_t)stream,
 			dparams, dlist, nlist, vpw, ysplit, hp.voices, (const int *)hp.ustate,
-			ysplit > 1 ? ustage : hp.ustate, hp.wavepool, hp.waves, hp.ptab, hp.busmem, hp.wavecoef, staged, voice_major);
+			ysplit > 1 ? ustage : hp.ustate, hp.wavepool, hp.waves, hp.ptab, hp.busmem, hp.wavecoef, staged, voice_major, lds_taps);
 	if(ysplit > 1) {
 		A2DCommit cm = { dlist, nlist, 2, ustage, staged };
 		if(defer)
diff --git a/audiality2_amd/csrc/a2amd_host.cpp b/audiality2_amd/csrc/a2amd_host.cpp
--- a/audiality2_amd/csrc/a2amd_host.cpp
+++ b/audiality2_amd/csrc/a2amd_host.cpp
@@ -2,6 +2,7 @@
 #include "a2amd_noisemap.h"
 #include "a2amd_cutsweep.h"
 #include "a2amd_settled.h"
+#include "a2amd_wavepads.h"
 
 namespace a2h { thread_local char g_err[256] = ""; }
 
@@ -373,6 +374,8 @@
 		if(!cap) {
 			HIPCHK(c, hipMemcpy(c->d_wavepool.d + pos, w->data[l], n * sizeof(int16_t), hipMemcpyHostToDevice));
 			c->wave_h2d_bytes += n * sizeof(int16_t);
+			if((w->flags & 0x100u) && a2w_pads_periodic(w->data[l], w->size[l], A2AMD_WAVEPRE, A2AMD_WAVEPOST))
+				hw.dw.periodic |= 1u << l;
 		}
 		loff[l] = (uint32_t)(pos - pos0);
 		lsize[l] = w->size[l];
diff --git a/audiality2_amd/csrc/a2amd_render.cpp b/audiality2_amd/csrc/a2amd_render.cpp
--- a/audiality2_amd/csrc/a2amd_render.cpp
+++ b/audiality2_amd/csrc/a2amd_render.cpp
@@ -1,4 +1,5 @@
 #include "a2amd_host.h"
+#include "a2amd_wavepads.h"
 
 extern "C" {
 static double now_us()
@@ -496,6 +497,16 @@
 	return A2AMD_OK;
 }
 
+unsigned a2amd_osc2_stage_rule(unsigned size0, int periodic0, unsigned size1, int periodic1)
+{
+	return a2d_osc2_stage(size0, periodic0 != 0, size1, periodic1 != 0);
+}
+
+int a2amd_wave_level_periodic(const int16_t *level, unsigned size)
+{
+	return a2w_pads_periodic(level, size, A2AMD_WAVEPRE, A2AMD_WAVEPOST);
+}
+
 int a2amd_last_batch_fbdpan(const a2amd_ctx *c, a2amd_fbdpan_batch_info *out)
 {
 	if(!c || !out)
diff --git a/audiality2_amd/csrc/a2amd_sched.cpp b/audiality2_amd/csrc/a2amd_sched.cpp
--- a/audiality2_amd/csrc/a2amd_sched.cpp
+++ b/audiality2_amd/csrc/a2amd_sched.cpp
@@ -1546,8 +1546,9 @@
 		int vpw, ysplit;
 		pick_fast_shape(c->sw, osc2pan.count, c->nfrags * A2D_FAST_FCH / A2D_OSC2_FCH, &vpw, &ysplit, 16);
 		const int voice_major = !(c->sw.debug & 16);
+		const int lds_taps = !(c->sw.debug & (1 << 17));
 		if(a2d_launch_leaf_osc2pan(c->d_params, c->hparams, list + osc2pan.first, osc2pan.count,
-				vpw, ysplit, c->d_ustage.d, c->d_staged.d + osc2pan.first, c->stream, &pend.c[pend.n], voice_major, &ysplit))
+				vpw, ysplit, c->d_ustage.d, c->d_staged.d + osc2pan.first, c->stream, &pend.c[pend.n], voice_major, lds_taps, &ysplit))
 			return c->fail(A2AMD_EHIP, "2-osc leaf launch failed: %s", hipGetErrorString(hipGetLastError()));
 		c->last_osc2.launched = 1;
 		c->last_osc2.voices = (uint32_t)osc2pan.count;
diff --git a/audiality2_amd/csrc/a2amd_taps.h b/audiality2_amd/csrc/a2amd_taps.h
--- a/audiality2_amd/csrc/a2amd_taps.h
+++ b/audiality2_amd/csrc/a2amd_taps.h
@@ -105,6 +105,35 @@
 DEV Coef4 coef_at(const CoefRsrc rs, int cb, unsigned ph)
 {
 	return a2d_coef_load(rs, (int)(ph >> 8), 0, cb, 0);
+}
+
+typedef __attribute__((address_space(3))) int LdsInt;
+DEV Coef4 coef_lds(const LdsInt *level, unsigned ph, unsigned lg)
+{
+	const LdsInt *e = level + A2D_COEF_WORDS * __builtin_amdgcn_ubfe(ph, 8, lg);
+	Coef4 k;
+	k.x = e[0];
+	k.y = e[1];
+	k.z = e[2];
+	return k;
+}
+
+DEV void stage_level(LdsInt *level, const int *wavecoef, int cb, unsigned size, int lane)
+{
+	const int *src = wavecoef + ((unsigned)cb >> 2);
+	const unsigned n = size * A2D_COEF_WORDS;
+#pragma unroll
+	for(int r = 0; r < A2D_OSC2_LDS_ENT * A2D_COEF_WORDS / 64; ++r) {
+		const unsigned i = (unsigned)(r * 64 + lane);
+		if(i < n)
+			level[i] = src[i];
+	}
+}
+
+DEV void lds_wave_fence()
+{
+	__builtin_amdgcn_fence(__ATOMIC_ACQ_REL, "wavefront");
+	__builtin_amdgcn_wave_barrier();
 }
 
 DEV unsigned tap_phase(uint64_t ph, unsigned ldph)
diff --git a/audiality2_amd/csrc/a2amd_wavepads.h b/audiality2_amd/csrc/a2amd_wavepads.h
--- /dev/null
+++ b/audiality2_amd/csrc/a2amd_wavepads.h
@@ -0,0 +1,18 @@
+#pragma once
+#include <stdint.h>
+
+static inline int a2w_pads_periodic(const int16_t *d, uint32_t size, uint32_t pre, uint32_t post)
+{
+	if(!d || !size || !pre)
+		return 0;
+	const int16_t *p = d + pre;
+	if(p[-1] != p[size - 1])
+		return 0;
+	for(uint32_t k = 0, j = 0; k < post; ++k) {
+		if(p[size + k] != p[j])
+			return 0;
+		if(++j == size)
+			j = 0;
+	}
+	return 1;
+}
diff --git a/audiality2_amd/replay.py b/audiality2_amd/replay.py
--- a/audiality2_amd/replay.py
+++ b/audiality2_amd/replay.py
@@ -206,6 +206,10 @@
         self._last_batch_osc2 = None
         if hasattr(lib, prefix + "last_batch_osc2"):
             self._last_batch_osc2 = fn("last_batch_osc2", i32, vp, C.POINTER(a2amd_osc2_batch_info))
+        self._osc2_stage_rule = self._wave_level_periodic = None
+        if hasattr(lib, prefix + "osc2_stage_rule"):
+            self._osc2_stage_rule = fn("osc2_stage_rule", u32, u32, i32, u32, i32)
+            self._wave_level_periodic = fn("wave_level_periodic", i32, C.POINTER(C.c_int16), u32)
         self._last_batch_fbdpan = None
         if hasattr(lib, prefix + "last_batch_fbdpan"):
             self._last_batch_fbdpan = fn("last_batch_fbdpan", i32, vp, C.POINTER(a2amd_fbdpan_batch_info))
@@ -351,6 +355,17 @@
         bi = a2amd_osc2_batch_info()
         self._chk(self._last_batch_osc2(self.ctx, C.byref(bi)), "last_batch_osc2")
         return bi
+
+    def osc2_stage_rule(self, size0, periodic0, size1, periodic1):
+        if self._osc2_stage_rule is None:
+            raise RuntimeError(f"this library has no {self.prefix}osc2_stage_rule")
+        return int(self._osc2_stage_rule(size0, int(bool(periodic0)), size1, int(bool(periodic1))))
+
+    def wave_level_periodic(self, level):
+        if self._wave_level_periodic is None:
+            raise RuntimeError(f"this library has no {self.prefix}wave_level_periodic")
+        arr = np.ascontiguousarray(level, dtype=np.int16)
+        return bool(self._wave_level_periodic(arr.ctypes.data_as(C.POINTER(C.c_int16)), len(arr) - WAVEPRE - WAVEPOST))
 
     def last_batch_fbdpan(self):
         if self._last_batch_fbdpan is None:
diff --git a/include/a2amd.h b/include/a2amd.h
--- a/include/a2amd.h
+++ b/include/a2amd.h
@@ -201,5 +201,6 @@
 #include "a2amd_buswin.h"
 #include "a2amd_vmbatch.h"
 #include "a2amd_osc2.h"
+#include "a2amd_osc2lds.h"
 
 #endif
diff --git a/include/a2amd_osc2lds.h b/include/a2amd_osc2lds.h
--- /dev/null
+++ b/include/a2amd_osc2lds.h
@@ -0,0 +1,16 @@
+#ifndef A2AMD_OSC2LDS_H
+#define A2AMD_OSC2LDS_H
+#include <stdint.h>
+
+#ifdef __cplusplus
+extern "C" {
+#endif
+
+unsigned a2amd_osc2_stage_rule(unsigned size0, int periodic0, unsigned size1, int periodic1);
+
+int a2amd_wave_level_periodic(const int16_t *level, unsigned size);
+
+#ifdef __cplusplus
+}
+#endif
+#endif
```

Measured after the change: 534.6 billion voice-samples/s (median of 6 runs). 1.8% higher.
